# ruihuang1124/CAFE-MPC

Measured on AMD Instinct MI355X. Metric: DDP iterations/sec, Mini-Cheetah WB N=200, batch=4096; 1/2/4/8 GPU, higher is better.
Workload: dtype f64

## Files before the change

### cafe-mpc_amd/csrc/hkd_knot.hpp

```cpp
#pragma once
#include "hs_types.hpp"
#include "srb_knot.hpp"

namespace hs {

constexpr double HKD_MASS = 8.912;
constexpr double HKD_IXX = 0.02746078, HKD_IYY = 0.2425157968, HKD_IZZ = 0.2651935768;

template <class S>
HD void hkd_body_step(const S* xb, const S* pxy, const S* F, double dt, const int* contact, S* out) {
    S sy, cy, st, ct, sp, cp;
    sincos_(xb[0], sy, cy); sincos_(xb[1], st, ct); sincos_(xb[2], sp, cp);
    const V3<S> w{xb[6], xb[7], xb[8]};
    const S dyaw = (sp * w.y + cp * w.z) * srb_recip(ct);
    const S dth = cp * w.y - sp * w.z;
    const S dph = w.x + st * dyaw;
    V3<S> Fs{S(0.0), S(0.0), S(0.0)}, tw{S(0.0), S(0.0), S(0.0)};
    for (int l = 0; l < 4; l++) if (contact[l]) {
        const V3<S> f{F[3 * l], F[3 * l + 1], F[3 * l + 2]};
        const V3<S> r{pxy[2 * l] - xb[3], pxy[2 * l + 1] - xb[4], -xb[5]};
        Fs = Fs + f; tw = tw + cross(r, f);
    }
    const V3<S> tb = rotT<0, S>(cp, sp, rotT<1, S>(ct, st, rotT<2, S>(cy, sy, tw)));
    const V3<S> Iw{HKD_IXX * w.x, HKD_IYY * w.y, HKD_IZZ * w.z};
    const V3<S> rhs = tb - cross(w, Iw);
    out[0] = xb[0] + dt * dyaw; out[1] = xb[1] + dt * dth; out[2] = xb[2] + dt * dph;
    for (int i = 0; i < 3; i++) out[3 + i] = xb[3 + i] + dt * xb[9 + i];
    out[6] = xb[6] + dt * (rhs.x * (1.0 / HKD_IXX)); out[7] = xb[7] + dt * (rhs.y * (1.0 / HKD_IYY)); out[8] = xb[8] + dt * (rhs.z * (1.0 / HKD_IZZ));
    out[9] = xb[9] + dt * (Fs.x * (1.0 / HKD_MASS)); out[10] = xb[10] + dt * (Fs.y * (1.0 / HKD_MASS)); out[11] = xb[11] + dt * (Fs.z * (1.0 / HKD_MASS) - GRAV);
}

template <class S>
HD V3<S> hkd_foot(const S* pos, const S* eul, const S* ql, int leg, double cpsi, double spsi) {
    const double sx = leg < 2 ? 1.0 : -1.0, sgy = (leg % 2 == 0) ? -1.0 : 1.0;
    S s0, c0, s1, c1, s2, c2, sy, cy, st, ct, sp, cp;
    sincos_(ql[0], s0, c0); sincos_(ql[1], s1, c1); sincos_(ql[2], s2, c2);
    sincos_(eul[0], sy, cy); sincos_(eul[1], st, ct); sincos_(eul[2], sp, cp);
    V3<S> w{S(0.0), S(0.0), S(-0.195)};
    w = rot<1, S>(c2, s2, w); w.z = w.z - 0.209;
    w = rot<1, S>(c1, s1, w); w = rot<2, S>(cpsi, spsi, w); w.y = w.y + sgy * 0.062;
    w = rot<0, S>(c0, s0, w); w.x = w.x + sx * 0.19; w.y = w.y + sgy * 0.049;
    w = rot<2, S>(cy, sy, rot<1, S>(ct, st, rot<0, S>(cp, sp, w)));
    return {w.x + pos[0], w.y + pos[1], w.z + pos[2]};
}

struct HkdLds {
    double x[24], xb[24], u[24], xn[24], red[24], tmp[24];
    double K[576];
    double gval[20], bar[20], bd[20], bdd[20];
    double J[4 * 27];
    double pf[12], hx[4 * 24], coefg[4], coefh[4];
};

HD double hkd_grf_row(const double* u, int f, int r, double mu) {
    const double fx = u[3 * f], fy = u[3 * f + 1], fz = u[3 * f + 2];
    return r == 0 ? fz : r == 1 ? -fx + mu * fz : r == 2 ? fx + mu * fz : r == 3 ? -fy + mu * fz : fy + mu * fz;
}
HD double hkd_footreg(PhaseC& P, const double* x, int b, int k) {
    const double* fp = P.foot_pos + ref_row(P, b, k) * 12; const double* bp = P.body_pos + ref_row(P, b, k) * 3;
    double s = 0;
    for (int f = 0; f < 4; f++) for (int a = 0; a < 3; a++) { const double d = (x[12 + 3 * f + a] - x[3 + a]) - (fp[3 * f + a] - bp[a]); s += d * (P.contact[f] * P.w_foot_reg[a]) * d; }
    return s;
}

template <int NT>
HD void hkd_rollout_knot(HkdLds& L, PhaseC& P, int b, int k, double eps, int reb_active, const double* x0, SlotOut so, size_t slot, int* fail_flag, bool ss = false, bool wr = true) {
    const int h = P.h;
    const size_t kx = ((size_t)b * (h + 1) + k) * 24, ku = ((size_t)b * h + k) * 24, kk = (size_t)b * h + k;
    HS_PHASE(NT, if (tid < 24) { double xb = P.Xbar[kx + tid], x = ss ? P.Xsim[kx + tid] : xb + eps * P.dX[kx + tid]; L.xb[tid] = xb; L.x[tid] = x; if (wr) { P.X[kx + tid] = x; if (ss && k == 0) P.Defect[kx + tid] = 0.0; } }
             for (int i = tid; i < 576; i += NT) L.K[i] = P.K[kk * 576 + i];)
    HS_PHASE(NT, if (tid < 24) {
        double s = 0; for (int j = 0; j < 24; j++) s += L.K[tid + 24 * j] * (L.x[j] - L.xb[j]);
        const double u = P.Ubar[ku + tid] + eps * P.dU[ku + tid] + s;
        L.u[tid] = u; if (wr) P.U[ku + tid] = u;
    })
    HS_PHASE(NT, if (tid == 0) {
        double pxy[8]; for (int l = 0; l < 4; l++) { pxy[2 * l] = L.x[12 + 3 * l]; pxy[2 * l + 1] = L.x[13 + 3 * l]; }
        hkd_body_step<double>(L.x, pxy, L.u, P.dt, P.contact, L.xn);
    } else if (tid >= 32 && tid < 44) { const int j = tid - 32; L.xn[12 + j] = P.contact[j / 3] ? L.x[12 + j] : L.x[12 + j] + P.dt * L.u[12 + j]; })
    HS_PHASE(NT, if (tid < 24) {
        const double xs = L.xn[tid];
        if (wr) P.Xsim[kx + 24 + tid] = xs;
        const double d = ss ? 0.0 : xs - (P.Xbar[kx + 24 + tid] + eps * P.dX[kx + 24 + tid]);
        if (wr) P.Defect[kx + 24 + tid] = d;
        double dsq = d * d;
        if (x0 != nullptr && k == 0) { const double d0 = x0[(size_t)b * 24 + tid] - L.x[tid]; if (wr) { P.Xsim[kx + tid] = x0[(size_t)b * 24 + tid]; P.Defect[kx + tid] = d0; } dsq += d0 * d0; }
        L.red[tid] = dsq; L.tmp[tid] = xs * xs;
// ... 1 lines not shown
        const int c = tid - 32; const size_t gi = kk * P.ng + c;
        const double g = hkd_grf_row(L.u, P.feet[c / 5], c % 5, P.mu);
        L.gval[c] = g; if (wr) P.g[gi] = g; L.bar[c] = P.eps[gi] * reb_barrier(g, P.delta[gi]);
    })
    HS_PHASE(NT, if (tid == 0) {
        double lq = 0, lr = 0;
        const size_t rw = ref_row(P, b, k);
        for (int i = 0; i < 24; i++) { const double d = L.x[i] - P.xr[rw * 24 + i]; lq += d * P.q[i] * d; }
        for (int i = 0; i < 24; i++) { const double d = L.u[i] - P.ur[rw * 24 + i]; lr += d * P.r[i] * d; }
        double l = 0.5 * lq; l += 0.5 * lr; l *= P.dt;
        if (P.w_foot_reg[0] >= 0) { double t = .5 * hkd_footreg(P, L.x, b, k); t *= P.dt; l += t; }
        if (wr) P.lbase[kk] = l;
        double ming = 0;
        if (P.ng > 0) {
            double c = 0; for (int i = 0; i < P.ng; i++) { c += L.bar[i]; ming = fmin(ming, L.gval[i]); }
            if (reb_active) l += P.dt * c;
        }
        if (wr) P.l[kk] = l;
        double dsq = 0, nsq = 0; for (int i = 0; i < 24; i++) { dsq += L.red[i]; nsq += L.tmp[i]; }
        so.cost[slot] = l; so.dsq[slot] = dsq; so.ming[slot] = ming; so.maxh[slot] = 0.0;
        if (sqrt(nsq) > 1e6 || !(nsq == nsq)) fail_flag[b] = 1;
    })
}

template <int NT>
HD void hkd_rollout_terminal(HkdLds& L, PhaseC& P, PhaseC* Pn, const ModelDev& md, int b, double eps, int al_active, SlotOut so, size_t slot, bool ss = false, bool wr = true) {
    const int h = P.h;
    const size_t kx = ((size_t)b * (h + 1) + h) * 24;
    HS_PHASE(NT, if (tid < 24) { const double x = ss ? P.Xsim[kx + tid] : P.Xbar[kx + tid] + eps * P.dX[kx + tid]; L.x[tid] = x; if (wr) P.X[kx + tid] = x; })
    HS_PHASE(NT, if (tid < 4 && P.td[tid]) {
        const V3<double> f = hkd_foot<double>(L.x + 3, L.x, L.x + 12 + 3 * tid, tid, md.cpsi_kin, md.spsi_kin);
        L.pf[3 * tid] = f.x; L.pf[3 * tid + 1] = f.y; L.pf[3 * tid + 2] = f.z;
    })
    HS_PHASE(NT, if (tid == 0) {
        double s = 0; const size_t rw = ref_row(P, b, h); for (int i = 0; i < 24; i++) { const double d = L.x[i] - P.xr[rw * 24 + i]; s += d * P.qf[i] * d; }
        double pb = 0.5 * s;
        if (P.w_foot_reg[0] >= 0) pb += 10 * hkd_footreg(P, L.x, b, h);
        if (wr) P.Phibase[b] = pb;
        double maxh = 0, c = 0; int i = 0;
        for (int f = 0; f < 4; f++) if (P.td[f] && P.nt > 0) {
            const double hh = L.pf[3 * f + 2] - P.ground_height; if (wr) P.th[(size_t)b * P.nt + i] = hh; maxh = fmax(maxh, fabs(hh));
            const double sg = P.sigma[(size_t)b * P.nt + i], lm = P.lambda[(size_t)b * P.nt + i];
            c += 0.5 * sg * hh * hh; c += lm * hh; i++;
        }
        double Phi = pb; if (al_active && P.nt > 0) Phi += c;
        if (wr) P.Phi[b] = Phi;
        so.cost[slot] = Phi; so.ming[slot] = 0.0; so.maxh[slot] = maxh; so.dsq[slot] = 0.0;
    })
    if (Pn == nullptr) return;
    const size_t nx = ((size_t)b * (Pn->h + 1)) * 24;
    HS_PHASE(NT, if (tid < 24) {
        double xi = L.x[tid];
        if (tid >= 12) {
            const int l = (tid - 12) / 3, a = (tid - 12) % 3;
            if (P.contact[l] && !P.next_contact[l]) xi = (a == 0) ? 0.0 : (a == 1) ? -0.8 : 1.7;
            if (!P.contact[l] && P.next_contact[l]) xi = (a < 2) ? L.pf[3 * l + a] : 0.0;
        }
        if (wr) Pn->Xsim[nx + tid] = xi;
        const double d = (ss || !Pn->shooting) ? 0.0 : xi - (Pn->Xbar[nx + tid] + eps * Pn->dX[nx + tid]);
        if (wr) Pn->Defect[nx + tid] = d; L.red[tid] = d * d;
    })
    HS_PHASE(NT, if (tid == 0) { double s = 0; for (int i = 0; i < 24; i++) s += L.red[i]; so.dsq[slot] = s; })
}

template <int NT>
HD void hkd_lq_knot(HkdLds& L, PhaseC& P, int b, int k, int reb_active) {
    const int h = P.h; const double dt = P.dt;
    const size_t kx = ((size_t)b * (h + 1) + k) * 24, ku = ((size_t)b * h + k) * 24, kk = (size_t)b * h + k;
    double* AB = L.K;
    HS_PHASE(NT, if (tid < 24) { L.x[tid] = P.X[kx + tid]; L.u[tid] = P.U[ku + tid]; })
    HS_PHASE(NT, if (tid < 32) {
        Dual xb[12], pxy[8], F[12], out[12];
        for (int i = 0; i < 12; i++) { xb[i] = Dual(L.x[i], (tid == i) ? 1.0 : 0.0); F[i] = Dual(L.u[i], (tid == 20 + i) ? 1.0 : 0.0); }
        for (int i = 0; i < 8; i++) pxy[i] = Dual(L.x[12 + 3 * (i / 2) + (i % 2)], (tid == 12 + i) ? 1.0 : 0.0);
        hkd_body_step<Dual>(xb, pxy, F, dt, P.contact, out);
        for (int i = 0; i < 12; i++) AB[i * 32 + tid] = out[i].d;
    } else if (tid >= 32 && tid < 32 + P.ng) {
        const int c = tid - 32; const size_t gi = kk * P.ng + c;
        const double g = P.g[gi], delta = P.delta[gi], e = P.eps[gi]; double bd, bdd;
        if (g > delta) { bd = -1.0 / g; bdd = 1.0 / (g * g); } else { bd = (g - 2 * delta) / delta / delta; bdd = 1.0 / (delta * delta); }
        L.bd[c] = reb_active ? e * bd : 0.0; L.bdd[c] = reb_active ? e * bdd : 0.0;
    })
    const double fr = (P.w_foot_reg[0] >= 0) ? 1.0 : 0.0;
    HS_PHASE(NT, for (int e = tid; e < 576; e += NT) {
        const int r = e % 24, c = e / 24;
        double a, bb;
        if (r < 12) {
            if (c < 12) a = AB[r * 32 + c];
            else { const int l = (c - 12) / 3, ax = (c - 12) % 3; a = (ax < 2) ? AB[r * 32 + 12 + 2 * l + ax] : 0.0; }
            bb = (c < 12) ? AB[r * 32 + 20 + c] : 0.0;
        } else {
            a = (r == c) ? 1.0 : 0.0;
            bb = (r == c && !P.contact[(r - 12) / 3]) ? dt : 0.0;
        }
        rec_put(P, kk, P.oA + e, a); rec_put(P, kk, P.oB + e, bb);
        double q = (r == c) ? dt * P.q[r] : 0.0;
        if (fr != 0.0) {
            if (r == c && r >= 3 && r < 6) { for (int f = 0; f < 4; f++) q += dt * P.contact[f] * P.w_foot_reg[r - 3]; }
            else if (r == c && r >= 12) q += dt * P.contact[(r - 12) / 3] * P.w_foot_reg[(r - 12) % 3];
            else if (r >= 3 && r < 6 && c >= 12 && (c - 12) % 3 == r - 3) q -= dt * P.contact[(c - 12) / 3] * P.w_foot_reg[r - 3];
            else if (c >= 3 && c < 6 && r >= 12 && (r - 12) % 3 == c - 3) q -= dt * P.contact[(r - 12) / 3] * P.w_foot_reg[c - 3];
        }
        rec_put(P, kk, P.oLxx + e, q);
        double uu = (r == c) ? dt * P.r[r] : 0.0;
        if (P.go_grf >= 0 && r < 12 && c < 12 && r / 3 == c / 3) {
            const int f = r / 3; int a2 = -1; for (int t = 0; t < P.nc; t++) if (P.feet[t] == f) a2 = t;
            if (a2 >= 0) for (int cc = 0; cc < 5; cc++) {
                const double r0 = (cc == 1) ? -1.0 : (cc == 2) ? 1.0 : 0.0, r1 = (cc == 3) ? -1.0 : (cc == 4) ? 1.0 : 0.0, r2 = (cc == 0) ? 1.0 : P.mu;
                const double vr = (r % 3 == 0) ? r0 : (r % 3 == 1) ? r1 : r2, vc = (c % 3 == 0) ? r0 : (c % 3 == 1) ? r1 : r2;
                uu += dt * L.bdd[P.go_grf + 5 * a2 + cc] * vr * vc;
            }
        }
        rec_put(P, kk, P.oLuu + e, uu);
    } if (tid < 24) {
        const int i = tid;
        const size_t rw = ref_row(P, b, k);
        double lx = dt * P.q[i] * (L.x[i] - P.xr[rw * 24 + i]);
        if (fr != 0.0) {
            const double* fp = P.foot_pos + rw * 12; const double* bp = P.body_pos + rw * 3;
            if (i >= 3 && i < 6) { for (int f = 0; f < 4; f++) lx -= dt * P.contact[f] * P.w_foot_reg[i - 3] * ((L.x[12 + 3 * f + i - 3] - L.x[i]) - (fp[3 * f + i - 3] - bp[i - 3])); }
            else if (i >= 12) { const int f = (i - 12) / 3, a = (i - 12) % 3; lx += dt * P.contact[f] * P.w_foot_reg[a] * ((L.x[i] - L.x[3 + a]) - (fp[3 * f + a] - bp[a])); }
        }
        rec_put(P, kk, P.oLx + i, lx);
        double lu = dt * P.r[i] * (L.u[i] - P.ur[rw * 24 + i]);
        if (P.go_grf >= 0 && i < 12) {
            const int f = i / 3; int a2 = -1; for (int t = 0; t < P.nc; t++) if (P.feet[t] == f) a2 = t;
            if (a2 >= 0) for (int cc = 0; cc < 5; cc++) {
                const double r0 = (cc == 1) ? -1.0 : (cc == 2) ? 1.0 : 0.0, r1 = (cc == 3) ? -1.0 : (cc == 4) ? 1.0 : 0.0, r2 = (cc == 0) ? 1.0 : P.mu;
                lu += dt * L.bd[P.go_grf + 5 * a2 + cc] * ((i % 3 == 0) ? r0 : (i % 3 == 1) ? r1 : r2);
            }
        }
        rec_put(P, kk, P.oLu + i, lu);
    })
}

template <int NT>
HD void hkd_lq_terminal(HkdLds& L, PhaseC& P, PhaseC* Pn, const ModelDev& md, int b, int al_active) {
    const int h = P.h;
    const size_t kx = ((size_t)b * (h + 1) + h) * 24;
    HS_PHASE(NT, if (tid < 24) L.x[tid] = P.X[kx + tid]; for (int i = tid; i < 96; i += NT) L.hx[i] = 0.0; for (int i = tid; i < 108; i += NT) L.J[i] = 0.0;)
    HS_PHASE(NT, if (tid < 24 && P.td[tid / 6]) {
        const int l = tid / 6, d = tid % 6;
        Dual pos[3], eul[3], ql[3];
        for (int i = 0; i < 3; i++) { pos[i] = Dual(L.x[3 + i]); eul[i] = Dual(L.x[i], (d == i) ? 1.0 : 0.0); ql[i] = Dual(L.x[12 + 3 * l + i], (d == 3 + i) ? 1.0 : 0.0); }
        const V3<Dual> f = hkd_foot<Dual>(pos, eul, ql, l, md.cpsi_kin, md.spsi_kin);
        L.J[l * 27 + 0 * 9 + 3 + d] = f.x.d; L.J[l * 27 + 1 * 9 + 3 + d] = f.y.d; L.J[l * 27 + 2 * 9 + 3 + d] = f.z.d;
        if (d < 3) L.J[l * 27 + d * 9 + d] = 1.0;
    })
    HS_PHASE(NT, if (tid == 0) {
        int t = 0;
        for (int f = 0; f < 4; f++) if (P.td[f] && P.nt > 0) {
            const double sg = P.sigma[(size_t)b * P.nt + t], lm = P.lambda[(size_t)b * P.nt + t], hh = P.th[(size_t)b * P.nt + t];
            L.coefg[t] = al_active ? sg * hh + lm : 0.0; L.coefh[t] = al_active ? sg * (1 + hh) + lm : 0.0;
            for (int j = 0; j < 3; j++) { L.hx[t * 24 + j] = L.J[f * 27 + 2 * 9 + 3 + j]; L.hx[t * 24 + 3 + j] = L.J[f * 27 + 2 * 9 + j]; L.hx[t * 24 + 12 + 3 * f + j] = L.J[f * 27 + 2 * 9 + 6 + j]; }
            t++;
        }
    })
    const double fr = (P.w_foot_reg[0] >= 0) ? 20.0 : 0.0;
    HS_PHASE(NT, for (int e = tid; e < 576; e += NT) {
        const int r = e % 24, c = e / 24;
        double q = (r == c) ? P.qf[r] : 0.0;
        if (fr != 0.0) {
            if (r == c && r >= 3 && r < 6) { for (int f = 0; f < 4; f++) q += fr * P.contact[f] * P.w_foot_reg[r - 3]; }
            else if (r == c && r >= 12) q += fr * P.contact[(r - 12) / 3] * P.w_foot_reg[(r - 12) % 3];
            else if (r >= 3 && r < 6 && c >= 12 && (c - 12) % 3 == r - 3) q -= fr * P.contact[(c - 12) / 3] * P.w_foot_reg[r - 3];
            else if (c >= 3 && c < 6 && r >= 12 && (r - 12) % 3 == c - 3) q -= fr * P.contact[(r - 12) / 3] * P.w_foot_reg[c - 3];
        }
        for (int t = 0; t < P.nt; t++) q += L.coefh[t] * (L.hx[t * 24 + r] * L.hx[t * 24 + c]);
        P.Phixx[(size_t)b * 576 + e] = q;
        if (Pn != nullptr) {
            double v = (r == c) ? 1.0 : 0.0;
            if (r >= 12) {
                const int l = (r - 12) / 3, a = (r - 12) % 3;
                if (P.contact[l] && !P.next_contact[l]) v = 0.0;
                if (!P.contact[l] && P.next_contact[l]) {
                    if (a == 2) v = 0.0;
                    else if (c < 3) v = L.J[l * 27 + a * 9 + 3 + c];
                    else if (c < 6) v = L.J[l * 27 + a * 9 + (c - 3)];
                    else if (c >= 12 && (c - 12) / 3 == l) v = L.J[l * 27 + a * 9 + 6 + (c - 12) % 3];
                    else v = 0.0;
                }
            }
            P.Px[(size_t)b * 576 + e] = v;
        }
    } if (tid < 24) {
        const int i = tid;
        const size_t rw = ref_row(P, b, h);
        double px = P.qf[i] * (L.x[i] - P.xr[rw * 24 + i]);
        if (fr != 0.0) {
            const double* fp = P.foot_pos + rw * 12; const double* bp = P.body_pos + rw * 3;
            if (i >= 3 && i < 6) { for (int f = 0; f < 4; f++) px -= fr * P.contact[f] * P.w_foot_reg[i - 3] * ((L.x[12 + 3 * f + i - 3] - L.x[i]) - (fp[3 * f + i - 3] - bp[i - 3])); }
            else if (i >= 12) { const int f = (i - 12) / 3, a = (i - 12) % 3; px += fr * P.contact[f] * P.w_foot_reg[a] * ((L.x[i] - L.x[3 + a]) - (fp[3 * f + a] - bp[a])); }
        }
        for (int t = 0; t < P.nt; t++) px += L.coefg[t] * L.hx[t * 24 + i];
        P.Phix[(size_t)b * 24 + i] = px;
    })
// ... 4 lines not shown
```

### cafe-mpc_amd/csrc/hs_host.hpp

```cpp
#pragma once
#include <cstring>
#include <vector>
#include <algorithm>
#include "hsddp.h"
#include "hs_types.hpp"

#if !defined(__HIP_DEVICE_COMPILE__)
namespace hs {

inline bool phase_chain_ok(int model, int next_model) {
    if (model == HSDDP_MODEL_WB) return next_model == HSDDP_MODEL_WB || next_model == HSDDP_MODEL_SRB;
    return model == next_model;
}

template <class Mem>
int setup_phase(Mem& mem, const hsddp_phase_desc_t& d, const hsddp_phase_desc_t* next, bool is_last, size_t B, PhaseDev& P, int slot0, bool f32 = false) {
    std::memset(&P, 0, sizeof(P));
    P.model = d.model; P.h = d.horizon; P.dt = d.dt; P.bg_alpha = d.BG_alpha;
    if (d.model == HSDDP_MODEL_WB) { P.n = 36; P.m = 12; P.p = 12; } else if (d.model == HSDDP_MODEL_SRB) { P.n = 12; P.m = 12; P.p = 0; } else { P.n = 24; P.m = 24; P.p = 0; }
    const size_t n = P.n, m = P.m, py = P.p;
    for (int l = 0; l < 4; l++) {
        P.contact[l] = d.contact[l]; P.next_contact[l] = d.next_contact[l];
        if (d.contact[l] > 0) P.feet[P.nc++] = l;
        P.td[l] = (d.contact[l] == 0 && d.next_contact[l] == 1) ? 1 : 0; P.n_td += P.td[l];
    }
    P.has_impact = P.n_td > 0; P.next_model = d.next_model; P.shooting = d.shooting; P.is_last = is_last ? 1 : 0;
    P.next_n = next ? (next->model == HSDDP_MODEL_WB ? 36 : next->model == HSDDP_MODEL_SRB ? 12 : 24) : P.n;
    std::memcpy(P.q, d.q, sizeof(P.q)); std::memcpy(P.r, d.r, sizeof(P.r)); std::memcpy(P.qf, d.qf, sizeof(P.qf));
    std::memcpy(P.w_foot_reg, d.w_foot_reg, 24); std::memcpy(P.w_swing_pos, d.w_swing_pos, 24); std::memcpy(P.w_swing_vel, d.w_swing_vel, 24);
    P.w_td_vel = d.w_td_vel;
    P.c_torque = d.c_torque; P.c_joint = d.c_joint; P.c_minheight = d.c_minheight; P.c_grf = d.c_grf; P.c_touchdown = d.c_touchdown;
    P.torque_limit = d.torque_limit; std::memcpy(P.joint_lb, d.joint_lb, 24); std::memcpy(P.joint_ub, d.joint_ub, 24);
    P.h_min = d.h_min; P.mu = d.mu; P.ground_height = d.ground_height;
    P.c_jspeed = d.c_jointspeed; P.jspeed_lb = d.jointspeed_lb; P.jspeed_ub = d.jointspeed_ub;
    const hsddp_reb_t* rb[5] = {&d.reb_torque, &d.reb_joint, &d.reb_minheight, &d.reb_grf, &d.reb_jointspeed};
    for (int g = 0; g < 5; g++) { P.reb_init[g][0] = rb[g]->delta; P.reb_init[g][1] = rb[g]->delta_min; P.reb_init[g][2] = rb[g]->eps; }
    P.al_init[0] = d.al_td.sigma; P.al_init[1] = d.al_td.lambda; P.al_init[2] = d.al_td.sigma_max;
    int ng = 0; P.go_torque = P.go_joint = P.go_height = P.go_grf = P.go_jspeed = -1;
    const bool wb = d.model == HSDDP_MODEL_WB;
    if (wb && d.c_torque) { P.go_torque = ng; ng += 24; }
    if (wb && d.c_jointspeed) { P.go_jspeed = ng; ng += 24; }
    if (wb && d.c_joint) { P.go_joint = ng; ng += 24; }
    if (d.c_minheight) { P.go_height = ng; ng += 1; }
    const bool hkd = d.model == HSDDP_MODEL_HKD, srb = d.model == HSDDP_MODEL_SRB;
    if (hkd) { ng = 0; P.go_height = -1; }
    if ((wb || hkd) && d.c_grf && P.nc > 0) { P.go_grf = ng; ng += 5 * P.nc; }
    if (srb) { P.n_td = 0; P.has_impact = 0; for (int l = 0; l < 4; l++) P.td[l] = 0; }
    P.ng = ng; P.nt = (!srb && d.c_touchdown) ? P.n_td : 0; P.slot0 = slot0;
    { int offs[5], sz[5]; P.nobj = constraint_objects(P, offs, sz); P.obj_off = P.obj_sz = 0;
      for (int o = 0; o < P.nobj; o++) { P.obj_off |= (unsigned long long)offs[o] << (8 * o); P.obj_sz |= (unsigned long long)sz[o] << (8 * o); } }
    const size_t h1 = P.h + 1, hh = P.h;
    bool ok = true;
    auto up = [&](const double** dst, const double* src, size_t cnt) { void* p = mem.alloc(cnt * 8); if (!p) { ok = false; return; } if (src) mem.upload(p, src, cnt * 8); *dst = (const double*)p; };
    up(&P.xr, d.xr, h1 * n); up(&P.ur, d.ur, h1 * m); up(&P.yr, py ? d.yr : nullptr, h1 * std::max<size_t>(py, 1));
    up(&P.foot_pos, d.foot_pos, h1 * 12); up(&P.foot_vel, d.foot_vel, h1 * 12); up(&P.body_pos, d.body_pos, h1 * 3);
    { void* p = mem.alloc(h1 * 4 * sizeof(int)); if (!p) ok = false; else { if (d.ref_contact) mem.upload(p, d.ref_contact, h1 * 4 * sizeof(int)); P.ref_contact = (const int*)p; } }
    if (d.model == HSDDP_MODEL_WB) {
        std::vector<double> rr(h1 * 80, 0.0);
        for (size_t k = 0; k < h1; k++) {
            double* r = rr.data() + k * 80;
            if (d.xr) for (int i = 0; i < 36; i++) r[i] = d.xr[k * 36 + i];
            if (d.ur) for (int i = 0; i < 12; i++) r[36 + i] = d.ur[k * 12 + i];
            if (d.foot_vel) for (int i = 0; i < 12; i++) r[48 + i] = d.foot_vel[k * 12 + i];
            if (d.ref_contact) for (int i = 0; i < 4; i++) r[60 + i] = (double)d.ref_contact[k * 4 + i];
            for (int i = 0; i < 12; i++) r[64 + i] = (d.foot_pos ? d.foot_pos[k * 12 + i] : 0.0) - (d.body_pos ? d.body_pos[k * 3 + i % 3] : 0.0);
        }
        up(&P.rref, rr.data(), h1 * 80);
    }
    auto al = [&](double** dst, size_t cnt) { void* p = mem.alloc(std::max<size_t>(cnt, 1) * 8); if (!p) ok = false; *dst = (double*)p; };
    double** sx[] = {&P.X, &P.Xbar, &P.Xsim, &P.Defect, &P.Defect_bar, &P.dX, &P.G};
    for (auto p : sx) al(p, B * h1 * n);
    double** su[] = {&P.U, &P.Ubar, &P.dU, &P.Qu, &P.KdX};
    for (auto p : su) al(p, B * hh * m);
    al(&P.Y, B * hh * py);
    double** smn[] = {&P.K, &P.Qux};
    for (auto p : smn) al(p, B * hh * m * n);
    al(&P.Quu, B * hh * m * m);
    {
        auto rnd = [](size_t x) { return (x + 255) / 256 * 256; };
        const size_t ar = (size_t)rec_arows((int)n);
        const size_t oA = 0, oLxx = oA + rnd(ar * n), oB = oLxx + rnd(n * n), oC = oB + rnd(ar * m), oD = oC + rnd(py * n), oLuu = oD + rnd(py * m),
                     oLyy = oLuu + rnd(m * m), oLx = oLyy + rnd(py * py), oLu = oLx + n, oLy = oLu + m, size = oLx + rnd(n + m + py);
        P.rs = (int)size;
        P.oA = (int)oA; P.oLxx = (int)oLxx; P.oB = (int)oB; P.oC = (int)oC; P.oD = (int)oD; P.oLuu = (int)oLuu; P.oLyy = (int)oLyy; P.oLx = (int)oLx; P.oLu = (int)oLu; P.oLy = (int)oLy;
        if (f32) { void* p = mem.alloc(std::max<size_t>(B * hh * size, 1) * sizeof(float)); if (!p) ok = false; P.rec32 = (float*)p; }
        else al(&P.rec, B * hh * size);
        if (P.rec) { P.A = P.rec + oA; P.lxx = P.rec + oLxx; P.B = P.rec + oB; P.C = P.rec + oC; P.D = P.rec + oD; P.luu = P.rec + oLuu;
                     P.lyy = P.rec + oLyy; P.lx = P.rec + oLx; P.lu = P.rec + oLu; P.ly = P.rec + oLy; }
    }
    al(&P.l, B * hh); al(&P.lbase, B * hh);
    al(&P.Phi, B); al(&P.Phibase, B); al(&P.Phix, B * n); al(&P.Phixx, B * n * n); al(&P.H0, B * n * n); al(&P.Px, B * (size_t)P.next_n * n);
    al(&P.g, B * hh * ng); al(&P.delta, B * hh * ng); al(&P.eps, B * hh * ng);
    if (wb) al(&P.kc, B * hh * KC_SIZE);
    al(&P.th, B * P.nt); al(&P.sigma, B * P.nt); al(&P.lambda, B * P.nt);
    if (!ok) return HSDDP_ENOMEM;
    if (ng > 0) {
        std::vector<double> dl(hh * ng), ep(hh * ng);
        for (size_t k = 0; k < hh; k++) for (int c = 0; c < ng; c++) { int grp = constraint_group(P, c); dl[k * ng + c] = P.reb_init[grp][0]; ep[k * ng + c] = P.reb_init[grp][2]; }
        mem.upload(P.delta, dl.data(), dl.size() * 8); mem.replicate(P.delta, dl.size() * 8, B);
        mem.upload(P.eps, ep.data(), ep.size() * 8); mem.replicate(P.eps, ep.size() * 8, B);
    }
    if (P.nt > 0) { std::vector<double> sg(B * P.nt, P.al_init[0]), lm(B * P.nt, P.al_init[1]); mem.upload(P.sigma, sg.data(), sg.size() * 8); mem.upload(P.lambda, lm.data(), lm.size() * 8); }
    return HSDDP_OK;
}

inline const double* field_dev(const PhaseDev& P, int f, int& count, int& elems) {
    const int n = P.n, m = P.m, p = P.p, h = P.h;
    switch (f) {
        case HSDDP_F_X: count = h + 1; elems = n; return P.X;
        case HSDDP_F_XBAR: count = h + 1; elems = n; return P.Xbar;
        case HSDDP_F_XSIM: count = h + 1; elems = n; return P.Xsim;
        case HSDDP_F_DEFECT: count = h + 1; elems = n; return P.Defect;
        case HSDDP_F_DX: count = h + 1; elems = n; return P.dX;
        case HSDDP_F_G: count = h + 1; elems = n; return P.G;
        case HSDDP_F_U: count = h; elems = m; return P.U;
        case HSDDP_F_UBAR: count = h; elems = m; return P.Ubar;
        case HSDDP_F_DU: count = h; elems = m; return P.dU;
        case HSDDP_F_QU: count = h; elems = m; return P.Qu;
        case HSDDP_F_Y: count = h; elems = p; return P.Y;
        case HSDDP_F_K: count = h; elems = m * n; return P.K;
        case HSDDP_F_QUX: count = h; elems = m * n; return P.Qux;
        case HSDDP_F_QUU: count = h; elems = m * m; return P.Quu;
        case HSDDP_F_A: count = h; elems = n * n; return P.A;
        case HSDDP_F_B: count = h; elems = n * m; return P.B;
        case HSDDP_F_C: count = h; elems = p * n; return P.C;
        case HSDDP_F_D: count = h; elems = p * m; return P.D;
        case HSDDP_F_L: count = h; elems = 1; return P.l;
        case HSDDP_F_LX: count = h; elems = n; return P.lx;
        case HSDDP_F_LU: count = h; elems = m; return P.lu;
        case HSDDP_F_LY: count = h; elems = p; return P.ly;
        case HSDDP_F_LXX: count = h; elems = n * n; return P.lxx;
        case HSDDP_F_LUX: count = h; elems = m * n; return nullptr;
        case HSDDP_F_LUU: count = h; elems = m * m; return P.luu;
        case HSDDP_F_LYY: count = h; elems = p * p; return P.lyy;
        case HSDDP_F_PHI: count = 1; elems = 1; return P.Phi;
        case HSDDP_F_PHIX: count = 1; elems = n; return P.Phix;
        case HSDDP_F_PHIXX: count = 1; elems = n * n; return P.Phixx;
        case HSDDP_F_H0: count = 1; elems = n * n; return P.H0;
        case HSDDP_F_REB_EPS: count = h; elems = P.ng; return P.eps;
        case HSDDP_F_REB_DELTA: count = h; elems = P.ng; return P.delta;
        case HSDDP_F_AL_SIGMA: count = 1; elems = P.nt; return P.sigma;
        case HSDDP_F_AL_LAMBDA: count = 1; elems = P.nt; return P.lambda;
        default: count = 0; elems = 0; return nullptr;
    }
}

inline bool wb_structured(const PhaseDev& P, int f) { return P.model == HSDDP_MODEL_WB && (f == HSDDP_F_A || f == HSDDP_F_B); }
inline void wb_expand_ab(int f, double dt, const double* stored, double* full) {
    const int cols = f == HSDDP_F_A ? 36 : 12;
    for (int c = 0; c < cols; c++) for (int r = 0; r < 36; r++) {
        double v;
        if (r >= 18) v = stored[(r - 18) + 18 * c];
        else v = f == HSDDP_F_A ? ((c == r ? 1.0 : 0.0) + (c == 18 + r ? dt : 0.0)) : 0.0;
        full[r + 36 * c] = v;
    }
}

inline const double* field_dev(const PhaseDev& P, int f, int& count, int& elems, int& stride) {
    const double* base = field_dev(P, f, count, elems);
    const bool in_rec = (f == HSDDP_F_A || f == HSDDP_F_B || f == HSDDP_F_C || f == HSDDP_F_D || f == HSDDP_F_LX || f == HSDDP_F_LU || f == HSDDP_F_LY ||
                         f == HSDDP_F_LXX || f == HSDDP_F_LUU || f == HSDDP_F_LYY);
    stride = in_rec ? P.rs : elems;
    return base;
}

}
#endif
```

### cafe-mpc_amd/csrc/hs_types.hpp

```cpp
#pragma once
#include "hs_common.hpp"

namespace hs {

constexpr int MAXN = 36, MAXM = 24, MAXP = 12, MAXG = 96;
constexpr int rec_rnd(int x) { return (x + 255) / 256 * 256; }
constexpr int rec_arows(int N) { return N == 36 ? 18 : N; }
template <int N, int M, int PY> struct RecLayout {
    static constexpr int AR = rec_arows(N);
    static constexpr int oA = 0, oLxx = oA + rec_rnd(AR * N), oB = oLxx + rec_rnd(N * N), oC = oB + rec_rnd(AR * M), oD = oC + rec_rnd(PY * N),
                         oLuu = oD + rec_rnd(PY * M), oLyy = oLuu + rec_rnd(M * M), oLx = oLyy + rec_rnd(PY * PY), oLu = oLx + N, oLy = oLu + M,
                         size = oLx + rec_rnd(N + M + PY);
    static constexpr int rA = rec_rnd(AR * N) / 256, rQ = rec_rnd(N * N) / 256, rB = rec_rnd(AR * M) / 256, rC = rec_rnd(PY * N) / 256, rD = rec_rnd(PY * M) / 256,
                         rLuu = rec_rnd(M * M) / 256, rLyy = rec_rnd(PY * PY) / 256;
    static constexpr int rounds = rA + rQ + rB + rC + rD + rLuu + rLyy;
};

constexpr int KC_M = 0, KC_X = 324, KC_LG = 540, KC_RDM = 684, KC_RDG = 702, KC_QDD = 714, KC_GRF = 732, KC_LAM = 744, KC_J = 756, KC_FP = 972, KC_FV = 984, KC_SIZE = 1024;

struct PhaseDev {
    int model, n, m, p, h;
    double dt, bg_alpha;
    int contact[4], next_contact[4], td[4], feet[4];
    int nc, n_td, has_impact, next_model, next_n, shooting, is_last;
    double q[MAXN], r[MAXM], qf[MAXN], w_foot_reg[3], w_swing_pos[3], w_swing_vel[3], w_td_vel;
    int c_torque, c_joint, c_minheight, c_grf, c_touchdown, c_jspeed;
    double torque_limit, joint_lb[3], joint_ub[3], h_min, mu, ground_height, jspeed_lb, jspeed_ub;
    double reb_init[5][3];
    double al_init[3];
    int ng, go_torque, go_joint, go_height, go_grf, go_jspeed;
    int nt;
    int slot0;
    int nobj; unsigned long long obj_off, obj_sz;
    const HS_GLOBAL double *xr, *ur, *yr, *foot_pos, *foot_vel, *body_pos;
    const HS_GLOBAL int* ref_contact;
    const HS_GLOBAL double* rref;
    int ref_pb;
    HS_GLOBAL double *X, *Xbar, *Xsim, *Defect, *Defect_bar, *dX, *G;
    HS_GLOBAL double *U, *Ubar, *dU, *Qu;
    HS_GLOBAL double *KdX;
    HS_GLOBAL double *Y;
    HS_GLOBAL double *K, *Qux, *Quu;
    HS_GLOBAL double *A, *B, *C, *D;
    HS_GLOBAL double* rec; int rs;
    HS_GLOBAL float* rec32;
    int oA, oLxx, oB, oC, oD, oLuu, oLyy, oLx, oLu, oLy;
    HS_GLOBAL double *l, *lbase, *lx, *lu, *ly, *lxx, *luu, *lyy;
    HS_GLOBAL double *Phi, *Phibase, *Phix, *Phixx, *H0, *Px;
    HS_GLOBAL double *g, *delta, *eps;
    HS_GLOBAL double* kc;
    HS_GLOBAL double *th, *sigma, *lambda;
};

template <class PD> HD void rec_put(PD& P, size_t kk, int off, double v) {
    if (P.rec32 != nullptr) P.rec32[kk * P.rs + off] = (float)v; else P.rec[kk * P.rs + off] = v;
}

template <class PD> HD size_t ref_row(PD& P, int b, int k) { return (unsigned)(b * P.ref_pb + k); }

using PhaseC = const HS_CONST PhaseDev;

HDH int constraint_group(const PhaseDev& P, int c) {
    if (P.go_torque >= 0 && c >= P.go_torque && c < P.go_torque + 24) return 0;
    if (P.go_jspeed >= 0 && c >= P.go_jspeed && c < P.go_jspeed + 24) return 4;
    if (P.go_joint >= 0 && c >= P.go_joint && c < P.go_joint + 24) return 1;
    if (P.go_height >= 0 && c == P.go_height) return 2;
    return 3;
}
HDH int constraint_objects(const PhaseDev& P, int* offs, int* sz) {
    int n = 0;
    if (P.go_torque >= 0) { offs[n] = P.go_torque; sz[n++] = 24; }
    if (P.go_jspeed >= 0) { offs[n] = P.go_jspeed; sz[n++] = 24; }
    if (P.go_joint >= 0) { offs[n] = P.go_joint; sz[n++] = 24; }
    if (P.go_height >= 0) { offs[n] = P.go_height; sz[n++] = 1; }
    if (P.go_grf >= 0) { offs[n] = P.go_grf; sz[n++] = 5 * P.nc; }
    return n;
}

struct ProbState {
    double actual_cost, merit, feas, dV_1, dV_2, merit_rho;
    double cost_prev, merit_prev, feas_prev, reg;
    double max_tconstr, max_pconstr, max_tconstr_prev, max_pconstr_prev;
    double info_tconstr, info_pconstr;
    double ls_eps;
    int iter, ls_total, reg_total, status;
    int outer_active, inner_active, ls_active, ls_success, rollout_ok, bs_ok;
    int iter_in, iter_ou;
    int hist_n, push_pending;
    int need_commit, pad_;
};

struct OptDev {
    double alpha, gamma, update_penalty, update_relax, update_regularization, update_ReB;
    int max_DDP_iter, max_AL_iter;
    double cost_thresh, tconstr_thresh, pconstr_thresh, dynamics_feas_thresh, merit_scale, merit_offset;
    int AL_active, ReB_active, MS;
};

struct ModelDev { double cpsi_dyn, spsi_dyn, cpsi_kin, spsi_kin; };

}
```

### cafe-mpc_amd/csrc/hsddp_hip.hip

```cpp
#include <hip/hip_runtime.h>
#include <atomic>
#include <chrono>
#include <cstdio>
#include <cstring>
#include <string>
#include <thread>
#include <vector>
#include <cmath>
#include "hsddp.h"
#include "hsddp_ensemble.h"
#include "hsddp_hkd.h"
#include "hsddp_refs.h"
#include "hsddp_sim.h"
#include "hsddp_mc.h"
#include "hs_types.hpp"
#include "hs_host.hpp"
#include "wb_knot.hpp"
#include "wb_quad.hpp"
#include "srb_knot.hpp"
#include "hkd_knot.hpp"
#include "sweep.hpp"
#include "ensemble.hpp"
#include "hkd_pack.hpp"
#include "refs.hpp"
// ... 1001 lines not shown
    HIPCK(hipGetLastError());
    return HSDDP_OK;
}

int hsddp_hybrid_rollout(hsddp_handle_t* h, double eps, const hsddp_option_t* opt) {
    if (!h || !opt) return HSDDP_EINVAL;
    HIPCK(hipSetDevice(h->device)); OptDev o = to_dev(*opt);
    launch_rollout(h, eps, o, MASK_NONE); launch_eval(h, EV_REDUCE_ONLY, o, 0.0, false, 0);
    HIPCK(hipStreamSynchronize(h->stream)); drain_events(h); HIPCK(hipGetLastError()); return HSDDP_OK;
}
int hsddp_compute_cost(hsddp_handle_t* h, const hsddp_option_t* opt) {
    if (!h || !opt) return HSDDP_EINVAL; HIPCK(hipSetDevice(h->device)); OptDev o = to_dev(*opt);
    launch_cost(h, o, MASK_NONE); launch_eval(h, EV_REDUCE_ONLY, o, 0.0, false, 0);
    HIPCK(hipStreamSynchronize(h->stream)); drain_events(h); HIPCK(hipGetLastError()); return HSDDP_OK;
}
int hsddp_LQ_approximation(hsddp_handle_t* h, const hsddp_option_t* opt) {
    if (!h || !opt) return HSDDP_EINVAL; HIPCK(hipSetDevice(h->device)); OptDev o = to_dev(*opt);
    launch_lq(h, o, MASK_NONE); HIPCK(hipStreamSynchronize(h->stream)); drain_events(h); HIPCK(hipGetLastError()); return HSDDP_OK;
}
int hsddp_backward_sweep(hsddp_handle_t* h, double regularization, int* success) {
    if (!h) return HSDDP_EINVAL; HIPCK(hipSetDevice(h->device)); OptDev o{};
    launch_sweep(h, o, MASK_NONE, regularization, 0, 0, 0.0, h->d_success);
    if (!h->has_hkd && !h->f32) hipLaunchKernelGGL(k_refresh_kdx, dim3(64, h->batch), dim3(64), 0, h->stream, h->d_ph, h->nph);
    HIPCK(hipStreamSynchronize(h->stream)); drain_events(h); HIPCK(hipGetLastError());
    if (success) HIPCK(hipMemcpy(success, h->d_success, h->batch * sizeof(int), hipMemcpyDeviceToHost));
    return HSDDP_OK;
}
int hsddp_linear_rollout(hsddp_handle_t* h, double eps, const hsddp_option_t* opt) {
    (void)opt; if (!h) return HSDDP_EINVAL; HIPCK(hipSetDevice(h->device));
    { Timed t(h, "k_linear");
      if (h->f32) hipLaunchKernelGGL(k_linear32, dim3(h->batch), dim3(SW_NT), 0, h->stream, h->d_ph, h->nph, h->d_st, eps);
      else if (h->has_hkd) hipLaunchKernelGGL(k_linear_hkd, dim3(h->batch), dim3(SW_NT), 0, h->stream, h->d_ph, h->nph, h->d_st, eps);
      else hipLaunchKernelGGL(k_linear, dim3(h->batch), dim3(SW_NT), 0, h->stream, h->d_ph, h->nph, h->d_st, eps); }
    HIPCK(hipStreamSynchronize(h->stream)); drain_events(h); HIPCK(hipGetLastError()); return HSDDP_OK;
}
int hsddp_update_nominal_trajectory(hsddp_handle_t* h) {
    if (!h) return HSDDP_EINVAL; HIPCK(hipSetDevice(h->device));
    launch_update_nominal(h, MASK_NONE); HIPCK(hipStreamSynchronize(h->stream)); drain_events(h); return HSDDP_OK;
}
static int read_states(hsddp_handle* h, std::vector<ProbState>& st) {
    st.resize(h->batch); HIPCK(hipSetDevice(h->device));
    HIPCK(hipMemcpy(st.data(), h->d_st, sizeof(ProbState) * h->batch, hipMemcpyDeviceToHost)); return HSDDP_OK;
}
int hsddp_get_exp_cost_change(hsddp_handle_t* h, double* dV_1, double* dV_2) {
    if (!h || !dV_1 || !dV_2) return HSDDP_EINVAL;
    std::vector<ProbState> st; int rc = read_states(h, st); if (rc) return rc;
    for (int b = 0; b < h->batch; b++) { dV_1[b] = st[b].dV_1; dV_2[b] = st[b].dV_2; } return HSDDP_OK;
}
int hsddp_measure_dynamics_feasibility(hsddp_handle_t* h, double* feas) {
    if (!h || !feas) return HSDDP_EINVAL;
    std::vector<ProbState> st; int rc = read_states(h, st); if (rc) return rc;
    for (int b = 0; b < h->batch; b++) feas[b] = st[b].feas; return HSDDP_OK;
}
int hsddp_get_info(hsddp_handle_t* h, hsddp_info_t* info) {
    if (!h || !info) return HSDDP_EINVAL;
    std::vector<ProbState> st; int rc = read_states(h, st); if (rc) return rc;
    for (int b = 0; b < h->batch; b++) {
        info[b].actual_cost = st[b].actual_cost; info[b].dyn_feas = st[b].feas; info[b].max_tconstr = st[b].info_tconstr; info[b].max_pconstr = st[b].info_pconstr;
        info[b].n_iters = st[b].iter; info[b].n_ls_iters = st[b].ls_total; info[b].n_reg_iters = st[b].reg_total; info[b].status = st[b].status;
    }
    return HSDDP_OK;
}

int hsddp_get_history(hsddp_handle_t* h, int problem, int cap, float* cost, float* dyn_feas, float* eqn_feas, float* ineq_feas, int* n) {
    if (!h || problem < 0 || problem >= h->batch || cap < 0 || !n) return HSDDP_EINVAL;
    HIPCK(hipSetDevice(h->device));
    ProbState st; HIPCK(hipMemcpy(&st, h->d_st + problem, sizeof(ProbState), hipMemcpyDeviceToHost));
    const int have = std::min(st.hist_n, h->hist_cap); *n = have;
    const int m = std::min(have, cap);
    float* dst[4] = {cost, dyn_feas, eqn_feas, ineq_feas};
    for (int q = 0; q < 4 && m > 0; q++) if (dst[q]) HIPCK(hipMemcpy(dst[q], h->d_hist + ((size_t)problem * 4 + q) * h->hist_cap, m * sizeof(float), hipMemcpyDeviceToHost));
    return HSDDP_OK;
}

int hsddp_field_shape(hsddp_handle_t* h, int phase, int field, int* count, int* elems) {
    if (!h || phase < 0 || phase >= h->nph || field < 0 || field >= HSDDP_F_COUNT) return HSDDP_EINVAL;
    int stride; field_dev(h->ph[phase], field, *count, *elems, stride); return HSDDP_OK;
}
int hsddp_get_field(hsddp_handle_t* h, int phase, int field, int b0, int nb, double* dst) {
    if (!h || phase < 0 || phase >= h->nph || field < 0 || field >= HSDDP_F_COUNT || b0 < 0 || nb < 0 || b0 + nb > h->batch || !dst) return HSDDP_EINVAL;
    HIPCK(hipSetDevice(h->device));
    int count, elems, stride; const double* src = field_dev(h->ph[phase], field, count, elems, stride);
    const size_t sz = (size_t)count * elems;
    if (h->f32 && stride != elems && sz > 0 && nb > 0) {
        const PhaseDev& P = h->ph[phase];
        const int off = field == HSDDP_F_A ? P.oA : field == HSDDP_F_B ? P.oB : field == HSDDP_F_C ? P.oC : field == HSDDP_F_D ? P.oD : field == HSDDP_F_LX ? P.oLx : field == HSDDP_F_LU ? P.oLu :
                        field == HSDDP_F_LY ? P.oLy : field == HSDDP_F_LXX ? P.oLxx : field == HSDDP_F_LUU ? P.oLuu : P.oLyy;
        std::vector<float> tmp(sz * nb);
        HIPCK(hipMemcpy2D(tmp.data(), (size_t)elems * 4, P.rec32 + (size_t)b0 * count * stride + off, (size_t)stride * 4, (size_t)elems * 4, (size_t)nb * count, hipMemcpyDeviceToHost));
        for (size_t i = 0; i < tmp.size(); i++) dst[i] = tmp[i];
        return HSDDP_OK;
    }
    if (!src) { memset(dst, 0, sz * nb * 8); return HSDDP_OK; }
    if (sz == 0 || nb == 0) return HSDDP_OK;
    if (wb_structured(h->ph[phase], field)) {
        const int st = field == HSDDP_F_A ? 648 : 216;
        std::vector<double> tmp((size_t)st * nb * count);
        HIPCK(hipMemcpy2D(tmp.data(), (size_t)st * 8, src + (size_t)b0 * count * stride, (size_t)stride * 8, (size_t)st * 8, (size_t)nb * count, hipMemcpyDeviceToHost));
        for (size_t r = 0; r < (size_t)nb * count; r++) wb_expand_ab(field, h->ph[phase].dt, tmp.data() + r * st, dst + r * elems);
        return HSDDP_OK;
    }
    if (stride == elems) HIPCK(hipMemcpy(dst, src + (size_t)b0 * sz, sz * nb * 8, hipMemcpyDeviceToHost));
    else HIPCK(hipMemcpy2D(dst, (size_t)elems * 8, src + (size_t)b0 * count * stride, (size_t)stride * 8, (size_t)elems * 8, (size_t)nb * count, hipMemcpyDeviceToHost));
    return HSDDP_OK;
}
float hsddp_get_solve_time_ms(hsddp_handle_t* h) { return h ? h->solve_ms : 0.f; }

int hsddp_warm_start_phase(hsddp_handle_t* dst, int dphase, hsddp_handle_t* src, int sphase, int shift) {
    if (!dst || dphase < 0 || dphase >= dst->nph || shift < 0) return HSDDP_EINVAL;
    const PhaseDev& D = dst->ph[dphase];
    dst->cache_valid = false;
    const bool has = src != nullptr && sphase >= 0;
    if (has && (sphase >= src->nph || src->batch != dst->batch || src->device != dst->device || src->ph[sphase].model != D.model)) return HSDDP_EINVAL;
    HIPCK(hipSetDevice(dst->device));
    if (has) HIPCK(hipStreamSynchronize(src->stream));
    hipLaunchKernelGGL(k_warm_start, dim3(D.h + 1, dst->batch), dim3(256), 0, dst->stream, D, has ? src->ph[sphase] : D, has ? 1 : 0, shift);
    HIPCK(hipStreamSynchronize(dst->stream));
    return HSDDP_OK;
}

int hsddp_export_mpc_command(hsddp_handle_t* h, int problem, int n_steps, double mpc_time, double dt, const float* status_times, unsigned int* out) {
    if (!h || problem < 0 || problem >= h->batch || n_steps <= 0 || !out) return HSDDP_EINVAL;
    std::vector<int> sp, sk;
    for (int i = 0; i < h->nph && (int)sp.size() < n_steps; i++) {
        if (h->ph[i].model != HSDDP_MODEL_WB) break;
        for (int k = 0; k < h->ph[i].h && (int)sp.size() < n_steps; k++) { sp.push_back(i); sk.push_back(k); }
    }
    if ((int)sp.size() < n_steps) return HSDDP_EINVAL;
    HIPCK(hipSetDevice(h->device));
    const size_t words = 1 + (size_t)n_steps * HSDDP_CMD_WORDS_PER_STEP;
    if (words > h->cmd_words) { if (h->d_cmd) HIPCK(hipFree(h->d_cmd)); h->d_cmd = nullptr; h->cmd_words = 0; HIPCK(hipMalloc((void**)&h->d_cmd, words * 4)); h->cmd_words = words; }
    if (n_steps > h->cmd_steps) { if (h->d_cmd_map) HIPCK(hipFree(h->d_cmd_map)); h->d_cmd_map = nullptr; h->cmd_steps = 0; HIPCK(hipMalloc((void**)&h->d_cmd_map, 2 * (size_t)n_steps * sizeof(int))); h->cmd_steps = n_steps; }
    if (status_times && !h->d_cmd_status) HIPCK(hipMalloc((void**)&h->d_cmd_status, (size_t)h->nph * 4 * sizeof(float)));
    HIPCK(hipMemcpyAsync(h->d_cmd_map, sp.data(), n_steps * sizeof(int), hipMemcpyHostToDevice, h->stream));
    HIPCK(hipMemcpyAsync(h->d_cmd_map + n_steps, sk.data(), n_steps * sizeof(int), hipMemcpyHostToDevice, h->stream));
    if (status_times) HIPCK(hipMemcpyAsync(h->d_cmd_status, status_times, (size_t)h->nph * 4 * sizeof(float), hipMemcpyHostToDevice, h->stream));
    hipLaunchKernelGGL(k_pack_command, dim3(n_steps), dim3(256), 0, h->stream, h->d_ph, h->d_cmd_map, h->d_cmd_map + n_steps, n_steps, problem, mpc_time, dt,
                       status_times ? h->d_cmd_status : nullptr, h->d_cmd);
    HIPCK(hipMemcpyAsync(out, h->d_cmd, words * 4, hipMemcpyDeviceToHost, h->stream));
    HIPCK(hipStreamSynchronize(h->stream));
    return HSDDP_OK;
}

int hsddp_export_solver_info(hsddp_handle_t* h, int problem, unsigned int* out) {
    if (!h || problem < 0 || problem >= h->batch || !out) return HSDDP_EINVAL;
    HIPCK(hipSetDevice(h->device));
    ProbState st; HIPCK(hipMemcpy(&st, h->d_st + problem, sizeof(ProbState), hipMemcpyDeviceToHost));
    const int iv[3] = {st.iter, st.ls_total, st.reg_total};
    const float fv[5] = {h->solve_ms, (float)st.actual_cost, (float)st.feas, (float)st.info_pconstr, (float)st.info_tconstr};
    memcpy(out, iv, sizeof(iv)); memcpy(out + 3, fv, sizeof(fv));
    return HSDDP_OK;
}

int hsddp_get_kernel_units(hsddp_handle_t* h, const char* name, long long* units) {
    if (!h || !name || !units) return HSDDP_EINVAL;
    const int id = !strcmp(name, "k_rollout") ? UNIT_ROLLOUT : !strcmp(name, "k_lq") ? UNIT_LQ : !strcmp(name, "k_sweep") ? UNIT_SWEEP : !strcmp(name, "k_ls_probe") ? UNIT_PROBE : -1;
    if (id < 0) return HSDDP_EINVAL;
    HIPCK(hipSetDevice(h->device));
    unsigned long long v = 0; HIPCK(hipMemcpy(&v, h->d_units + id, sizeof(v), hipMemcpyDeviceToHost));
    *units = (long long)v; return HSDDP_OK;
}

int hsddp_get_kernel_times(hsddp_handle_t* h, int max_n, double* ms, long long* launches, char* names, int names_cap) {
    if (!h) return 0;
    int n = std::min<int>(max_n, (int)h->kname.size()); int pos = 0;
    for (int i = 0; i < n; i++) {
        ms[i] = h->kms[i]; launches[i] = h->kcnt[i];
        int len = (int)h->kname[i].size();
        if (pos + len + 1 < names_cap) { memcpy(names + pos, h->kname[i].c_str(), len + 1); pos += len + 1; }
    }
    if (pos < names_cap) names[pos] = 0;
    return n;
}
#if defined(LQ_PROF) || defined(ROLL_PROF)
int hsddp_debug_lq_prof(unsigned long long* out16, int reset) {
    hipMemcpyFromSymbol(out16, HIP_SYMBOL(g_lq_prof), 16 * sizeof(unsigned long long));
    if (reset) { unsigned long long z[16] = {0}; hipMemcpyToSymbol(HIP_SYMBOL(g_lq_prof), z, sizeof(z)); }
    return 0;
}
#endif
#ifdef QUAD_PROF
int hsddp_debug_quad_prof(unsigned long long* out24, int reset) {
    hipMemcpyFromSymbol(out24, HIP_SYMBOL(g_quad_prof), 24 * sizeof(unsigned long long));
    if (reset) { unsigned long long z[24] = {0}; hipMemcpyToSymbol(HIP_SYMBOL(g_quad_prof), z, sizeof(z)); }
// ... 530 lines not shown
```

### cafe-mpc_amd/csrc/srb_knot.hpp

```cpp
#pragma once
#include "hs_types.hpp"
#include "wb_knot.hpp"

namespace hs {

constexpr double SRB_MASS = 8.912;
constexpr double SRB_IXX = 0.061578036, SRB_IYY = 0.2207093, SRB_IZZ = 0.272612336, SRB_IXZ = 5.38e-5;

HD double srb_recip(double a) { return 1.0 / a; }
HD Dual srb_recip(Dual a) { const double r = 1.0 / a.v; return Dual(r, -a.d * r * r); }

template <class S>
HD void srb_xdot(const S* x, const S* u, const double* pf, const int* contact, S* xd) {
    S sy, cy, st, ct, sp, cp;
    sincos_(x[3], sy, cy); sincos_(x[4], st, ct); sincos_(x[5], sp, cp);
    const S dyaw = x[9], dth = x[10], dph = x[11];
    V3<S> F{S(0.0), S(0.0), S(0.0)}, tw{S(0.0), S(0.0), S(0.0)};
    for (int l = 0; l < 4; l++) if (contact[l]) {
        const V3<S> f{u[3 * l], u[3 * l + 1], u[3 * l + 2]};
        const V3<S> r{S(pf[3 * l]) - x[0], S(pf[3 * l + 1]) - x[1], S(pf[3 * l + 2]) - x[2]};
        F = F + f; tw = tw + cross(r, f);
    }
    for (int i = 0; i < 6; i++) xd[i] = x[6 + i];
    xd[6] = F.x * (1.0 / SRB_MASS); xd[7] = F.y * (1.0 / SRB_MASS); xd[8] = F.z * (1.0 / SRB_MASS) - GRAV;
    const V3<S> tb = rotT<0, S>(cp, sp, rotT<1, S>(ct, st, rotT<2, S>(cy, sy, tw)));
    const V3<S> w{dph - st * dyaw, sp * ct * dyaw + cp * dth, cp * ct * dyaw - sp * dth};
    const V3<S> Iw{SRB_IXX * w.x + SRB_IXZ * w.z, SRB_IYY * w.y, SRB_IXZ * w.x + SRB_IZZ * w.z};
    const V3<S> rhs = tb - cross(w, Iw);
    constexpr double det = SRB_IXX * SRB_IZZ - SRB_IXZ * SRB_IXZ;
    const V3<S> wd{(SRB_IZZ * rhs.x - SRB_IXZ * rhs.z) * (1.0 / det), rhs.y * (1.0 / SRB_IYY), (SRB_IXX * rhs.z - SRB_IXZ * rhs.x) * (1.0 / det)};
    const V3<S> c0d{-(ct * dth), cp * ct * dph - sp * st * dth, -(sp * ct * dph) - cp * st * dth};
    const V3<S> c1d{S(0.0), -(sp * dph), -(cp * dph)};
    const V3<S> bb = wd - (scale(dyaw, c0d) + scale(dth, c1d));
    const S ddyaw = (sp * bb.y + cp * bb.z) * srb_recip(ct);
    xd[9] = ddyaw; xd[10] = cp * bb.y - sp * bb.z; xd[11] = bb.x + st * ddyaw;
}

struct SrbLds {
    double x[12], xb[12], u[12], xd[12], red[12], tmp[12];
    double K[144], AB[288];
    double g, bar, bd, bdd;
};

template <int NT>
HD void srb_rollout_knot(SrbLds& L, PhaseC& P, int b, int k, double eps, int reb_active, const double* x0, SlotOut so, size_t slot, int* fail_flag, bool ss = false, bool wr = true) {
    const int h = P.h;
    const size_t kx = ((size_t)b * (h + 1) + k) * 12, ku = ((size_t)b * h + k) * 12, kk = (size_t)b * h + k;
    HS_PHASE(NT, if (tid < 12) { double xb = P.Xbar[kx + tid], x = ss ? P.Xsim[kx + tid] : xb + eps * P.dX[kx + tid]; L.xb[tid] = xb; L.x[tid] = x; if (wr) { P.X[kx + tid] = x; if (ss && k == 0) P.Defect[kx + tid] = 0.0; } }
             for (int i = tid; i < 144; i += NT) L.K[i] = P.K[kk * 144 + i];)
    HS_PHASE(NT, if (tid < 12) {
        double s = 0; for (int j = 0; j < 12; j++) s += L.K[tid + 12 * j] * (L.x[j] - L.xb[j]);
        const double u = P.Ubar[ku + tid] + eps * P.dU[ku + tid] + s;
        L.u[tid] = u; if (wr) P.U[ku + tid] = u;
    })
    HS_PHASE(NT, if (tid == 0) srb_xdot<double>(L.x, L.u, P.foot_pos + ref_row(P, b, k) * 12, P.ref_contact + ref_row(P, b, k) * 4, L.xd);)
    HS_PHASE(NT, if (tid < 12) {
        const double xs = L.x[tid] + L.xd[tid] * P.dt;
        if (wr) P.Xsim[kx + 12 + tid] = xs;
        const double d = ss ? 0.0 : xs - (P.Xbar[kx + 12 + tid] + eps * P.dX[kx + 12 + tid]);
        if (wr) P.Defect[kx + 12 + tid] = d;
        double dsq = d * d;
        if (x0 != nullptr && k == 0) { const double d0 = x0[(size_t)b * 12 + tid] - L.x[tid]; if (wr) { P.Xsim[kx + tid] = x0[(size_t)b * 12 + tid]; P.Defect[kx + tid] = d0; } dsq += d0 * d0; }
        L.red[tid] = dsq; L.tmp[tid] = xs * xs;
    })
    HS_PHASE(NT, if (tid == 0) {
        double lq = 0, lr = 0;
        const size_t rw = ref_row(P, b, k);
        for (int i = 0; i < 12; i++) { const double d = L.x[i] - P.xr[rw * 12 + i]; lq += d * P.q[i] * d; }
        for (int i = 0; i < 12; i++) { const double d = L.u[i] - P.ur[rw * 12 + i]; lr += d * P.r[i] * d; }
        double l = 0.5 * lq; l += 0.5 * lr; l *= P.dt;
        if (wr) P.lbase[kk] = l;
        double ming = 0;
        if (P.go_height >= 0) {
            const size_t gi = kk * P.ng + P.go_height; const double g = L.x[2] - P.h_min;
            if (wr) P.g[gi] = g; ming = fmin(ming, g);
            if (reb_active) l += P.dt * (P.eps[gi] * reb_barrier(g, P.delta[gi]));
        }
        if (wr) P.l[kk] = l;
        double dsq = 0, nsq = 0; for (int i = 0; i < 12; i++) { dsq += L.red[i]; nsq += L.tmp[i]; }
        so.cost[slot] = l; so.dsq[slot] = dsq; so.ming[slot] = ming; so.maxh[slot] = 0.0;
        if (sqrt(nsq) > 1e6 || !(nsq == nsq)) fail_flag[b] = 1;
    })
}

template <int NT>
HD void srb_rollout_terminal(SrbLds& L, PhaseC& P, PhaseC* Pn, int b, double eps, SlotOut so, size_t slot, bool ss = false, bool wr = true) {
    const int h = P.h;
    const size_t kx = ((size_t)b * (h + 1) + h) * 12;
    HS_PHASE(NT, if (tid < 12) { const double x = ss ? P.Xsim[kx + tid] : P.Xbar[kx + tid] + eps * P.dX[kx + tid]; L.x[tid] = x; if (wr) P.X[kx + tid] = x; })
    HS_PHASE(NT, if (tid == 0) {
        double s = 0; const size_t rw = ref_row(P, b, h); for (int i = 0; i < 12; i++) { const double d = L.x[i] - P.xr[rw * 12 + i]; s += d * P.qf[i] * d; }
        const double Phi = 0.5 * s;
        if (wr) { P.Phibase[b] = Phi; P.Phi[b] = Phi; }
        so.cost[slot] = Phi; so.ming[slot] = 0.0; so.maxh[slot] = 0.0; so.dsq[slot] = 0.0;
    })
    if (Pn == nullptr) return;
    const size_t nx = ((size_t)b * (Pn->h + 1)) * 12;
    HS_PHASE(NT, if (tid < 12) {
        const double xi = L.x[tid];
        if (wr) Pn->Xsim[nx + tid] = xi;
        const double d = (ss || !Pn->shooting) ? 0.0 : xi - (Pn->Xbar[nx + tid] + eps * Pn->dX[nx + tid]);
        if (wr) Pn->Defect[nx + tid] = d; L.red[tid] = d * d;
    })
    HS_PHASE(NT, if (tid == 0) { double s = 0; for (int i = 0; i < 12; i++) s += L.red[i]; so.dsq[slot] = s; })
}

template <int NT>
HD void srb_lq_knot(SrbLds& L, PhaseC& P, int b, int k, int reb_active) {
    const int h = P.h; const double dt = P.dt;
    const size_t kx = ((size_t)b * (h + 1) + k) * 12, ku = ((size_t)b * h + k) * 12, kk = (size_t)b * h + k;
    HS_PHASE(NT, if (tid < 12) { L.x[tid] = P.X[kx + tid]; L.u[tid] = P.U[ku + tid]; })
    HS_PHASE(NT, if (tid < 24) {
        Dual xs[12], us[12], out[12];
        for (int i = 0; i < 12; i++) { xs[i] = Dual(L.x[i], (tid == i) ? 1.0 : 0.0); us[i] = Dual(L.u[i], (tid == 12 + i) ? 1.0 : 0.0); }
        srb_xdot<Dual>(xs, us, P.foot_pos + ref_row(P, b, k) * 12, P.ref_contact + ref_row(P, b, k) * 4, out);
        for (int i = 0; i < 12; i++) L.AB[i + 12 * tid] = out[i].d * dt + ((tid == i) ? 1.0 : 0.0);
    } if (tid == 32) {
        double bd = 0, bdd = 0;
        if (P.go_height >= 0 && reb_active) {
            const size_t gi = kk * P.ng + P.go_height; const double g = P.g[gi], delta = P.delta[gi], e = P.eps[gi];
            if (g > delta) { bd = -1.0 / g; bdd = 1.0 / (g * g); } else { bd = (g - 2 * delta) / delta / delta; bdd = 1.0 / (delta * delta); }
            bd *= e; bdd *= e;
        }
        L.bd = bd; L.bdd = bdd;
    })
    HS_PHASE(NT, for (int e = tid; e < 144; e += NT) {
        const int r = e % 12, c = e / 12;
        rec_put(P, kk, P.oA + e, L.AB[e]); rec_put(P, kk, P.oB + e, L.AB[144 + e]);
        double qd = 0, rd = 0;
        if (r == c) { qd = dt * P.q[r]; rd = dt * P.r[r]; if (r == 2) qd += dt * L.bdd; }
        rec_put(P, kk, P.oLxx + e, qd); rec_put(P, kk, P.oLuu + e, rd);
    } if (tid < 12) {
        double lx = dt * P.q[tid] * (L.x[tid] - P.xr[ref_row(P, b, k) * 12 + tid]); if (tid == 2) lx += dt * L.bd;
        rec_put(P, kk, P.oLx + tid, lx);
        rec_put(P, kk, P.oLu + tid, dt * P.r[tid] * (L.u[tid] - P.ur[ref_row(P, b, k) * 12 + tid]));
    })
}

template <int NT>
HD void srb_lq_terminal(SrbLds& L, PhaseC& P, PhaseC* Pn, int b) {
    const int h = P.h;
    const size_t kx = ((size_t)b * (h + 1) + h) * 12;
    HS_PHASE(NT, if (tid < 12) P.Phix[(size_t)b * 12 + tid] = P.qf[tid] * (P.X[kx + tid] - P.xr[ref_row(P, b, h) * 12 + tid]);
             for (int e = tid; e < 144; e += NT) { P.Phixx[(size_t)b * 144 + e] = (e % 12 == e / 12) ? P.qf[e % 12] : 0.0; if (Pn != nullptr) P.Px[(size_t)b * 144 + e] = (e % 12 == e / 12) ? 1.0 : 0.0; })
    (void)L;
}

}
```

### cafe-mpc_amd/csrc/sweep.hpp

```cpp
#pragma once
#include <cstddef>
#include <limits>
#include <type_traits>
#include "hs_types.hpp"
#include "hs_mfma.hpp"

namespace hs {

constexpr int SW_NT = 256;
constexpr int SW_SET_WB = 0, SW_SET_HKD = 1;
constexpr int SW_N = 36;
constexpr int SW_PRE = 20;
#ifndef SW_UNROLL_N
#define SW_UNROLL_N 4
#endif
#define HS_STR_(x) #x
#define HS_UNROLL_N(n) _Pragma(HS_STR_(unroll n))
#ifndef SW_LDLT_NB
#define SW_LDLT_NB ((M <= 12 || sizeof(R) == 4) ? 2 : 1)
#endif
#ifndef SW_MINB
#define SW_MINB 2
#endif
#ifndef SW_LDLT_WDW
#define SW_LDLT_WDW 1
#endif
#ifndef SW_OVERLAP_LDLT
#define SW_OVERLAP_LDLT 1
#endif

template <int N, int M, int PY, class R = double> struct SweepLdsT {
    static constexpr int LDN = N + 1, LDM = (M > PY ? M : PY) + 1, PYd = PY > 0 ? PY : 1;
    static constexpr int AR = rec_arows(N), LDA = AR + 1, A0 = N - AR;
    R H[LDN * N], A[LDA * N], HA[LDN * N];
    R B[LDA * M], HB[LDN * M];
    R Qux[LDM * N];
    union { R K[LDM * N]; R lC[PY > 0 ? LDM * N : 1]; };
    R C[PY > 0 ? LDM * N : 1], D[PY > 0 ? LDM * M : 1];
    union { R LQ[LDM * M]; R lD[PY > 0 ? LDM * M : 1]; };
    R lyy[PY > 0 ? LDM * PY : 1], Quu[LDM * M];
    R G[N], Gn[N], Qx[N], Qu[M], dU[M], ly[PYd], def[N];
};
template <int N, int M, int PY, class R = double> struct LinLdsT {
    static constexpr int AR = rec_arows(N), A0 = N - AR;
    R A[2][AR * N], Q[2][N * N], B[2][AR * M], K[2][M * N], U[2][M * M], v[2][256];
    R dx[N], dxn[N], du[M];
};
struct SweepCtl { double dV1, dV2, xfer[SW_N]; unsigned long long t_last; int ok; };
constexpr size_t sw_max(size_t a, size_t b) { return a > b ? a : b; }
template <class R> constexpr size_t sweep_bytes_wb() { return sw_max(sw_max(sizeof(SweepLdsT<36, 12, 12, R>), sizeof(LinLdsT<36, 12, 12, R>)), sw_max(sizeof(SweepLdsT<12, 12, 0, R>), sizeof(LinLdsT<12, 12, 0, R>))); }
template <class R> constexpr size_t sweep_bytes_hkd() { return sw_max(sw_max(sizeof(SweepLdsT<24, 24, 0, R>), sizeof(LinLdsT<24, 24, 0, R>)), sw_max(sizeof(SweepLdsT<12, 12, 0, R>), sizeof(LinLdsT<12, 12, 0, R>))); }
template <class R, int SET> struct SweepLdsRaw { R raw[(SET == 0 ? sweep_bytes_wb<R>() : sweep_bytes_hkd<R>()) / sizeof(R)]; SweepCtl c; };
using SweepLds = SweepLdsRaw<double, 0>;
using SweepLdsHkd = SweepLdsRaw<double, 1>;
using SweepLds32 = SweepLdsRaw<float, 1>;

#define CM(M, i, j, ld) (M)[(i) + (ld) * (j)]

#if defined(SW_PROF) && !defined(HS_HOST_EMU)
__device__ unsigned long long g_sw_prof[48];
#define SW_STAMP(i) { if (blockIdx.x == 0 && threadIdx.x == 0) { unsigned long long t_ = clock64(); atomicAdd(&g_sw_prof[i], t_ - SWC.t_last); SWC.t_last = t_; } }
#define SW_STAMP0() { if (blockIdx.x == 0 && threadIdx.x == 0) SWC.t_last = clock64(); }
#define SW_WSTAMP(p) { if (blockIdx.x == 0 && (tid & 63) == 0) atomicAdd(&g_sw_prof[16 + 4 * (p) + (tid >> 6)], clock64() - SWC.t_last); }
#else
#define SW_WSTAMP(p)
#define SW_STAMP(i)
#define SW_STAMP0()
#endif

#ifdef HS_HOST_EMU
#define SW_PRE_DECL static R pre_all_[SW_NT][SW_PRE];
#define PRE(r) pre_all_[tid][r]
#else
#define SW_PRE_DECL R pre_[SW_PRE];
#define PRE(r) pre_[r]
#endif

#ifndef HS_HOST_EMU
template <int CTRL> HD double dpp_quad(double v) {
    const int lo = __builtin_amdgcn_mov_dpp(__double2loint(v), CTRL, 0xf, 0xf, true), hi = __builtin_amdgcn_mov_dpp(__double2hiint(v), CTRL, 0xf, 0xf, true);
    return __hiloint2double(hi, lo);
}
HD double quad_sum(double v) { v += dpp_quad<0xB1>(v); v += dpp_quad<0x4E>(v); return v; }
template <int CTRL> HD float dpp_quad(float v) { return __int_as_float(__builtin_amdgcn_mov_dpp(__float_as_int(v), CTRL, 0xf, 0xf, true)); }
HD float quad_sum(float v) { v += dpp_quad<0xB1>(v); v += dpp_quad<0x4E>(v); return v; }
#endif
#ifdef HS_HOST_EMU
#define SW_QS 1
#define SW_QUAD_ROWS(CNT, PARTIAL, FINISH) if (tid < (CNT)) { const int o = tid; R p_[4]; R p2_[4]; for (int part = 0; part < 4; part++) { R partial = 0; R partial2 = 0; PARTIAL p_[part] = partial; p2_[part] = partial2; } \
    const R total = (p_[0] + p_[1]) + (p_[2] + p_[3]); const R total2 = (p2_[0] + p2_[1]) + (p2_[2] + p2_[3]); (void)total2; FINISH }
#else
#define SW_QS 4
#define SW_QUAD_ROWS(CNT, PARTIAL, FINISH) if ((tid >> 2) < (CNT)) { const int o = tid >> 2; const int part = tid & 3; R partial = 0; R partial2 = 0; PARTIAL \
    const R total = quad_sum(partial); const R total2 = quad_sum(partial2); (void)total2; if (part == 0) FINISH }
#endif

template <int M, int LD, class R, int PART>
HD void ldlt_parts(int tid, const R* A, R diag_add, R* NI, R* Lw, int* iw, int* ok, R* W1 = nullptr, R* W2 = nullptr) {
    const R TOL = R(1.0) / std::numeric_limits<R>::max();
#ifdef HS_HOST_EMU
    if (PART == 2) return;
    if (tid == 0) {
        R m[M * M]; int tr[M]; int sign = 0; (void)Lw; (void)iw;
        for (int j = 0; j < M; j++) for (int i = 0; i < M; i++) m[i + M * j] = A[i + LD * j] + (i == j ? diag_add : 0.0);
        auto Mx = [&](int i, int j) -> R& { return m[i + M * j]; };
        R temp[M];
        for (int k = 0; k < M; k++) {
            int big = k; R best = std::fabs(Mx(k, k));
            for (int i = k + 1; i < M; i++) if (std::fabs(Mx(i, i)) > best) { best = std::fabs(Mx(i, i)); big = i; }
            tr[k] = big;
            if (k != big) {
                for (int j = 0; j < k; j++) { const R t = Mx(k, j); Mx(k, j) = Mx(big, j); Mx(big, j) = t; }
                for (int i = big + 1; i < M; i++) { const R t = Mx(i, k); Mx(i, k) = Mx(i, big); Mx(i, big) = t; }
                { const R t = Mx(k, k); Mx(k, k) = Mx(big, big); Mx(big, big) = t; }
                for (int i = k + 1; i < big; i++) { const R t = Mx(i, k); Mx(i, k) = Mx(big, i); Mx(big, i) = t; }
            }
            for (int j = 0; j < k; j++) temp[j] = Mx(j, j) * Mx(k, j);
            { R s = 0; for (int j = 0; j < k; j++) s += Mx(k, j) * temp[j]; Mx(k, k) -= s; }
            for (int i = k + 1; i < M; i++) { R t = 0; for (int j = 0; j < k; j++) t += Mx(i, j) * temp[j]; Mx(i, k) -= t; }
            const R akk = Mx(k, k); const bool valid = std::fabs(akk) > 0.0;
            if (valid) for (int i = k + 1; i < M; i++) Mx(i, k) /= akk;
            if (sign == 1) { if (akk < 0) sign = 2; } else if (sign == -1) { if (akk > 0) sign = 2; } else if (sign == 0) { if (akk > 0) sign = 1; else if (akk < 0) sign = -1; }
        }
        if (!(sign == 1 || sign == 0)) *ok = 0;
        for (int c = 0; c < M; c++) {
            R x[M]; for (int i = 0; i < M; i++) x[i] = (i == c) ? 1.0 : 0.0;
            for (int k = 0; k < M; k++) if (tr[k] != k) { const R t = x[k]; x[k] = x[tr[k]]; x[tr[k]] = t; }
            for (int i = 0; i < M; i++) { R s = x[i]; for (int j = 0; j < i; j++) s -= Mx(i, j) * x[j]; x[i] = s; }
// ... 43 lines not shown
        int pv[M]; int myrank = 0;
        _Pragma("unroll") for (int k = 0; k < M; k++) { pv[k] = iw[k]; myrank = (pv[k] == me) ? k : myrank; }
        if (PART != 2) {
        const int prow = iw[me];
        R arow[M];
        _Pragma("unroll") for (int j = 0; j < M; j++) { const int r = prow > pv[j] ? prow : pv[j], c = prow > pv[j] ? pv[j] : prow; arow[j] = A[r + LD * c] + ((j == me) ? diag_add : 0.0); }
        SW_LSTAMP(10)
        bool anyneg = false;
        _Pragma("unroll") for (int j = 0; j < M; j++) {
            const R d = hs_readlane(arow[j], j);
            R rd = hs_rcp(d); rd = rd * (R(2.0) - d * rd); rd = rd * (R(2.0) - d * rd);
            rd = (fabs(d) > TOL) ? rd : 0.0;
            anyneg = anyneg || (d < 0.0);
            const R lij = (fabs(d) > 0.0) ? arow[j] * rd : arow[j];
            if (M <= 12) { if (act && me >= j) Lw[me * M + j] = (me == j) ? rd : lij; }
            else if (act) { if (me > j) Lw[me * M + j] = lij; else if (me == j) Lw[j * M + j] = rd; }
            _Pragma("unroll") for (int k = j + 1; k < M; k++) arow[k] -= lij * hs_readlane(arow[j], k);
        }
        SW_LSTAMP(11)
        if (tid == 0 && anyneg) *ok = 0;
        }
        if (PART == 1) return;
        __builtin_amdgcn_fence(__ATOMIC_RELEASE, "wavefront"); __builtin_amdgcn_wave_barrier(); __builtin_amdgcn_fence(__ATOMIC_ACQUIRE, "wavefront");
        constexpr int NB = SW_LDLT_NB;
        R y[M], lr[NB][M];
        if (NB == 1) { lr[0][0] = 0.0; }
        _Pragma("unroll") for (int k = 0; k < M; k++) {
            if (NB == 2) { if (k + 1 < M) { _Pragma("unroll") for (int j = 0; j <= k; j++) lr[(k + 1) % NB][j] = Lw[(k + 1) * M + j]; } }
            else { _Pragma("unroll") for (int j = 0; j < k; j++) lr[0][j] = Lw[k * M + j]; }
            HS_CBAR();
            R sacc = (k == myrank) ? 1.0 : 0.0;
            _Pragma("unroll") for (int j = 0; j < k; j++) sacc -= lr[k % NB][j] * y[j];
            HS_PIN(sacc);
            y[k] = sacc;
        }
        SW_LSTAMP(12)
#if SW_LDLT_WDW
        if (PART == 2 && sizeof(R) == 8) {
            if (act) { _Pragma("unroll") for (int k = 0; k < M; k++) { W1[k + M * me] = y[k]; W2[k + M * me] = -(y[k] * Lw[k * M + k]); } }
            __builtin_amdgcn_fence(__ATOMIC_RELEASE, "wavefront"); __builtin_amdgcn_wave_barrier(); __builtin_amdgcn_fence(__ATOMIC_ACQUIRE, "wavefront");
            constexpr int TMq = (M + 15) / 16;
            MTileT<R> td[TMq * TMq];
            _Pragma("unroll") for (int t = 0; t < TMq * TMq; t++) td[t] = MTileT<R>{NI, LD, nullptr, 0, 16 * (t % TMq), 16 * (t / TMq), M, M, W1, M, W2, M, M, true, nullptr, 0, nullptr, 0, 0};
            mfma_tiles<TMq * TMq, (M + 3) / 4 * 4, 0, R>(tid, td);
            SW_LSTAMP(13)
            return;
        }
#endif
        _Pragma("unroll") for (int k = 0; k < M; k++) y[k] = y[k] * Lw[k * M + k];
        _Pragma("unroll") for (int k = M - 1; k >= 0; k--) {
            if (NB == 2) { if (k > 0) { _Pragma("unroll") for (int j = k; j < M; j++) lr[(k - 1) % NB][j] = Lw[j * M + (k - 1)]; } }
            else { _Pragma("unroll") for (int j = k + 1; j < M; j++) lr[0][j] = Lw[j * M + k]; }
            HS_CBAR();
            R sacc = y[k];
            _Pragma("unroll") for (int j = k + 1; j < M; j++) sacc -= lr[k % NB][j] * y[j];
            HS_PIN(sacc);
            y[k] = sacc;
        }
        if (act) { _Pragma("unroll") for (int k = 0; k < M; k++) NI[pv[k] + LD * me] = -y[k]; }
        SW_LSTAMP(13)
    }
#endif
}
template <int M, int LD, class R>
HD void ldlt_inverse_w(const R* A, R diag_add, R* NI, R* Lw, int* iw, int* ok) {
    HS_WPHASE(ldlt_parts<M, LD, R, 0>(tid, A, diag_add, NI, Lw, iw, ok);)
}
template <int NT, class TD, class TS> HD void ld_mat(int tid, TD* dst, int ldd, const TS* src, int rows, int cols) {
    const int i = tid % rows, j0 = tid / rows, js = NT / rows;
    if (j0 < js) for (int j = j0; j < cols; j += js) dst[i + ldd * j] = src[i + rows * j];
}
template <int NT, class TD, class TS> HD void st_mat(int tid, TD* dst, const TS* src, int lds_, int rows, int cols) {
    const int i = tid % rows, j0 = tid / rows, js = NT / rows;
    if (j0 < js) for (int j = j0; j < cols; j += js) dst[i + rows * j] = src[i + lds_ * j];
}

#define SW_RICCATI_FETCH(kk_, k_) { \
    const HS_GLOBAL R* rec_ = grec + (kk_) * (size_t)RL::size + tid; \
    _Pragma("unroll") for (int r = 0; r < RL::rounds; r++) if (r < RL::rA || r >= RL::rA + RL::rQ) PRE(r) = rec_[NT * r];      \
    PRE(RL::rounds) = (tid < N + M + PY) ? rec_[RL::oLx] : (tid < 2 * N + M + PY) ? (R)gDefect[((size_t)b * (h + 1) + (k_) + 1) * N + tid - N - M - PY] : R(0.0); }
#define SW_RICCATI_FETCH_LXX(kk_) { \
    const HS_GLOBAL R* rec_ = grec + (kk_) * (size_t)RL::size + tid; \
    _Pragma("unroll") for (int r = RL::rA; r < RL::rA + RL::rQ; r++) PRE(r) = rec_[NT * r]; }
#define SW_RICCATI_LXX() { \
    _Pragma("unroll") for (int r = 0; r < RL::rQ; r++) { const int e = tid + NT * r; if (e < N * N) S.H[(e % N) + LDN * (e / N)] += PRE(RL::rA + r); } }
#define SW_RICCATI_COMMIT() { \
    constexpr int PYd = PY > 0 ? PY : 1; \
    _Pragma("unroll") for (int r = 0; r < RL::rA; r++) { const int e = tid + NT * r; if (e < AR * N) S.A[(e % AR) + LDA * (e / AR)] = PRE(r); } \
    _Pragma("unroll") for (int r = 0; r < RL::rB; r++) { const int e = tid + NT * r; if (e < AR * M) S.B[(e % AR) + LDA * (e / AR)] = PRE(RL::rA + RL::rQ + r); } \
    _Pragma("unroll") for (int r = 0; r < RL::rC; r++) { const int e = tid + NT * r; if (e < PY * N) S.C[(e % PYd) + LDM * (e / PYd)] = PRE(RL::rA + RL::rQ + RL::rB + r); } \
    _Pragma("unroll") for (int r = 0; r < RL::rD; r++) { const int e = tid + NT * r; if (e < PY * M) S.D[(e % PYd) + LDM * (e / PYd)] = PRE(RL::rA + RL::rQ + RL::rB + RL::rC + r); } \
    _Pragma("unroll") for (int r = 0; r < RL::rLuu; r++) { const int e = tid + NT * r; if (e < M * M) S.Quu[(e % M) + LDM * (e / M)] = PRE(RL::rA + RL::rQ + RL::rB + RL::rC + RL::rD + r); } \
    _Pragma("unroll") for (int r = 0; r < RL::rLyy; r++) { const int e = tid + NT * r; if (e < PY * PY) S.lyy[(e % PYd) + LDM * (e / PYd)] = PRE(RL::rA + RL::rQ + RL::rB + RL::rC + RL::rD + RL::rLuu + r); } \
    if (tid < N) S.Qx[tid] = PRE(RL::rounds); else if (tid < N + M) S.Qu[tid - N] = PRE(RL::rounds); else if (tid < N + M + PY) S.ly[tid - N - M] = PRE(RL::rounds); \
    else if (tid < 2 * N + M + PY) S.def[tid - N - M - PY] = PRE(RL::rounds); }

template <class R> HD const HS_GLOBAL R* rec_of(const PhaseDev& P);
template <> HD const HS_GLOBAL double* rec_of<double>(const PhaseDev& P) { return P.rec; }
template <> HD const HS_GLOBAL float* rec_of<float>(const PhaseDev& P) { return P.rec32; }

template <class E> HD constexpr int deal_order(int n, int ix) {
    int c = 0;
    for (int e = 0; e < n; e++) if (!E::edge(e)) { if (c == ix) return e; c++; }
    for (int e = 0; e < n; e++) if (E::edge(e)) { if (c == ix) return e; c++; }
    return ix;
}
template <int W, int N, int M, int PY, class R, int DEAL = 0>
HD void sweep_tiles1(SweepLdsT<N, M, PY, R>& S, int lane, R dt) {
    constexpr int LDN = SweepLdsT<N, M, PY, R>::LDN, LDM = SweepLdsT<N, M, PY, R>::LDM, AR = SweepLdsT<N, M, PY, R>::AR, LDA = SweepLdsT<N, M, PY, R>::LDA, A0 = SweepLdsT<N, M, PY, R>::A0;
    constexpr int TN = (N + 15) / 16, TM = (M + 15) / 16, TP = (PY + 15) / 16, TPd = TP > 0 ? TP : 1;
    constexpr int t1 = TN * TN, t2 = t1 + TN * TM, t3 = t2 + TP * TN, t4 = t3 + TP * TM;
    constexpr bool WBT = (DEAL == 0 && t4 == 16 && t3 == 15);
    constexpr int nA = t1 + (t3 - t2), nB = (t2 - t1) + (t4 - t3);
    constexpr int NTL = DEAL == 1 ? (W == 0 ? nB : (nA - (W - 1) + 2) / 3) : WBT ? (W == 0 ? 5 : W == 3 ? 3 : 4) : (t4 - W + 3) / 4;
    if (NTL <= 0) return;
    MTileT<R> td[NTL > 0 ? NTL : 1];
    _Pragma("unroll") for (int q = 0; q < NTL; q++) {
        struct E1 { static constexpr bool edge(int e) { return e < t1 ? mfma_edge_tile<R>(N, N, 16 * (e % TN), 16 * (e / TN)) : mfma_edge_tile<R>(PY, N, 16 * ((e - t1) % TPd), 16 * ((e - t1) / TPd)); } };
        const int ix = DEAL == 1 && W > 0 ? deal_order<E1>(nA, (W - 1) + 3 * q) : (W - 1) + 3 * q;
        const int t = DEAL == 1 ? (W == 0 ? (q < t2 - t1 ? t1 + q : t3 + (q - (t2 - t1))) : (ix < t1 ? ix : t2 + (ix - t1))) : (WBT && W == 0 && q == 4) ? 15 : W + 4 * q;
        if (t < t1) { td[q] = MTileT<R>{S.HA, LDN, nullptr, 0, 16 * (t % TN), 16 * (t / TN), N, N, S.H + LDN * A0, LDN, S.A, LDA, AR, false, nullptr, 0, nullptr, 0, 0};
                      if (A0 > 0) { td[q].T = S.H; td[q].ldt = LDN; td[q].tmode = 1; td[q].tsplit = A0; td[q].tscale = dt; } }
        else if (t < t2) td[q] = MTileT<R>{S.HB, LDN, nullptr, 0, 16 * ((t - t1) % TN), 16 * ((t - t1) / TN), N, M, S.H + LDN * A0, LDN, S.B, LDA, AR, false, nullptr, 0, nullptr, 0, 0};
        else if (t < t3) td[q] = MTileT<R>{S.lC, LDM, nullptr, 0, 16 * ((t - t2) % TPd), 16 * ((t - t2) / TPd), PY, N, S.lyy, LDM, S.C, LDM, PY, false, nullptr, 0, nullptr, 0, 0};
        else td[q] = MTileT<R>{S.lD, LDM, nullptr, 0, 16 * ((t - t3) % TPd), 16 * ((t - t3) / TPd), PY, M, S.lyy, LDM, S.D, LDM, PY, false, nullptr, 0, nullptr, 0, 0};
    }
    mfma_tiles<(NTL > 0 ? NTL : 1), ((AR > PY ? AR : PY) + 3) / 4 * 4, 0, R>(lane, td);
}
template <int W, int N, int M, int PY, class R, int DEAL = 0>
HD void sweep_tiles2(SweepLdsT<N, M, PY, R>& S, int lane, R reg, R dt) {
    constexpr int LDN = SweepLdsT<N, M, PY, R>::LDN, LDM = SweepLdsT<N, M, PY, R>::LDM, AR = SweepLdsT<N, M, PY, R>::AR, LDA = SweepLdsT<N, M, PY, R>::LDA, A0 = SweepLdsT<N, M, PY, R>::A0;
    constexpr int TN = (N + 15) / 16, TM = (M + 15) / 16;
    constexpr int t1 = TN * (TN + 1) / 2, t2 = t1 + TM * TN, t3 = t2 + TM * TM;
    constexpr int NTL = DEAL == 0 ? (t3 - W + 3) / 4 : DEAL == 2 ? (t3 - t2 - W + 3) / 4 : (W == 0 ? t3 - t2 : (t2 - (W - 1) + 2) / 3);
    if (NTL <= 0) return;
    MTileT<R> td[NTL > 0 ? NTL : 1];
    _Pragma("unroll") for (int q = 0; q < NTL; q++) {
        struct E2 { static constexpr bool edge(int e) {
            if (e < t1) { int c = 0; for (int jj = 0; jj < TN; jj++) for (int ii = 0; ii <= jj; ii++) { if (c == e) return mfma_edge_tile<R>(N, N, 16 * ii, 16 * jj); c++; } return false; }
            return mfma_edge_tile<R>(M, N, 16 * ((e - t1) % TM), 16 * ((e - t1) / TM)); } };
        const int t = DEAL == 0 ? W + 4 * q : DEAL == 2 ? t2 + W + 4 * q : (W == 0 ? t2 + q : deal_order<E2>(t2, (W - 1) + 3 * q));
        int bi = 0, bj = 0;
        { int c = 0; for (int jj = 0; jj < TN; jj++) for (int ii = 0; ii <= jj; ii++) { if (c == t) { bi = ii; bj = jj; } c++; } }
        if (t < t1) { td[q] = MTileT<R>{S.H, LDN, nullptr, 0, 16 * bi, 16 * bj, N, N, S.A, LDA, S.HA + A0, LDN, AR, true, S.C, LDM, S.lC, LDM, PY}; if (bi == bj) td[q].dadd = reg; else td[q].mirror = true;
                      if (A0 > 0) { td[q].T = S.HA; td[q].ldt = LDN; td[q].tmode = 2; td[q].tsplit = A0; td[q].tscale = dt; } }
        else if (t < t2) td[q] = MTileT<R>{S.Qux, LDM, nullptr, 0, 16 * ((t - t1) % TM), 16 * ((t - t1) / TM), M, N, S.B, LDA, S.HA + A0, LDN, AR, true, S.D, LDM, S.lC, LDM, PY};
        else { td[q] = MTileT<R>{S.Quu, LDM, S.Quu, LDM, 16 * ((t - t2) % TM), 16 * ((t - t2) / TM), M, M, S.B, LDA, S.HB + A0, LDN, AR, true, S.D, LDM, S.lD, LDM, PY}; if ((t - t2) % TM == (t - t2) / TM) td[q].dadd = reg; }
    }
    mfma_tiles<(NTL > 0 ? NTL : 1), (AR + 3) / 4 * 4, (PY + 3) / 4 * 4, R>(lane, td);
}

template <int W, int N, int M, int PY, class R>
HD void sweep_tiles3(SweepLdsT<N, M, PY, R>& S, int lane) {
    constexpr int LDN = SweepLdsT<N, M, PY, R>::LDN, LDM = SweepLdsT<N, M, PY, R>::LDM;
    constexpr int TN = (N + 15) / 16;
    constexpr int NTL = (TN * TN - W + 3) / 4;
    if (NTL <= 0) return;
    MTileT<R> td[NTL > 0 ? NTL : 1];
    _Pragma("unroll") for (int q = 0; q < NTL; q++) {
        struct E3 { static constexpr bool edge(int e) { return mfma_edge_tile<R>(N, N, 16 * (e % TN), 16 * (e / TN)); } };
        const int t = deal_order<E3>(TN * TN, W + 4 * q);
        td[q] = MTileT<R>{S.H, LDN, S.H, LDN, 16 * (t % TN), 16 * (t / TN), N, N, S.Qux, LDM, S.K, LDM, M, true, nullptr, 0, nullptr, 0, 0};
    }
    mfma_tiles<(NTL > 0 ? NTL : 1), (M + 3) / 4 * 4, 0, R>(lane, td);
}

template <int W, int N, int M, int PY, class R>
HD void sweep_tilesK(SweepLdsT<N, M, PY, R>& S, int lane) {
    constexpr int LDM = SweepLdsT<N, M, PY, R>::LDM;
    constexpr int TN = (N + 15) / 16, TM = (M + 15) / 16;
    constexpr int NTL = (TM * TN - W + 3) / 4;
    if (NTL <= 0) return;
    MTileT<R> td[NTL > 0 ? NTL : 1];
    _Pragma("unroll") for (int q = 0; q < NTL; q++) {
        const int t = W + 4 * q;
        td[q] = MTileT<R>{S.K, LDM, nullptr, 0, 16 * (t % TM), 16 * (t / TM), M, N, S.LQ, LDM, S.Qux, LDM, M, false, nullptr, 0, nullptr, 0, 0};
    }
    mfma_tiles<(NTL > 0 ? NTL : 1), (M + 3) / 4 * 4, 0, R>(lane, td);
}

template <int NT, int N, int M, int PY, class R, class LDS>
HD bool riccati_phase(LDS& SS, const PhaseDev& P, int b, R reg) {
    using RL = RecLayout<N, M, PY>; using ST = SweepLdsT<N, M, PY, R>;
    static_assert(NT == 256 && RL::rounds + 1 <= SW_PRE && N <= SW_N && 2 * N + M + PY <= NT && 64 + M <= NT - N - 1 - M && N <= 64 && M <= 64, "sweep limits");
    constexpr bool WBS = (N == 36 && M == 12 && PY == 12);
    constexpr bool OVL = SW_OVERLAP_LDLT != 0;
    constexpr int GN0 = WBS ? 64 : 0, G0 = WBS ? 64 : NT - N, DV0 = WBS ? 64 + N : NT - N - 1, DU0 = WBS ? 64 + N + 1 : NT - N - 1 - M;
    constexpr int LDN = ST::LDN, LDM = ST::LDM, AR = ST::AR, LDA = ST::LDA, A0 = ST::A0;
    static_assert(sizeof(ST) <= sizeof(SS.raw), "the view fits the raw LDS block of its model set");
    ST& S = *reinterpret_cast<ST*>(SS.raw); SweepCtl& SWC = SS.c;
    constexpr int TN = (N + 15) / 16, TM = (M + 15) / 16, TP = (PY + 15) / 16;
    const int h = P.h; const R dtR = (R)P.dt;
    const auto grec = rec_of<R>(P); const auto gDefect = P.Defect; const auto gQu = P.Qu; const auto gQuu = P.Quu; const auto gQux = P.Qux;
    const auto gK = P.K; const auto gdU = P.dU; const auto gG = P.G;
    SW_PRE_DECL
    HS_PHASE(NT, { const int i = tid % N, j0 = tid / N; if (j0 < NT / N) for (int j = j0; j < N; j += NT / N) CM(S.H, i, j, LDN) += P.Phixx[(size_t)b * N * N + i + N * j]; }
             if (tid < N) { const R g = SWC.xfer[tid] + P.Phix[(size_t)b * N + tid]; S.G[tid] = g; gG[((size_t)b * (h + 1) + h) * N + tid] = g; }
             if (tid == 0) { SWC.ok = 1; }
             SW_RICCATI_FETCH((size_t)b * h + (h - 1), h - 1) SW_RICCATI_FETCH_LXX((size_t)b * h + (h - 1)))
    for (int k = h - 1; k >= 0; k--) {
        const size_t kk = (size_t)b * h + k;
        SW_STAMP0()
        HS_PHASE_L(NT, SW_RICCATI_COMMIT() if (k > 0) SW_RICCATI_FETCH(kk - 1, k - 1))
        SW_STAMP(0)
        HS_PHASE_L(NT, {
            const int w = tid >> 6, lane = tid & 63;
            if constexpr (OVL && M > 12) {
            switch (w) { case 0: sweep_tiles1<0, N, M, PY, R>(S, lane, dtR); break; case 1: sweep_tiles1<1, N, M, PY, R>(S, lane, dtR); break;
                         case 2: sweep_tiles1<2, N, M, PY, R>(S, lane, dtR); break; default: sweep_tiles1<3, N, M, PY, R>(S, lane, dtR); }
            } else if constexpr (OVL) {
            switch (w) { case 0: sweep_tiles1<0, N, M, PY, R, 1>(S, lane, dtR);
#ifndef HS_HOST_EMU
                                 __builtin_amdgcn_fence(__ATOMIC_RELEASE, "wavefront"); __builtin_amdgcn_wave_barrier(); __builtin_amdgcn_fence(__ATOMIC_ACQUIRE, "wavefront");
#endif
                                 sweep_tiles2<0, N, M, PY, R, 1>(S, lane, reg, dtR); break;
                         case 1: sweep_tiles1<1, N, M, PY, R, 1>(S, lane, dtR); break;
                         case 2: sweep_tiles1<2, N, M, PY, R, 1>(S, lane, dtR); break; default: sweep_tiles1<3, N, M, PY, R, 1>(S, lane, dtR); }
            } else {
            switch (w) { case 0: sweep_tiles1<0, N, M, PY, R>(S, lane, dtR); break; case 1: sweep_tiles1<1, N, M, PY, R>(S, lane, dtR); break;
                         case 2: sweep_tiles1<2, N, M, PY, R>(S, lane, dtR); break; default: sweep_tiles1<3, N, M, PY, R>(S, lane, dtR); }
            }
            if (tid >= GN0 && tid < GN0 + N) { const int i = tid - GN0; R s = S.G[i]; _Pragma("unroll 6") for (int j = 0; j < N; j++) s += CM(S.H, i, j, LDN) * S.def[j]; S.Gn[i] = s; }
            SW_WSTAMP(0)
        })
        if constexpr (OVL && M > 12) {
            HS_PHASE_L(NT, { const int w = tid >> 6, lane = tid & 63;
                switch (w) { case 0: sweep_tiles2<0, N, M, PY, R, 2>(S, lane, reg, dtR); break; case 1: sweep_tiles2<1, N, M, PY, R, 2>(S, lane, reg, dtR); break;
                             case 2: sweep_tiles2<2, N, M, PY, R, 2>(S, lane, reg, dtR); break; default: sweep_tiles2<3, N, M, PY, R, 2>(S, lane, reg, dtR); } })
        }
        SW_STAMP(1)
        if constexpr (OVL) {
        HS_PHASE_L(NT, {
            const int w = tid >> 6, lane = tid & 63;
            switch (w) { case 0: break; case 1: sweep_tiles2<1, N, M, PY, R, 1>(S, lane, reg, dtR); break;
                         case 2: sweep_tiles2<2, N, M, PY, R, 1>(S, lane, reg, dtR); break; default: sweep_tiles2<3, N, M, PY, R, 1>(S, lane, reg, dtR); }
            if (tid >= 128 && tid < 128 + N) {
                const int i = tid - 128; R s = 0;
                if (A0 > 0) s = (i < A0) ? S.Gn[i] : dtR * S.Gn[i - A0];
                _Pragma("unroll 6") for (int t = 0; t < AR; t++) s += CM(S.A, t, i, LDA) * S.Gn[A0 + t];
                if (PY > 0) { _Pragma("unroll 6") for (int t = 0; t < PY; t++) s += CM(S.C, t, i, LDM) * S.ly[t]; }
                S.Qx[i] += s;
            } else if (tid >= 192 && tid < 192 + M) {
                const int a = tid - 192; R s = 0;
                _Pragma("unroll 6") for (int t = 0; t < AR; t++) s += CM(S.B, t, a, LDA) * S.Gn[A0 + t];
                if (PY > 0) { _Pragma("unroll 6") for (int t = 0; t < PY; t++) s += CM(S.D, t, a, LDM) * S.ly[t]; }
                S.Qu[a] += s;
            }
            if (w == 0) ldlt_parts<M, LDM, R, 1>(lane, S.Quu, R(-1e-9), S.LQ, S.HB, reinterpret_cast<int*>(S.HB + M * M), &SWC.ok);
            SW_WSTAMP(1)
        })
        SW_STAMP(2)
        HS_PHASE_L(NT,
            if (tid < 64) ldlt_parts<M, LDM, R, 2>(tid, S.Quu, R(-1e-9), S.LQ, S.HB, reinterpret_cast<int*>(S.HB + M * M), &SWC.ok, S.HA, S.A);
            else for (int e = tid - 64; e < TN * 256; e += NT - 64) {
                const int i = 16 * (e >> 8) + (e & 15), j = 16 * (e >> 8) + ((e >> 4) & 15);
                if (i < j && j < N) { const R s = (CM(S.H, i, j, LDN) + CM(S.H, j, i, LDN)) / 2; CM(S.H, i, j, LDN) = s; CM(S.H, j, i, LDN) = s; }
            })
        SW_STAMP(5)
        } else {
        HS_PHASE_L(NT, {
            const int w = tid >> 6, lane = tid & 63;
            switch (w) { case 0: sweep_tiles2<0, N, M, PY, R>(S, lane, reg, dtR); break; case 1: sweep_tiles2<1, N, M, PY, R>(S, lane, reg, dtR); break;
                         case 2: sweep_tiles2<2, N, M, PY, R>(S, lane, reg, dtR); break; default: sweep_tiles2<3, N, M, PY, R>(S, lane, reg, dtR); }
            if (tid >= 128 && tid < 128 + N) {
                const int i = tid - 128; R s = 0;
                if (A0 > 0) s = (i < A0) ? S.Gn[i] : dtR * S.Gn[i - A0];
                _Pragma("unroll 6") for (int t = 0; t < AR; t++) s += CM(S.A, t, i, LDA) * S.Gn[A0 + t];
                if (PY > 0) { _Pragma("unroll 6") for (int t = 0; t < PY; t++) s += CM(S.C, t, i, LDM) * S.ly[t]; }
                S.Qx[i] += s;
            } else if (tid >= 192 && tid < 192 + M) {
                const int a = tid - 192; R s = 0;
                _Pragma("unroll 6") for (int t = 0; t < AR; t++) s += CM(S.B, t, a, LDA) * S.Gn[A0 + t];
// ... 20 lines not shown
        }
        if (!SWC.ok) return false;
        SW_STAMP(6)
        HS_PHASE_L(NT,
            { const int w = tid >> 6, lane = tid & 63;
              switch (w) { case 0: sweep_tilesK<0, N, M, PY, R>(S, lane); break; case 1: sweep_tilesK<1, N, M, PY, R>(S, lane); break;
                           case 2: sweep_tilesK<2, N, M, PY, R>(S, lane); break; default: sweep_tilesK<3, N, M, PY, R>(S, lane); } }
            if (tid >= NT - M) { const int i = tid - (NT - M); R s = 0; _Pragma("unroll") for (int t = 0; t < M; t++) s += CM(S.LQ, i, t, LDM) * S.Qu[t]; S.dU[i] = s; }
            SW_RICCATI_LXX() if (k > 0) SW_RICCATI_FETCH_LXX(kk - 1) SW_WSTAMP(2))
        HS_PHASE_L(NT,
            { const int w = tid >> 6, lane = tid & 63;
              switch (w) { case 0: sweep_tiles3<0, N, M, PY, R>(S, lane); break; case 1: sweep_tiles3<1, N, M, PY, R>(S, lane); break;
                           case 2: sweep_tiles3<2, N, M, PY, R>(S, lane); break; default: sweep_tiles3<3, N, M, PY, R>(S, lane); } }
            if constexpr (!WBS && M > 12) {
                constexpr int CH = (M + 3) / 4;
                SW_QUAD_ROWS(N, { _Pragma("unroll") for (int jj = 0; jj < CH; jj++) { const int t = part * CH + jj; if (t < M) partial += CM(S.Qux, t, o, LDM) * S.dU[t]; } },
                             { const R s = S.Qx[o] + total; S.G[o] = s; gG[((size_t)b * (h + 1) + k) * N + o] = s; })
            }
            if ((WBS || M <= 12) && tid >= G0 && tid < G0 + N) { const int i = tid - G0; R s = S.Qx[i]; _Pragma("unroll") for (int t = 0; t < M; t++) s += CM(S.Qux, t, i, LDM) * S.dU[t]; S.G[i] = s; gG[((size_t)b * (h + 1) + k) * N + i] = s; }
            else if (tid == DV0) { R dVk = 0; _Pragma("unroll") for (int t = 0; t < M; t++) dVk -= S.Qu[t] * S.dU[t]; SWC.dV1 -= dVk; SWC.dV2 += dVk; }
            else if (tid >= DU0 && tid < DU0 + M) { const int a = tid - DU0; gdU[kk * M + a] = S.dU[a]; } SW_WSTAMP(3))
        SW_STAMP(7)
        if constexpr (OVL) {
        HS_PHASE_L(NT, st_mat<NT>(tid, gK + kk * M * N, S.K, LDM, M, N); if (tid < M) gQu[kk * M + tid] = S.Qu[tid];
                   st_mat<NT>(tid, gQuu + kk * M * M, S.Quu, LDM, M, M); st_mat<NT>(tid, gQux + kk * M * N, S.Qux, LDM, M, N);)
        } else {
        HS_PHASE_L(NT, st_mat<NT>(tid, gK + kk * M * N, S.K, LDM, M, N);)
        }
        SW_STAMP(8)
    }
    HS_PHASE(NT, if (tid < N) S.def[tid] = gDefect[((size_t)b * (h + 1)) * N + tid];)
    HS_PHASE(NT, if (tid < N) { R s = S.G[tid]; for (int j = 0; j < N; j++) s += CM(S.H, tid, j, LDN) * S.def[j]; S.Gn[tid] = s; })
    HS_PHASE(NT, if (tid < N) { SWC.xfer[tid] = S.Gn[tid]; gG[((size_t)b * (h + 1)) * N + tid] = S.Gn[tid]; }
             st_mat<NT>(tid, P.H0 + (size_t)b * N * N, S.H, LDN, N, N);)
    return true;
}

template <int NT, class R, int SET, class LDS>
HD bool riccati_sweep(LDS& S, const PhaseDev* ph, int nph, int b, R reg) {
    HS_PHASE(NT, if (tid == 0) { S.c.dV1 = 0.0; S.c.dV2 = 0.0; })
    for (int i = nph - 1; i >= 0; i--) {
        const PhaseDev& P = ph[i];
        const int n = P.n;
        if (i == nph - 1) {
            HS_PHASE(NT, for (int e = tid; e < (n + 1) * n; e += NT) S.raw[e] = 0.0; if (tid < n) S.c.xfer[tid] = 0.0;)
        } else {
            const int nn = P.next_n, ldh = nn + 1;
            R* Hn = S.raw;
            R* Px = S.raw + (n + 1) * n;
            R* HP = S.raw + 2 * (n + 1) * n;
            const auto* Pxg = P.Px + (size_t)b * nn * n;
            R gnew = 0.0;
            HS_PHASE(NT, for (int e = tid; e < nn * n; e += NT) Px[e] = Pxg[e];)
            HS_PHASE(NT,
                for (int e = tid; e < nn * n; e += NT) { const int r = e % nn, c = e / nn; R s = 0; for (int t = 0; t < nn; t++) s += Hn[r + ldh * t] * Px[t + nn * c]; HP[e] = s; }
                if (tid >= NT - n) { const int i2 = tid - (NT - n); R s = 0; for (int t = 0; t < nn; t++) s += Px[t + nn * i2] * S.c.xfer[t]; S.raw[3 * (n + 1) * n + i2] = s; })
            (void)gnew;
            HS_PHASE(NT,
                for (int e = tid; e < n * n; e += NT) { const int r = e % n, c = e / n; R s = 0; for (int t = 0; t < nn; t++) s += Px[t + nn * r] * HP[t + nn * c]; S.raw[r + (n + 1) * c] = s; }
                if (tid >= NT - n) S.c.xfer[tid - (NT - n)] = S.raw[3 * (n + 1) * n + tid - (NT - n)];)
        }
        bool ok;
        if constexpr (SET == SW_SET_WB) {
            if (P.model == HSDDP_MODEL_WB) ok = riccati_phase<NT, 36, 12, 12, R>(S, P, b, reg); else ok = riccati_phase<NT, 12, 12, 0, R>(S, P, b, reg);
        } else {
            if (P.model == HSDDP_MODEL_SRB) ok = riccati_phase<NT, 12, 12, 0, R>(S, P, b, reg); else ok = riccati_phase<NT, 24, 24, 0, R>(S, P, b, reg);
        }
        if (!ok) return false;
    }
    return true;
}

#define SW_LIN_FETCH(kk_, k_) { \
    const HS_GLOBAL R* rec_ = grec + (kk_) * (size_t)RL::size + tid; \
    _Pragma("unroll") for (int r = 0; r < RL::rA; r++) PRE(r) = rec_[RL::oA + NT * r]; \
    _Pragma("unroll") for (int r = 0; r < RL::rQ; r++) PRE(RL::rA + r) = rec_[RL::oLxx + NT * r]; \
    _Pragma("unroll") for (int r = 0; r < RL::rB; r++) PRE(RL::rA + RL::rQ + r) = rec_[RL::oB + NT * r]; \
    _Pragma("unroll") for (int r = 0; r < rK; r++) { const int e = tid + NT * r; PRE(RL::rA + RL::rQ + RL::rB + r) = (e < M * N) ? (R)gK[(kk_) * M * N + e] : R(0.0); } \
    _Pragma("unroll") for (int r = 0; r < RL::rLuu; r++) PRE(RL::rA + RL::rQ + RL::rB + rK + r) = rec_[RL::oLuu + NT * r]; \
    PRE(RL::rA + RL::rQ + RL::rB + rK + RL::rLuu) = (tid < N + M) ? rec_[RL::oLx] : (tid < N + 2 * M) ? (R)gdU[(kk_) * M + tid - N - M] \
            : (tid < 2 * N + 2 * M) ? (R)gDefect[((size_t)b * (h + 1) + (k_) + 1) * N + tid - N - 2 * M] : R(0.0); }
#define SW_LIN_COMMIT(p_) { \
    R* A_ = S.A[p_]; R* Q_ = S.Q[p_]; R* B_ = S.B[p_]; R* K_ = S.K[p_]; R* U_ = S.U[p_]; R* v_ = S.v[p_]; \
    _Pragma("unroll") for (int r = 0; r < RL::rA; r++) { const int e = tid + NT * r; if (e < AR * N) A_[e] = PRE(r); } \
    _Pragma("unroll") for (int r = 0; r < RL::rQ; r++) { const int e = tid + NT * r; if (e < N * N) Q_[e] = PRE(RL::rA + r); } \
    _Pragma("unroll") for (int r = 0; r < RL::rB; r++) { const int e = tid + NT * r; if (e < AR * M) B_[e] = PRE(RL::rA + RL::rQ + r); } \
    _Pragma("unroll") for (int r = 0; r < rK; r++) { const int e = tid + NT * r; if (e < N * M) K_[e] = PRE(RL::rA + RL::rQ + RL::rB + r); } \
    _Pragma("unroll") for (int r = 0; r < RL::rLuu; r++) { const int e = tid + NT * r; if (e < M * M) U_[e] = PRE(RL::rA + RL::rQ + RL::rB + rK + r); } \
    { const R w_ = PRE(RL::rA + RL::rQ + RL::rB + rK + RL::rLuu); \
      if (tid < N) v_[tid] = w_; else if (tid < N + M) v_[64 + tid - N] = w_; \
      else if (tid < N + 2 * M) v_[128 + tid - N - M] = w_; else if (tid < 2 * N + 2 * M) v_[192 + tid - N - 2 * M] = w_; } }

template <int NT, int N, int M, int PY, class R, class LDS>
HD void linear_phase(LDS& SS, const PhaseDev& P, int b, R eps) {
    using RL = RecLayout<N, M, PY>; using ST = LinLdsT<N, M, PY, R>;
    constexpr int rK = rec_rnd(M * N) / 256, AR = ST::AR, A0 = ST::A0;
    static_assert(RL::rA + RL::rQ + RL::rB + rK + RL::rLuu + 1 <= SW_PRE && 2 * N + 2 * M <= NT && 4 * N <= 192 && 4 * M <= NT && 192 + M <= NT && N <= 64 && M <= 64, "prefetch registers / lane maps");
    const R dtR = (R)P.dt;
    static_assert(offsetof(ST, dx) >= 2 * NT * sizeof(R), "the partial-sum scratch must not reach dx");
    static_assert(sizeof(ST) <= sizeof(SS.raw), "the view fits the raw LDS block of its model set");
    ST& S = *reinterpret_cast<ST*>(SS.raw); SweepCtl& SWC = SS.c;
    const int h = P.h;
    const auto grec = rec_of<R>(P); const auto gDefect = P.Defect; const auto gK = P.K; const auto gdU = P.dU; const auto gdX = P.dX; const auto gKdX = P.KdX;
    SW_PRE_DECL
#ifdef HS_HOST_EMU
    static R acc1_all_[NT], acc2_all_[NT];
    for (int t = 0; t < NT; t++) { acc1_all_[t] = 0.0; acc2_all_[t] = 0.0; }
#define ACC1 acc1_all_[tid]
#define ACC2 acc2_all_[tid]
#else
    R acc1_ = 0.0, acc2_ = 0.0;
#define ACC1 acc1_
#define ACC2 acc2_
#endif
    HS_PHASE(NT, if (tid < N) { R v = SWC.xfer[tid] + eps * gDefect[((size_t)b * (h + 1)) * N + tid]; S.dx[tid] = v; gdX[((size_t)b * (h + 1)) * N + tid] = v; }
             SW_LIN_FETCH((size_t)b * h, 0))
    HS_PHASE_L(NT, SW_LIN_COMMIT(0) if (1 < h) SW_LIN_FETCH((size_t)b * h + 1, 1))
    for (int k = 0; k < h; k++) {
        const size_t kk = (size_t)b * h + k;
        const int p = k & 1;
        const R* A_ = S.A[p]; const R* Q_ = S.Q[p]; const R* B_ = S.B[p]; const R* K_ = S.K[p]; const R* U_ = S.U[p];
        const R* Qx_ = S.v[p]; const R* Qu_ = S.v[p] + 64; const R* dU_ = S.v[p] + 128; const R* def_ = S.v[p] + 192;
        const R* dxc = p ? S.dxn : S.dx; R* dxw = p ? S.dx : S.dxn;
        HS_PHASE_L(NT, SW_QUAD_ROWS(M, {
            constexpr int CH = (N + 3) / 4; R s = 0;
            _Pragma("unroll") for (int jj = 0; jj < CH; jj++) { const int j = part * CH + jj; if (j < N) s += CM(K_, o, j, M) * dxc[j]; }
            partial = s; }, { S.du[o] = eps * dU_[o] + total; gKdX[kk * M + o] = total; }))
        HS_PHASE_L(NT,
            SW_QUAD_ROWS(N, {
                constexpr int T = N + M; constexpr int CH = (T + 3) / 4; constexpr int CQ = (N + 3) / 4; R s = 0; R q = 0;
                if (o >= A0) {
                    _Pragma("unroll") for (int jj = 0; jj < CH; jj++) { const int t = part * CH + jj; if (t < N) s += CM(A_, o - A0, t, AR) * dxc[t]; else if (t < T) s += CM(B_, o - A0, t - N, AR) * S.du[t - N]; }
                } else if (part == 0) s = dxc[o] + dtR * dxc[A0 + o];
                _Pragma("unroll") for (int jj = 0; jj < CQ; jj++) { const int j = part * CQ + jj; if (j < N) q += CM(Q_, o, j, N) * dxc[j]; }
                partial = s; partial2 = q; }, {
                const R v = total + eps * def_[o];
                dxw[o] = v; gdX[((size_t)b * (h + 1) + k + 1) * N + o] = v;
                ACC2 += dxc[o] * total2;
                ACC1 += Qx_[o] * dxc[o]; })
            if (tid >= 192 && tid < 192 + M) {
                const int a = tid - 192; R q = 0;
                _Pragma("unroll") for (int j = 0; j < M; j++) q += CM(U_, a, j, M) * S.du[j];
                ACC2 += S.du[a] * q; ACC1 += Qu_[a] * S.du[a];
            }
            if (k + 1 < h) { SW_LIN_COMMIT(1 - p) if (k + 2 < h) SW_LIN_FETCH(kk + 2, k + 2) })
    }
    const R* dxe = (h & 1) ? S.dxn : S.dx;
    HS_PHASE(NT, for (int e = tid; e < N * N; e += NT) S.Q[0][e] = P.Phixx[(size_t)b * N * N + e];)
    HS_PHASE(NT, if (tid % SW_QS == 0 && tid / SW_QS < N) { const int o = tid / SW_QS;
                     R q = 0; for (int j = 0; j < N; j++) q += CM(S.Q[0], o, j, N) * dxe[j]; ACC2 += dxe[o] * q; ACC1 += P.Phix[(size_t)b * N + o] * dxe[o]; })
    R* scr = SS.raw;
    HS_PHASE(NT, scr[tid] = ACC1; scr[NT + tid] = ACC2;)
    HS_PHASE(NT, if (tid == 0) { R a1 = 0, a2 = 0; for (int j = 0; j < N; j++) { a1 += scr[SW_QS * j]; a2 += scr[NT + SW_QS * j]; }
                                 R b1 = 0, b2 = 0; for (int j = 0; j < M; j++) { b1 += scr[192 + j]; b2 += scr[NT + 192 + j]; }
                                 SWC.dV1 += a1 + b1; SWC.dV2 += a2; SWC.dV2 += b2; }
             if (tid >= 64 && tid < 64 + N) SWC.xfer[tid - 64] = dxe[tid - 64];)
#undef ACC1
#undef ACC2
}

template <int NT, class R, int SET, class LDS>
HD void linear_rollout(LDS& S, const PhaseDev* ph, int nph, int b, R eps) {
    HS_PHASE(NT, if (tid == 0) { S.c.dV1 = 0.0; S.c.dV2 = 0.0; } if (tid < SW_N) S.c.xfer[tid] = 0.0;)
    for (int i = 0; i < nph; i++) {
        const PhaseDev& P = ph[i];
        if (i > 0) {
            const PhaseDev& Pp = ph[i - 1]; const int np = Pp.n, n = P.n;
            const auto* Pxg = Pp.Px + (size_t)b * n * np;
            HS_PHASE(NT, if (tid < n) { R s = 0; for (int t = 0; t < np; t++) s += Pxg[tid + n * t] * S.c.xfer[t]; S.raw[tid] = s; })
            HS_PHASE(NT, if (tid < n) S.c.xfer[tid] = S.raw[tid];)
        }
        if constexpr (SET == SW_SET_WB) {
            if (P.model == HSDDP_MODEL_WB) linear_phase<NT, 36, 12, 12, R>(S, P, b, eps); else linear_phase<NT, 12, 12, 0, R>(S, P, b, eps);
        } else {
            if (P.model == HSDDP_MODEL_SRB) linear_phase<NT, 12, 12, 0, R>(S, P, b, eps); else linear_phase<NT, 24, 24, 0, R>(S, P, b, eps);
        }
    }
}

}
```

### cafe-mpc_amd/csrc/wb_knot.hpp

```cpp
#pragma once
#include "hs_types.hpp"
#include "wb_model.hpp"
#include "hs_mfma.hpp"

namespace hs {

struct WbCore {
    double x[36], xb[36], u[12], acc[18], tau[18], fext[12], cs[18], sn[18];
    double M[18 * 18];
    double h[18], Jall[12 * 18], Jdv[12], fpos[12], fvel[12];
    double JX[432];
    double gam[12];
    double GG[288 + 2 * MAXG];
    HD double* Jc() { return JX; }
    HD double* Xm() { return JX + 216; }
    HD double* G() { return GG; }
    HD double* LG() { return GG + 144; }
    HD double* gval() { return GG + 288; }
    HD double* bar() { return GG + 288 + MAXG; }
    HD double* dacc() { return GG; }
    HD double* dvel() { return GG + 216; }
    double a0[18], rhs[12], lam[12], qdd[18], grf[12], tmp[64], red[64], rdM[18], rdG[12];
    double wq[48];
    double xnext[36];
// ... 342 lines not shown
            if (part) { const int bs = 3 + (t >> 2); seed = base_seed(bs); leg = t & 3; slot = 4 * bs + leg; }
            else { const int jl = t - 12; seed = 42 + jl; leg = jl / 3; }
            LaneCfg c = lane_cfg(md, true, 0.0, 0.0, 1.0, vscale_kin, ascale_kin, -1, seed - 36, -1);
            c.l0 = leg; c.l1 = leg + 1; c.body = false; c.partial = part;
            DSink sk{&D, &L, seed, slot};
            wb_pass<Dual, DSink, 2>(c, L.x, L.x + 18, L.acc, L.cs, L.sn, L.fext, sk);
            if (!part) zero_rest(seed, leg);
        }
        for (int e = tid; e < 108; e += NT) { const int sd = e / 18, i = e % 18; D.W[i * WT + (sd < 3 ? sd : 33 + sd)] = 0.0; }
        for (int e = tid; e < 36; e += NT) { const int j = e / 12, r = e % 12; L.dacc()[r * 18 + j] = 0.0; L.dvel()[r * 18 + j] = 0.0; }
        if (NT >= 128 && chol_g && tid >= 64) WB_CHOL_G(D.LGs, D.rdGs, tid - 64);
        WB_W1_STAMP_END(6))
    HS_PHASE(NT, if (tid < (q_only ? 6 : 12)) {
        const int seed = base_seed(tid), tq = seed < 18 ? seed : seed >= 36 ? seed - 36 : -1;
        V3<Dual> fb = {Dual(0.0), Dual(0.0), Dual(0.0)}, nb = fb;
        for (int l = 0; l < 4; l++) {
            const double* p = D.JPW + 12 * (4 * tid + l);
            fb = fb + V3<Dual>{Dual(p[0], p[1]), Dual(p[2], p[3]), Dual(p[4], p[5])}; nb = nb + V3<Dual>{Dual(p[6], p[7]), Dual(p[8], p[9]), Dual(p[10], p[11])};
        }
        auto SC = [&](int i, Dual& s_, Dual& c_) { const double c0 = L.cs[i], s0 = L.sn[i]; const bool sd = (tq == i); s_ = Dual(s0, sd ? c0 : 0.0); c_ = Dual(c0, sd ? -s0 : 0.0); };
        Dual c3, s3, c4, s4, c5, s5;
        SC(3, s3, c3); SC(4, s4, c4); SC(5, s5, c5);
        DSink sk{&D, &L, seed, 0};
        sk.tau(5, nb.x);
        V3<Dual> f = rot<0>(c5, s5, fb), n = rot<0>(c5, s5, nb);
        sk.tau(4, n.y);
        f = rot<1>(c4, s4, f); n = rot<1>(c4, s4, n);
        sk.tau(3, n.z);
        f = rot<2>(c3, s3, f);
        sk.tau(0, f.x); sk.tau(1, f.y); sk.tau(2, f.z);
    })
}

HD double reb_barrier(double g, double delta) {
    if (g > delta) return -log(g);
    double t = (g - 2 * delta) / delta;
    return .5 * (t * t - 1) - log(delta);
}

HD double wb_constraint(PhaseC& P, const WbCore& L, int c) {
    if (P.go_torque >= 0 && c >= P.go_torque && c < P.go_torque + 24) { int i = c - P.go_torque; return i < 12 ? -L.u[i] + P.torque_limit : L.u[i - 12] + P.torque_limit; }
    if (P.go_jspeed >= 0 && c >= P.go_jspeed && c < P.go_jspeed + 24) { int i = c - P.go_jspeed; return i < 12 ? L.x[24 + i] - P.jspeed_lb : -L.x[24 + i - 12] + P.jspeed_ub; }
    if (P.go_joint >= 0 && c >= P.go_joint && c < P.go_joint + 24) { int i = c - P.go_joint; return i < 12 ? L.x[6 + i] - pick3(P.joint_lb, i % 3) : -L.x[6 + i - 12] + pick3(P.joint_ub, i % 3); }
    if (P.go_height >= 0 && c == P.go_height) return L.x[2] - P.h_min;
    int i = c - P.go_grf, a = i / 5, r = i % 5, f = feet_of(P)[a];
    double fx = L.grf[3 * f], fy = L.grf[3 * f + 1], fz = L.grf[3 * f + 2];
    if (r == 0) return fz;
    if (r == 1) return -fx + P.mu * fz;
    if (r == 2) return fx + P.mu * fz;
    if (r == 3) return -fy + P.mu * fz;
    return fy + P.mu * fz;
}

HD double wb_constraint_sel(PhaseC& P, const WbCore& L, int c) {
    const double* w = reinterpret_cast<const double*>(&L);
    constexpr int OX = offsetof(WbCore, x) / 8, OU = offsetof(WbCore, u) / 8, OG = offsetof(WbCore, grf) / 8;
    const int it = c - P.go_torque, is = c - P.go_jspeed, ij = c - P.go_joint;
    const bool bt = P.go_torque >= 0 && it >= 0 && it < 24, bs = P.go_jspeed >= 0 && is >= 0 && is < 24, bj = P.go_joint >= 0 && ij >= 0 && ij < 24;
    const bool bh = P.go_height >= 0 && c == P.go_height, lin = bt || bs || bj || bh;
    const int i = bt ? it : bs ? is : ij, lo = i < 12 ? i : i - 12;
    const bool up = i >= 12;
    const int a3 = lo % 3;
    const double cj = up ? pick3(P.joint_ub, a3) : -pick3(P.joint_lb, a3);
    const double c0 = bt ? P.torque_limit : bs ? (up ? P.jspeed_ub : -P.jspeed_lb) : bj ? cj : -P.h_min;
    const double sg = bt ? (up ? 1.0 : -1.0) : (bh || !up) ? 1.0 : -1.0;
    const int i1l = bt ? OU + lo : bs ? OX + 24 + lo : bj ? OX + 6 + lo : OX + 2;
    const int ig = lin ? 0 : c - P.go_grf, ga = ig / 5, gr = ig - 5 * ga, f = feet_of(P).pick(ga & 3);
    const int i1 = lin ? i1l : OG + 3 * f + 2, i2 = lin ? i1l : OG + 3 * f + (gr >= 3 ? 1 : 0);
    const double v1 = w[i1], v2 = w[i2];
    const double a = lin ? sg : (gr == 0 ? 1.0 : P.mu);
    const double t2 = lin ? c0 : (gr == 0 ? 0.0 : ((gr == 1 || gr == 3) ? -v2 : v2));
    return hs_fma(a, v1, t2);
}
HD double reb_barrier1(double g, double delta) {
    const bool above = g > delta;
    const double lg = log(above ? g : delta);
    double q = 0.0;
    if (!above) { const double t = (g - 2 * delta) / delta; q = .5 * (t * t - 1); }
    return above ? -lg : q - lg;
}

struct SlotOut { double* cost; double* dsq; double* ming; double* maxh; };

template <int NT, int CNT, int ROWS, class DST, class F>
HD void store_image(DST dst, int tid, F f) {
    constexpr int R = (CNT + NT - 1) / NT;
    const int c0 = tid / ROWS, r0 = tid - ROWS * c0;
    double v[R];
    _Pragma("unroll")
    for (int q = 0; q < R; q++) {
        const int e = tid + NT * q; int r = r0 + (NT * q) % ROWS, c = c0 + (NT * q) / ROWS;
        if (r >= ROWS) { r -= ROWS; c++; }
        v[q] = 0.0;
        if (R * NT == CNT || e < CNT) v[q] = f(e, r, c);
    }
    _Pragma("unroll")
    for (int q = 0; q < R; q++) { const int e = tid + NT * q; if (R * NT == CNT || e < CNT) dst[e] = v[q]; }
}

template <int NT>
HD void wb_rollout_knot(WbCore& L, PhaseC& P, const ModelDev& md, int b, int k, double eps, int reb_active,
                        const double* x0, SlotOut so, size_t slot, int* fail_flag, bool ss = false, bool wr = true) {
    const int h = P.h;
    const size_t kx = ((size_t)b * (h + 1) + k) * 36, ku = ((size_t)b * h + k) * 12;
    double* Kst = L.Jc();
    RL_STAMP0()
    const size_t kk = (size_t)b * h + k;
    struct Late { double kr[7]; } late[HS_NLANES(NT)];
    HS_PHASE(NT,
        const int g = tid < 36 ? 0 : tid < 48 ? 1 : tid < 60 ? 2 : 3, i = tid < 36 ? tid : tid < 48 ? tid - 36 : tid < 60 ? tid - 48 : 0;
        const double* pa = g == 0 ? P.Xbar + kx + i : (g == 1 && !ss) ? P.KdX + ku + i : P.Xbar + kx; const double* pb = P.dX + kx + (g == 0 ? i : 0);
        const double* rr = P.rref + ref_row(P, b, k) * 80;
        const double* pc = rr + tid;
        const double* pd = g == 0 ? P.Xbar + kx + (ss ? 0 : 36) + i : g == 1 ? P.Ubar + ku + i : rr + 64 + i;
        const double* pe = g == 0 ? P.dX + kx + (ss ? 0 : 36) + i : g == 1 ? P.dU + ku + i : rr;
        double va = *pa, vb = *pb, vc = *pc, vd = *pd, ve = *pe;
        const double* pw = tid < 36 ? &P.q[tid] : &P.r[tid < 48 ? tid - 36 : 0];
        const double vw = *pw;
        double er[2], dr[2];
        _Pragma("unroll") for (int q = 0; q < 2; q++) { const int c = q * NT + tid; er[q] = (c < P.ng) ? P.eps[kk * P.ng + c] : 0.0; dr[q] = (c < P.ng) ? P.delta[kk * P.ng + c] : 0.0; }
        if (ss) { Late& lt = late[HS_LANE(tid)]; _Pragma("unroll") for (int q = 0; q < 7; q++) { const int e = q * NT + tid; lt.kr[q] = (e < 432) ? P.K[kk * 432 + e] : 0.0; } }
        HS_CBAR();
        if (tid < 36) {
            const double xb = va, x = ss ? L.xnext[tid] : xb + eps * vb;
            L.xb[tid] = xb; L.x[tid] = x; if (wr) P.X[kx + tid] = x;
            L.tmp[tid] = vc; L.red[tid] = ss ? 0.0 : vd + eps * ve;
        } else if (tid < 48) {
            L.tmp[tid] = vc;
            if (ss) L.red[tid] = vd + eps * ve;
            else { const double u = vd + eps * (ve + va); L.u[i] = u; if (wr) P.U[ku + i] = u; L.tau[6 + i] = u; }
        }
        else if (tid < 60) { L.tmp[tid] = vc; L.red[tid] = vd; }
        else if (tid < 64) L.red[tid] = vc;
        if (tid < 18) { L.acc[tid] = 0.0; if (ss || tid < 6) L.tau[tid] = 0.0; } if (tid < 12) L.fext[tid] = 0.0; if (tid < 48) L.wq[tid] = vw;
        _Pragma("unroll") for (int q = 0; q < 2; q++) { const int c = q * NT + tid; if (c < P.ng) { L.gval()[c] = er[q]; L.bar()[c] = dr[q]; } })
    RL_STAMP(0)
    wb_terms<NT>(L, md, true);
    RL_STAMP(1)
    if (ss) {
        HS_PHASE(NT,
            const Late& lt = late[HS_LANE(tid)];
            _Pragma("unroll") for (int q = 0; q < 7; q++) { const int e = q * NT + tid; if (e < 432) Kst[e] = lt.kr[q]; })
        HS_PHASE(NT, if (tid < 12) {
            double s = 0; for (int j = 0; j < 36; j++) s += Kst[tid + 12 * j] * (L.x[j] - L.xb[j]);
            double u = L.red[36 + tid] + s;
            L.u[tid] = u; if (wr) P.U[ku + tid] = u; L.tau[6 + tid] = u;
        })
    }
    wb_kkt_direct<NT>(L, P.nc, feet_of(P), 0, P.bg_alpha);
    RL_STAMP(2)
    if (wr) {
        double* kc = P.kc + kk * KC_SIZE;
        HS_PHASE_L(NT,
            store_image<NT, 324, 324>(kc + KC_M, tid, [&](int e, int, int) { return L.M[e]; });
            store_image<NT, 216, 216>(kc + KC_X, tid, [&](int e, int, int) { return L.Xm()[e]; });
            store_image<NT, 216, 216>(kc + KC_J, tid, [&](int e, int, int) { return L.Jall[e]; });
            store_image<NT, 144, 144>(kc + KC_LG, tid, [&](int e, int, int) { return L.G()[e]; });
            if (tid < 18) { kc[KC_RDM + tid] = L.rdM[tid]; kc[KC_QDD + tid] = L.qdd[tid]; }
            if (tid < 12) { kc[KC_GRF + tid] = L.grf[tid]; kc[KC_LAM + tid] = L.lam[tid]; kc[KC_FP + tid] = L.fpos[tid]; kc[KC_FV + tid] = L.fvel[tid]; })
    }
    RL_STAMP(3)
    double* S = L.JX;
    HS_PHASE(NT, if (tid < 36) {
        const double xs = (tid < 18) ? L.x[tid] + L.x[18 + tid] * P.dt : L.x[tid] + L.qdd[tid - 18] * P.dt;
        if (wr) P.Xsim[kx + 36 + tid] = xs;
        const double xn = ss ? xs : L.red[tid];
        const double d = xs - xn; if (wr) P.Defect[kx + 36 + tid] = d;
        if (ss) { L.xnext[tid] = xs; if (k == 0 && wr) { P.Xsim[kx + tid] = L.x[tid]; P.Defect[kx + tid] = 0.0; } }
        double dsq = d * d;
        if (x0 != nullptr && k == 0) { const double d0 = x0[(size_t)b * 36 + tid] - L.x[tid]; if (wr) { P.Xsim[kx + tid] = x0[(size_t)b * 36 + tid]; P.Defect[kx + tid] = d0; } dsq += d0 * d0; }
        S[64 + tid] = dsq; S[100 + tid] = xs * xs;
        const double dx = L.x[tid] - L.tmp[tid]; S[tid] = dx * L.wq[tid] * dx;
    } else if (tid < 48) {
        const int i = tid - 36; if (wr) P.Y[kk * 12 + i] = L.grf[i];
        const double du = L.u[i] - L.tmp[tid]; S[tid] = du * L.wq[36 + i] * du;
    } else if (tid < 52) {
        const int f = tid - 48; const int rc = (int)L.red[60 + f];
        const double d0 = (L.fpos[3 * f] - L.x[0]) - L.red[48 + 3 * f], d1 = (L.fpos[3 * f + 1] - L.x[1]) - L.red[48 + 3 * f + 1], d2 = (L.fpos[3 * f + 2] - L.x[2]) - L.red[48 + 3 * f + 2];
        double l2 = 0, l3 = 0, l4 = 0;
        if (rc > 0 && P.w_foot_reg[0] >= 0) l2 = 0.5 * (d0 * P.w_foot_reg[0] * d0 + d1 * P.w_foot_reg[1] * d1 + d2 * P.w_foot_reg[2] * d2) * P.dt;
// ... 264 lines not shown
    LQ_STAMP(11)
    if (cached) {
        if (NT < 128) chol_f<NT, 12, 12>(D.LGs, D.LGs, D.rdGs, 0.0);
        LQ_STAMP(0)
    } else {
        HS_PHASE(NT, if (tid < 12) L.tau[6 + tid] = L.u[tid];)
        wb_terms<NT>(L, md, true);
        LQ_STAMP(0)
        wb_kkt_direct<NT>(L, P.nc, feet_of(P), 0, P.bg_alpha);
        wb_keep_schur<NT>(L, D);
    }
    LQ_STAMP(1)
    const int m = 3 * P.nc;
    HS_PHASE(NT, if (tid < 18) L.acc[tid] = L.qdd[tid]; if (tid < 12) L.fext[tid] = L.grf[tid];)
    wb_dpass<NT>(L, D, md, GRAV, 1.0, 1.0, 1.0, false, cached);
    LQ_STAMP(2)
    if (NT >= 128) {
        HS_WPHASE_W(0, if (tid < 48) {
        const int d = tid;
        double top[18], bot[12];
        {
            const int dc = d < 36 ? d : 35, c = dc < 18 ? dc : dc - 18, d2 = d < 18 ? d : 0;
            double w1[18], w2[18], vg[12], vd[12], vj[12];
            _Pragma("unroll") for (int i = 0; i < 18; i++) { w1[i] = D.W[wb_pi(i) * WT + dc]; w2[i] = D.W[wb_pi(i) * WT + 36 + d2]; }
            const Feet4 ft = feet_of(P);
            _Pragma("unroll") for (int a = 0; a < 12; a++) {
                const int r = 3 * ft[a / 3] + a % 3;
                vg[a] = L.G()[r * 18 + c]; vd[a] = L.dvel()[r * 18 + c]; vj[a] = L.Jall[r * 18 + c];
            }
            HS_CBAR();
            _Pragma("unroll") for (int i = 0; i < 18; i++) top[i] = (d < 36) ? (w1[i] + ((d < 18) ? w2[i] : 0.0)) : ((wb_pi(i) == 6 + d - 36) ? 1.0 : 0.0);
            _Pragma("unroll") for (int a = 0; a < 12; a++) {
                const double t1 = dc < 18 ? vg[a] : 2.0 * vd[a], t2 = dc < 18 ? vd[a] : vj[a];
                bot[a] = (a < m && d < 36) ? t1 + 2.0 * P.bg_alpha * t2 : 0.0;
            }
        }
        wb_kkt_column(L, D, top, bot, false, m);
        if (d < 36) {
            _Pragma("unroll")
            for (int i = 0; i < 18; i++) D.W[WR0 + wb_pi(i) * 36 + d] = -top[i] * dt + ((d == 18 + wb_pi(i)) ? 1.0 : 0.0);
            _Pragma("unroll")
            for (int a = 0; a < 12; a++) D.stC()[a + 12 * d] = 0.0;
            for (int a = 0; a < m; a++) D.stC()[(3 * P.feet[a / 3] + a % 3) + 12 * d] = bot[a];
        } else {
            const int j = d - 36;
            _Pragma("unroll")
            for (int i = 0; i < 18; i++) D.stB()[wb_pi(i) + 18 * j] = top[i] * dt;
            _Pragma("unroll")
            for (int a = 0; a < 12; a++) D.stD()[a + 12 * j] = 0.0;
            for (int a = 0; a < m; a++) D.stD()[(3 * P.feet[a / 3] + a % 3) + 12 * j] = -bot[a];
        }
        })
        LQ_STAMP(3)
        double* const T1 = L.Jc();
        WB_W1_STAMP_BEGIN()
        HS_WPHASE_W(1, wb_cost_blocks_lane(S, P, false, tid);
            if (tid < 36) {
                const int d = tid;
                double lxd = dt * L.wq[d] * (L.x[d] - L.tmp[d]);
                double diag = dt * L.wq[d];
                if (P.go_joint >= 0 && d >= 6 && d < 18) {
                    const int i = d - 6;
                    lxd += dt * (D.bd()[P.go_joint + i] - D.bd()[P.go_joint + 12 + i]); diag += dt * (D.bdd()[P.go_joint + i] + D.bdd()[P.go_joint + 12 + i]);
                }
                if (P.go_height >= 0 && d == 2) { lxd += dt * D.bd()[P.go_height]; diag += dt * D.bdd()[P.go_height]; }
                if (P.go_jspeed >= 0 && d >= 24) {
                    const int i = d - 24;
                    lxd += dt * (D.bd()[P.go_jspeed + i] - D.bd()[P.go_jspeed + 12 + i]); diag += dt * (D.bdd()[P.go_jspeed + i] + D.bdd()[P.go_jspeed + 12 + i]);
                }
                T1[d] = lxd; T1[36 + d] = diag;
            })
#ifdef HS_HOST_EMU
        static double emu_tile[1296];
        HS_WPHASE_W(1, if (tid < 37) {
            const int j = tid;
            auto E = [&](int k2, int c) { if (k2 < 12) return (c >= 3 && c < 18) ? L.Jall[k2 * 18 + c] : 0.0; const int r = k2 - 12; return c < 18 ? L.dvel()[r * 18 + c] : L.Jall[r * 18 + c - 18]; };
            for (int i = 0; i < 36; i++) {
                double sm = 0;
                for (int k2 = 0; k2 < 24; k2++) { const double w = k2 < 12 ? D.wp[k2] : D.wv[k2 - 12]; sm += w * E(k2, i) * (j < 36 ? E(k2, j) : (k2 < 12 ? D.ep[k2] : D.ev[k2 - 12])); }
                if (j < 36) emu_tile[i * 36 + j] = sm; else T1[120 + i] = sm;
            }
        })
        HS_WPHASE_W(1, if (tid < 36) { emu_tile[tid * 36 + tid] += T1[36 + tid]; P.lx[kk * P.rs + tid] = T1[tid] + T1[120 + tid]; })
        HS_WPHASE_W(1, store_image<64, 1296, 36>(P.lxx + kk * P.rs, tid, [&](int, int r, int c) { return emu_tile[c * 36 + r]; });)
#else
        HS_WPHASE_W(1, {
            const int li = tid & 15, lk = tid >> 4;
            d4_t c[3][3];
            wb_cost_gram_acc(L, D, tid, c);
            _Pragma("unroll") for (int ti = 0; ti < 3; ti++) _Pragma("unroll") for (int tj = 0; tj < 3; tj++) _Pragma("unroll") for (int q = 0; q < 4; q++) {
                const int row = 16 * ti + lk + 4 * q, col = 16 * tj + li;
                if (row < 36) {
                    if (col < 36) { double v = c[ti][tj][q]; if (row == col) v += T1[36 + row]; P.lxx[kk * P.rs + col + 36 * row] = v; }
                    else if (col == 36) P.lx[kk * P.rs + row] = T1[row] + c[ti][tj][q];
                }
            }
        })
#endif
        HS_WPHASE_W(1, if (tid < 12) {
            const int i = tid;
            double lu = dt * L.wq[36 + i] * (L.u[i] - L.tmp[36 + i]), luu = dt * L.wq[36 + i];
            if (P.go_torque >= 0) { lu += dt * (-D.bd()[P.go_torque + i] + D.bd()[P.go_torque + 12 + i]); luu += dt * (D.bdd()[P.go_torque + i] + D.bdd()[P.go_torque + 12 + i]); }
            P.lu[kk * P.rs + i] = lu; T1[72 + i] = luu;
            double ly = 0.0, b0 = 0.0, b1 = 0.0, b2 = 0.0; const int f = i / 3, r = i % 3; int a = -1; for (int t = 0; t < P.nc; t++) if (P.feet[t] == f) a = t;
            if (P.go_grf >= 0 && a >= 0) {
                const double mu = P.mu;
                for (int c = 0; c < 5; c++) {
                    const double r0 = (c == 1) ? -1.0 : (c == 2) ? 1.0 : 0.0, r1 = (c == 3) ? -1.0 : (c == 4) ? 1.0 : 0.0, r2 = (c == 0) ? 1.0 : mu;
                    const double rr = (r == 0) ? r0 : (r == 1) ? r1 : r2;
                    const double hb = dt * D.bdd()[P.go_grf + 5 * a + c] * rr;
                    ly += D.bd()[P.go_grf + 5 * a + c] * rr;
                    b0 += hb * r0; b1 += hb * r1; b2 += hb * r2;
                }
            }
            T1[84 + 3 * i] = b0; T1[85 + 3 * i] = b1; T1[86 + 3 * i] = b2;
            P.ly[kk * P.rs + i] = dt * ly;
        })
        HS_WPHASE_W(1, store_image<64, 144, 12>(P.luu + kk * P.rs, tid, [&](int, int r, int c) { return r == c ? T1[72 + r] : 0.0; });
                       store_image<64, 144, 12>(P.lyy + kk * P.rs, tid, [&](int, int r, int c) { return (r / 3 == c / 3) ? T1[84 + (r % 3) + 3 * c] : 0.0; });)
        WB_W1_STAMP_END(5)
        hs_phase_sync_all<NT>();
        HS_PHASE_L(NT,
            store_image<NT, 648, 18>(P.A + kk * P.rs, tid, [&](int, int r, int c) { return D.W[WR0 + r * 36 + c]; });
            store_image<NT, 432, 36>(P.C + kk * P.rs, tid, [&](int e, int, int) { return D.stC()[e]; });
            store_image<NT, 216, 18>(P.B + kk * P.rs, tid, [&](int e, int, int) { return D.stB()[e]; });
            store_image<NT, 144, 12>(P.D + kk * P.rs, tid, [&](int e, int, int) { return D.stD()[e]; });)
        LQ_STAMP(4)
        return;
    }
    HS_PHASE(NT, if (tid < 48) {
        const int d = tid;
        double top[18], bot[12];
        {
            const int dc = d < 36 ? d : 35, c = dc < 18 ? dc : dc - 18, d2 = d < 18 ? d : 0;
            double w1[18], w2[18], vg[12], vd[12], vj[12];
            _Pragma("unroll") for (int i = 0; i < 18; i++) { w1[i] = D.W[wb_pi(i) * WT + dc]; w2[i] = D.W[wb_pi(i) * WT + 36 + d2]; }
            const Feet4 ft = feet_of(P);
            _Pragma("unroll") for (int a = 0; a < 12; a++) {
                const int r = 3 * ft[a / 3] + a % 3;
                vg[a] = L.G()[r * 18 + c]; vd[a] = L.dvel()[r * 18 + c]; vj[a] = L.Jall[r * 18 + c];
            }
            HS_CBAR();
            _Pragma("unroll") for (int i = 0; i < 18; i++) top[i] = (d < 36) ? (w1[i] + ((d < 18) ? w2[i] : 0.0)) : ((wb_pi(i) == 6 + d - 36) ? 1.0 : 0.0);
            _Pragma("unroll") for (int a = 0; a < 12; a++) {
                const double t1 = dc < 18 ? vg[a] : 2.0 * vd[a], t2 = dc < 18 ? vd[a] : vj[a];
                bot[a] = (a < m && d < 36) ? t1 + 2.0 * P.bg_alpha * t2 : 0.0;
            }
        }
        wb_kkt_column(L, D, top, bot, false, m);
        if (d < 36) {
            _Pragma("unroll")
            for (int i = 0; i < 18; i++) D.W[WR0 + wb_pi(i) * 36 + d] = -top[i] * dt + ((d == 18 + wb_pi(i)) ? 1.0 : 0.0);
            _Pragma("unroll")
            for (int a = 0; a < 12; a++) D.stC()[a + 12 * d] = 0.0;
            for (int a = 0; a < m; a++) D.stC()[(3 * P.feet[a / 3] + a % 3) + 12 * d] = bot[a];
        } else {
            const int j = d - 36;
            _Pragma("unroll")
            for (int i = 0; i < 18; i++) D.stB()[wb_pi(i) + 18 * j] = top[i] * dt;
            _Pragma("unroll")
            for (int a = 0; a < 12; a++) D.stD()[a + 12 * j] = 0.0;
            for (int a = 0; a < m; a++) D.stD()[(3 * P.feet[a / 3] + a % 3) + 12 * j] = -bot[a];
        }
    })
    LQ_STAMP(3)
    HS_PHASE_L(NT,
        store_image<NT, 648, 18>(P.A + kk * P.rs, tid, [&](int, int r, int c) { return D.W[WR0 + r * 36 + c]; });
        store_image<NT, 432, 36>(P.C + kk * P.rs, tid, [&](int e, int, int) { return D.stC()[e]; });
        store_image<NT, 216, 18>(P.B + kk * P.rs, tid, [&](int e, int, int) { return D.stB()[e]; });
        store_image<NT, 144, 12>(P.D + kk * P.rs, tid, [&](int e, int, int) { return D.stD()[e]; });)
    LQ_STAMP(4)
    wb_cost_blocks<NT>(S, P, k, false);
    wb_cost_gram<NT>(S, D.JPW);
    HS_PHASE_L(NT, if (tid < 36) {
        const int d = tid;
        double lxd = dt * L.wq[d] * (L.x[d] - L.tmp[d]);
        double diag = dt * L.wq[d];
        lxd += D.JPW[d];
        if (P.go_joint >= 0 && d >= 6 && d < 18) {
            const int i = d - 6;
            lxd += dt * (D.bd()[P.go_joint + i] - D.bd()[P.go_joint + 12 + i]); diag += dt * (D.bdd()[P.go_joint + i] + D.bdd()[P.go_joint + 12 + i]);
        }
        if (P.go_height >= 0 && d == 2) { lxd += dt * D.bd()[P.go_height]; diag += dt * D.bdd()[P.go_height]; }
        if (P.go_jspeed >= 0 && d >= 24) {
            const int i = d - 24;
            lxd += dt * (D.bd()[P.go_jspeed + i] - D.bd()[P.go_jspeed + 12 + i]); diag += dt * (D.bdd()[P.go_jspeed + i] + D.bdd()[P.go_jspeed + 12 + i]);
        }
        D.W[d * 36 + d] += diag;
        P.lx[kk * P.rs + d] = lxd;
    })
    HS_PHASE_L(NT, store_image<NT, 1296, 36>(P.lxx + kk * P.rs, tid, [&](int, int r, int c) { return D.W[r * 36 + c]; });)
    LQ_STAMP(5)
    HS_PHASE_L(NT, for (int i = tid; i < 288; i += NT) L.Jc()[i] = 0.0;)
    HS_PHASE_L(NT, if (tid < 12) {
        const int i = tid;
        double lu = dt * L.wq[36 + i] * (L.u[i] - L.tmp[36 + i]), luu = dt * L.wq[36 + i];
        if (P.go_torque >= 0) { lu += dt * (-D.bd()[P.go_torque + i] + D.bd()[P.go_torque + 12 + i]); luu += dt * (D.bdd()[P.go_torque + i] + D.bdd()[P.go_torque + 12 + i]); }
        P.lu[kk * P.rs + i] = lu; L.Jc()[i + 12 * i] = luu;
        double ly = 0.0; const int f = i / 3, r = i % 3; int a = -1; for (int t = 0; t < P.nc; t++) if (P.feet[t] == f) a = t;
        if (P.go_grf >= 0 && a >= 0) {
            const double mu = P.mu;
            for (int c = 0; c < 5; c++) {
                const double r0 = (c == 1) ? -1.0 : (c == 2) ? 1.0 : 0.0, r1 = (c == 3) ? -1.0 : (c == 4) ? 1.0 : 0.0, r2 = (c == 0) ? 1.0 : mu;
                const double rr = (r == 0) ? r0 : (r == 1) ? r1 : r2;
                const double hb = dt * D.bdd()[P.go_grf + 5 * a + c] * rr;
                ly += D.bd()[P.go_grf + 5 * a + c] * rr;
                L.Jc()[144 + (3 * f) + 12 * i] += hb * r0; L.Jc()[144 + (3 * f + 1) + 12 * i] += hb * r1; L.Jc()[144 + (3 * f + 2) + 12 * i] += hb * r2;
            }
        }
        P.ly[kk * P.rs + i] = dt * ly;
    })
    HS_PHASE_L(NT, store_image<NT, 144, 12>(P.luu + kk * P.rs, tid, [&](int e, int, int) { return L.Jc()[e]; });
                   store_image<NT, 144, 12>(P.lyy + kk * P.rs, tid, [&](int e, int, int) { return L.Jc()[144 + e]; });)
    LQ_STAMP(6)
}

template <int NT>
HD void wb_lq_terminal(WbLqLds& S, PhaseC& P, PhaseC* Pn, const ModelDev& md, int b, int al_active) {
    WbCore& L = S.c; WbDeriv& D = S.d;
    const int h = P.h;
    const size_t kx = ((size_t)b * (h + 1) + h) * 36;
    HS_PHASE(NT, if (tid < 36) L.x[tid] = P.X[kx + tid]; if (tid < 18) { L.acc[tid] = 0.0; L.tau[tid] = 0.0; } if (tid < 12) L.fext[tid] = 0.0;
             wb_cost_prefetch(L, P, b, h, tid);)
    wb_terms<NT>(L, md, true);
    wb_dpass<NT>(L, D, md, 0.0, 1.0, 1.0, 0.0, true);
    wb_cost_blocks<NT>(S, P, h, true);
    HS_PHASE(NT, if (tid < 36) {
        const int d = tid;
        double px = P.qf[d] * (L.x[d] - L.tmp[d]);
        px += wb_cost_column(D, L.Jall, L.dvel(), d, D.W + d);
        double diag = P.qf[d];
        if (al_active && P.nt > 0) {
            int t = 0;
            for (int f = 0; f < 4; f++) if (P.td[f]) {
                const double sg = P.sigma[(size_t)b * P.nt + t], lm = P.lambda[(size_t)b * P.nt + t], hh = P.th[(size_t)b * P.nt + t];
                const double hd = d < 18 ? L.Jall[(3 * f + 2) * 18 + d] : 0.0;
                px += (sg * hh + lm) * hd;
                for (int i = 0; i < 18; i++) D.W[i * 36 + d] += (sg * (1 + hh) + lm) * (L.Jall[(3 * f + 2) * 18 + i] * hd);
                t++;
            }
        }
        D.W[d * 36 + d] += diag;
        P.Phix[(size_t)b * 36 + d] = px;
    })
    HS_PHASE(NT, for (int e = tid; e < 1296; e += NT) { const int r = e % 36, c = e / 36; P.Phixx[(size_t)b * 1296 + e] = D.W[r * 36 + c]; })
    if (Pn == nullptr) return;
    const int nn = Pn->n;
    if (!P.has_impact) {
        HS_PHASE(NT, for (int i = tid; i < nn * 36; i += NT) { int r = i % nn, c = i / nn; int src = (nn == 36) ? r : (r < 6 ? r : r + 12); P.Px[(size_t)b * nn * 36 + i] = (src == c) ? 1.0 : 0.0; })
        return;
    }
    int tdfeet[4] = {0, 0, 0, 0}; int ntd = 0; for (int f = 0; f < 4; f++) if (P.td[f]) tdfeet[ntd++] = f;
    const int m = 3 * ntd;
    wb_kkt_direct<NT>(L, ntd, Feet4{tdfeet[0], tdfeet[1], tdfeet[2], tdfeet[3]}, 1, 0.0);
    wb_keep_schur<NT>(L, D);
    HS_PHASE(NT, if (tid < 18) L.acc[tid] = L.qdd[tid] - L.x[18 + tid]; if (tid < 12) L.fext[tid] = 0.0;)
    HS_PHASE(NT, if (tid == 0) { double pad[16]; for (int i = 0; i < 16; i++) pad[i] = i < m ? L.lam[i] : 0.0;
                 for (int i = 0; i < ntd; i++) for (int d = 0; d < 3; d++) L.fext[3 * tdfeet[i] + d] = pad[i + d]; })
    wb_dpass<NT>(L, D, md, 0.0, 0.0, 0.0, 0.0, true);
    HS_PHASE(NT, if (tid < 18) for (int i = 0; i < 18; i++) D.W[i * WT + tid] += D.W[i * WT + 36 + tid];)
    HS_PHASE(NT, if (tid < 18) { L.xb[tid] = L.x[18 + tid]; })
    HS_PHASE(NT, if (tid < 18) { L.x[18 + tid] = L.qdd[tid]; })
    HS_PHASE(NT, if (tid >= 36 && tid < 54) {
        LaneCfg c = lane_cfg(md, true, 0.0, 0.0, 0.0, 1.0, 0.0, -1, tid - 36, -1);
        struct VSink { WbCore* C; int j; HD void tau(int, const Dual&) const {} HD void base(const V3<Dual>&, const V3<Dual>&) const {} HD void foot(int f, const V3<Dual>&, const V3<Dual>& v, const V3<Dual>&) const {
            C->dvel()[(3 * f) * 18 + j] = v.x.d; C->dvel()[(3 * f + 1) * 18 + j] = v.y.d; C->dvel()[(3 * f + 2) * 18 + j] = v.z.d; } } sk{&L, tid - 36};
        wb_pass<Dual>(c, L.x, L.x + 18, L.acc, L.cs, L.sn, L.fext, sk);
    })
    HS_PHASE(NT, if (tid < 36) {
        const int d = tid;
        double top[18], bot[12];
        _Pragma("unroll")
        for (int i = 0; i < 18; i++) {
            if (d < 18) top[i] = D.W[wb_pi(i) * WT + d];
            else { const int j = wb_pj(d - 18); top[i] = (i < j) ? L.M[j * 18 + i] : (i == j) ? 1.0 / L.rdM[j] : 0.0; }
        }
        _Pragma("unroll")
        for (int a = 0; a < 12; a++) bot[a] = (d < 18 && a < m) ? L.dvel()[(3 * tdfeet[a / 3] + a % 3) * 18 + d] : 0.0;
        wb_kkt_column(L, D, top, bot, d >= 18, m);
        _Pragma("unroll")
        for (int i = 0; i < 18; i++) D.W[WR0 + wb_pi(i) * 36 + d] = (d < 18) ? -top[i] : top[i];
    })
    HS_PHASE(NT, for (int e = tid; e < nn * 36; e += NT) {
        const int r = e % nn, c = e / nn;
        double v;
        if (nn == 36) v = (r < 18) ? ((r == c) ? 1.0 : 0.0) : D.W[WR0 + (r - 18) * 36 + c];
        else v = (r < 6) ? ((r == c) ? 1.0 : 0.0) : D.W[WR0 + (r - 6) * 36 + c];
        P.Px[(size_t)b * nn * 36 + e] = v;
    })
}

}
```

Measured before the change: 96110.

## Store per-knot LQ record matrices with padded leading dimensions matching LDS layout

The per-knot record images (A, B, C, D, Lxx, Luu, Lyy) are now written with a leading dimension of rows+1, the same padded stride the sweep's LDS tiles use. The sweep can then copy prefetched registers straight into LDS without the modulo/divide scatter per element. The knot writers, the host layout, and the readback path are all updated to the padded layout. The records grow slightly and every writer has to zero the pad entries, but the static_assert shows the rounded record sizes are unchanged.

```diff
diff --git a/cafe-mpc_amd/csrc/hkd_knot.hpp b/cafe-mpc_amd/csrc/hkd_knot.hpp
--- a/cafe-mpc_amd/csrc/hkd_knot.hpp
+++ b/cafe-mpc_amd/csrc/hkd_knot.hpp
@@ -3,6 +3,7 @@
 #include "srb_knot.hpp"
 
 namespace hs {
+using HRL = RecLayout<24, 24, 0>;
 
 constexpr double HKD_MASS = 8.912;
 constexpr double HKD_IXX = 0.02746078, HKD_IYY = 0.2425157968, HKD_IZZ = 0.2651935768;
@@ -170,8 +171,8 @@
         L.bd[c] = reb_active ? e * bd : 0.0; L.bdd[c] = reb_active ? e * bdd : 0.0;
     })
     const double fr = (P.w_foot_reg[0] >= 0) ? 1.0 : 0.0;
-    HS_PHASE(NT, for (int e = tid; e < 576; e += NT) {
-        const int r = e % 24, c = e / 24;
+    HS_PHASE(NT, for (int ep = tid; ep < HRL::sQ; ep += NT) {
+        const int c = ep / HRL::ldN; const bool pad = ep - HRL::ldN * c == 24; const int r = pad ? 0 : ep - HRL::ldN * c;
         double a, bb;
         if (r < 12) {
             if (c < 12) a = AB[r * 32 + c];
@@ -181,7 +182,8 @@
             a = (r == c) ? 1.0 : 0.0;
             bb = (r == c && !P.contact[(r - 12) / 3]) ? dt : 0.0;
         }
-        rec_put(P, kk, P.oA + e, a); rec_put(P, kk, P.oB + e, bb);
+        if (HS_REC_PAD_ABCD) { rec_put(P, kk, P.oA + ep, pad ? 0.0 : a); rec_put(P, kk, P.oB + ep, pad ? 0.0 : bb); }
+        else if (!pad) { rec_put(P, kk, P.oA + r + 24 * c, a); rec_put(P, kk, P.oB + r + 24 * c, bb); }
         double q = (r == c) ? dt * P.q[r] : 0.0;
         if (fr != 0.0) {
             if (r == c && r >= 3 && r < 6) { for (int f = 0; f < 4; f++) q += dt * P.contact[f] * P.w_foot_reg[r - 3]; }
@@ -189,7 +191,7 @@
             else if (r >= 3 && r < 6 && c >= 12 && (c - 12) % 3 == r - 3) q -= dt * P.contact[(c - 12) / 3] * P.w_foot_reg[r - 3];
             else if (c >= 3 && c < 6 && r >= 12 && (r - 12) % 3 == c - 3) q -= dt * P.contact[(r - 12) / 3] * P.w_foot_reg[c - 3];
         }
-        rec_put(P, kk, P.oLxx + e, q);
+        rec_put(P, kk, P.oLxx + ep, pad ? 0.0 : q);
         double uu = (r == c) ? dt * P.r[r] : 0.0;
         if (P.go_grf >= 0 && r < 12 && c < 12 && r / 3 == c / 3) {
             const int f = r / 3; int a2 = -1; for (int t = 0; t < P.nc; t++) if (P.feet[t] == f) a2 = t;
@@ -199,7 +201,7 @@
                 uu += dt * L.bdd[P.go_grf + 5 * a2 + cc] * vr * vc;
             }
         }
-        rec_put(P, kk, P.oLuu + e, uu);
+        rec_put(P, kk, P.oLuu + ep, pad ? 0.0 : uu);
     } if (tid < 24) {
         const int i = tid;
         const size_t rw = ref_row(P, b, k);
diff --git a/cafe-mpc_amd/csrc/hs_host.hpp b/cafe-mpc_amd/csrc/hs_host.hpp
--- a/cafe-mpc_amd/csrc/hs_host.hpp
+++ b/cafe-mpc_amd/csrc/hs_host.hpp
@@ -78,10 +78,11 @@
     al(&P.Quu, B * hh * m * m);
     {
         auto rnd = [](size_t x) { return (x + 255) / 256 * 256; };
-        const size_t ar = (size_t)rec_arows((int)n);
-        const size_t oA = 0, oLxx = oA + rnd(ar * n), oB = oLxx + rnd(n * n), oC = oB + rnd(ar * m), oD = oC + rnd(py * n), oLuu = oD + rnd(py * m),
-                     oLyy = oLuu + rnd(m * m), oLx = oLyy + rnd(py * py), oLu = oLx + n, oLy = oLu + m, size = oLx + rnd(n + m + py);
-        P.rs = (int)size;
+        const size_t lda = (size_t)rec_lda((int)n), ldn = (size_t)rec_ldn((int)n), ldm = (size_t)rec_ldm((int)m, (int)py), ldc = (size_t)rec_ldc((int)m, (int)py);
+        const size_t sC = py ? ldc * n : 0, sD = py ? ldc * m : 0, sLyy = py ? ldm * py : 0;
+        const size_t oA = 0, oLxx = oA + rnd(lda * n), oB = oLxx + rnd(ldn * n), oC = oB + rnd(lda * m), oD = oC + rnd(sC), oLuu = oD + rnd(sD),
+                     oLyy = oLuu + rnd(ldm * m), oLx = oLyy + rnd(sLyy), oLu = oLx + n, oLy = oLu + m, size = oLx + rnd(n + m + py);
+        P.rs = (int)size; P.batch = (int)B;
         P.oA = (int)oA; P.oLxx = (int)oLxx; P.oB = (int)oB; P.oC = (int)oC; P.oD = (int)oD; P.oLuu = (int)oLuu; P.oLyy = (int)oLyy; P.oLx = (int)oLx; P.oLu = (int)oLu; P.oLy = (int)oLy;
         if (f32) { void* p = mem.alloc(std::max<size_t>(B * hh * size, 1) * sizeof(float)); if (!p) ok = false; P.rec32 = (float*)p; }
         else al(&P.rec, B * hh * size);
@@ -155,12 +156,46 @@
         full[r + 36 * c] = v;
     }
 }
+inline bool rec_field_geom(const PhaseDev& P, int f, int& off, int& rows, int& ld, int& cols) {
+    const int n = P.n, m = P.m, p = P.p, ar = rec_arows(n), lda = rec_lda(n), ldn = rec_ldn(n), ldm = rec_ldm(m, p), ldc = rec_ldc(m, p);
+    switch (f) {
+        case HSDDP_F_A: off = P.oA; rows = ar; ld = lda; cols = n; return true;
+        case HSDDP_F_B: off = P.oB; rows = ar; ld = lda; cols = m; return true;
+        case HSDDP_F_C: off = P.oC; rows = p; ld = ldc; cols = n; return true;
+        case HSDDP_F_D: off = P.oD; rows = p; ld = ldc; cols = m; return true;
+        case HSDDP_F_LXX: off = P.oLxx; rows = n; ld = ldn; cols = n; return true;
+        case HSDDP_F_LUU: off = P.oLuu; rows = m; ld = ldm; cols = m; return true;
+        case HSDDP_F_LYY: off = P.oLyy; rows = p; ld = ldm; cols = p; return true;
+        case HSDDP_F_LX: off = P.oLx; rows = n; ld = n; cols = 1; return true;
+        case HSDDP_F_LU: off = P.oLu; rows = m; ld = m; cols = 1; return true;
+        case HSDDP_F_LY: off = P.oLy; rows = p; ld = p; cols = 1; return true;
+        default: return false;
+    }
+}
+template <class T> inline void rec_unpad(const T* img, int rows, int ld, int cols, double* dense) {
+    for (int c = 0; c < cols; c++) for (int r = 0; r < rows; r++) dense[r + rows * c] = (double)img[r + ld * c];
+}
+
+#ifdef HS_HOST_EMU
+inline const double* rec_dense_view(const PhaseDev& P, int f, const double* base, int count, int elems) {
+    static std::vector<double> view;
+    int off, rows, ld, cols;
+    if (!base || !rec_field_geom(P, f, off, rows, ld, cols)) return base;
+    const size_t recs = (size_t)P.batch * count;
+    view.assign(recs * (size_t)elems + 1, 0.0);
+    for (size_t r = 0; r < recs; r++) rec_unpad(base + r * P.rs, rows, ld, cols, view.data() + r * elems);
+    return view.data();
+}
+#endif
 
 inline const double* field_dev(const PhaseDev& P, int f, int& count, int& elems, int& stride) {
     const double* base = field_dev(P, f, count, elems);
-    const bool in_rec = (f == HSDDP_F_A || f == HSDDP_F_B || f == HSDDP_F_C || f == HSDDP_F_D || f == HSDDP_F_LX || f == HSDDP_F_LU || f == HSDDP_F_LY ||
-                         f == HSDDP_F_LXX || f == HSDDP_F_LUU || f == HSDDP_F_LYY);
+    int off, rows, ld, cols;
+    const bool in_rec = rec_field_geom(P, f, off, rows, ld, cols);
     stride = in_rec ? P.rs : elems;
+#ifdef HS_HOST_EMU
+    if (in_rec && base) { base = rec_dense_view(P, f, base, count, elems); stride = elems; }
+#endif
     return base;
 }
 
diff --git a/cafe-mpc_amd/csrc/hs_types.hpp b/cafe-mpc_amd/csrc/hs_types.hpp
--- a/cafe-mpc_amd/csrc/hs_types.hpp
+++ b/cafe-mpc_amd/csrc/hs_types.hpp
@@ -6,15 +6,24 @@
 constexpr int MAXN = 36, MAXM = 24, MAXP = 12, MAXG = 96;
 constexpr int rec_rnd(int x) { return (x + 255) / 256 * 256; }
 constexpr int rec_arows(int N) { return N == 36 ? 18 : N; }
+#ifndef HS_REC_PAD_ABCD
+#define HS_REC_PAD_ABCD 1
+#endif
+constexpr int rec_lda(int N) { return rec_arows(N) + (HS_REC_PAD_ABCD ? 1 : 0); }
+constexpr int rec_ldc(int M, int PY) { return HS_REC_PAD_ABCD ? (M > PY ? M : PY) + 1 : PY; }
+constexpr int rec_ldn(int N) { return N + 1; }
+constexpr int rec_ldm(int M, int PY) { return (M > PY ? M : PY) + 1; }
 template <int N, int M, int PY> struct RecLayout {
-    static constexpr int AR = rec_arows(N);
-    static constexpr int oA = 0, oLxx = oA + rec_rnd(AR * N), oB = oLxx + rec_rnd(N * N), oC = oB + rec_rnd(AR * M), oD = oC + rec_rnd(PY * N),
-                         oLuu = oD + rec_rnd(PY * M), oLyy = oLuu + rec_rnd(M * M), oLx = oLyy + rec_rnd(PY * PY), oLu = oLx + N, oLy = oLu + M,
+    static constexpr int AR = rec_arows(N), ldA = rec_lda(N), ldN = rec_ldn(N), ldM = rec_ldm(M, PY), ldC = rec_ldc(M, PY);
+    static constexpr int sA = ldA * N, sQ = ldN * N, sB = ldA * M, sC = PY > 0 ? ldC * N : 0, sD = PY > 0 ? ldC * M : 0, sLuu = ldM * M, sLyy = PY > 0 ? ldM * PY : 0;
+    static constexpr int oA = 0, oLxx = oA + rec_rnd(sA), oB = oLxx + rec_rnd(sQ), oC = oB + rec_rnd(sB), oD = oC + rec_rnd(sC),
+                         oLuu = oD + rec_rnd(sD), oLyy = oLuu + rec_rnd(sLuu), oLx = oLyy + rec_rnd(sLyy), oLu = oLx + N, oLy = oLu + M,
                          size = oLx + rec_rnd(N + M + PY);
-    static constexpr int rA = rec_rnd(AR * N) / 256, rQ = rec_rnd(N * N) / 256, rB = rec_rnd(AR * M) / 256, rC = rec_rnd(PY * N) / 256, rD = rec_rnd(PY * M) / 256,
-                         rLuu = rec_rnd(M * M) / 256, rLyy = rec_rnd(PY * PY) / 256;
+    static constexpr int rA = rec_rnd(sA) / 256, rQ = rec_rnd(sQ) / 256, rB = rec_rnd(sB) / 256, rC = rec_rnd(sC) / 256, rD = rec_rnd(sD) / 256,
+                         rLuu = rec_rnd(sLuu) / 256, rLyy = rec_rnd(sLyy) / 256;
     static constexpr int rounds = rA + rQ + rB + rC + rD + rLuu + rLyy;
 };
+static_assert(RecLayout<36, 12, 12>::size == 4096 && RecLayout<24, 24, 0>::size == 3328 && RecLayout<12, 12, 0>::size == 1280, "the padded images fit the rounds of the dense ones");
 
 constexpr int KC_M = 0, KC_X = 324, KC_LG = 540, KC_RDM = 684, KC_RDG = 702, KC_QDD = 714, KC_GRF = 732, KC_LAM = 744, KC_J = 756, KC_FP = 972, KC_FV = 984, KC_SIZE = 1024;
 
@@ -43,6 +52,7 @@
     HS_GLOBAL double *K, *Qux, *Quu;
     HS_GLOBAL double *A, *B, *C, *D;
     HS_GLOBAL double* rec; int rs;
+    int batch;
     HS_GLOBAL float* rec32;
     int oA, oLxx, oB, oC, oD, oLuu, oLyy, oLx, oLu, oLy;
     HS_GLOBAL double *l, *lbase, *lx, *lu, *ly, *lxx, *luu, *lyy;
diff --git a/cafe-mpc_amd/csrc/hsddp_hip.hip b/cafe-mpc_amd/csrc/hsddp_hip.hip
--- a/cafe-mpc_amd/csrc/hsddp_hip.hip
+++ b/cafe-mpc_amd/csrc/hsddp_hip.hip
@@ -1107,24 +1107,27 @@
     HIPCK(hipSetDevice(h->device));
     int count, elems, stride; const double* src = field_dev(h->ph[phase], field, count, elems, stride);
     const size_t sz = (size_t)count * elems;
-    if (h->f32 && stride != elems && sz > 0 && nb > 0) {
-        const PhaseDev& P = h->ph[phase];
-        const int off = field == HSDDP_F_A ? P.oA : field == HSDDP_F_B ? P.oB : field == HSDDP_F_C ? P.oC : field == HSDDP_F_D ? P.oD : field == HSDDP_F_LX ? P.oLx : field == HSDDP_F_LU ? P.oLu :
-                        field == HSDDP_F_LY ? P.oLy : field == HSDDP_F_LXX ? P.oLxx : field == HSDDP_F_LUU ? P.oLuu : P.oLyy;
-        std::vector<float> tmp(sz * nb);
-        HIPCK(hipMemcpy2D(tmp.data(), (size_t)elems * 4, P.rec32 + (size_t)b0 * count * stride + off, (size_t)stride * 4, (size_t)elems * 4, (size_t)nb * count, hipMemcpyDeviceToHost));
-        for (size_t i = 0; i < tmp.size(); i++) dst[i] = tmp[i];
+    const PhaseDev& P = h->ph[phase];
+    int off, rows, ld, cols;
+    const bool in_rec = rec_field_geom(P, field, off, rows, ld, cols);
+    if (in_rec && !h->f32 && !src) { memset(dst, 0, sz * nb * 8); return HSDDP_OK; }
+    if (in_rec) {
+        if (sz == 0 || nb == 0) return HSDDP_OK;
+        const size_t img = (size_t)ld * cols, recs = (size_t)nb * count, esz = h->f32 ? 4 : 8;
+        std::vector<unsigned char> tmp(img * recs * esz);
+        const void* from = h->f32 ? (const void*)(P.rec32 + (size_t)b0 * count * stride + off) : (const void*)(src + (size_t)b0 * count * stride);
+        HIPCK(hipMemcpy2D(tmp.data(), img * esz, from, (size_t)stride * esz, img * esz, recs, hipMemcpyDeviceToHost));
+        const bool wbs = wb_structured(P, field);
+        std::vector<double> low(wbs ? (size_t)rows * cols : 0);
+        for (size_t r = 0; r < recs; r++) {
+            double* out = wbs ? low.data() : dst + r * elems;
+            if (h->f32) rec_unpad((const float*)tmp.data() + r * img, rows, ld, cols, out); else rec_unpad((const double*)tmp.data() + r * img, rows, ld, cols, out);
+            if (wbs) wb_expand_ab(field, P.dt, low.data(), dst + r * elems);
+        }
         return HSDDP_OK;
     }
     if (!src) { memset(dst, 0, sz * nb * 8); return HSDDP_OK; }
     if (sz == 0 || nb == 0) return HSDDP_OK;
-    if (wb_structured(h->ph[phase], field)) {
-        const int st = field == HSDDP_F_A ? 648 : 216;
-        std::vector<double> tmp((size_t)st * nb * count);
-        HIPCK(hipMemcpy2D(tmp.data(), (size_t)st * 8, src + (size_t)b0 * count * stride, (size_t)stride * 8, (size_t)st * 8, (size_t)nb * count, hipMemcpyDeviceToHost));
-        for (size_t r = 0; r < (size_t)nb * count; r++) wb_expand_ab(field, h->ph[phase].dt, tmp.data() + r * st, dst + r * elems);
-        return HSDDP_OK;
-    }
     if (stride == elems) HIPCK(hipMemcpy(dst, src + (size_t)b0 * sz, sz * nb * 8, hipMemcpyDeviceToHost));
     else HIPCK(hipMemcpy2D(dst, (size_t)elems * 8, src + (size_t)b0 * count * stride, (size_t)stride * 8, (size_t)elems * 8, (size_t)nb * count, hipMemcpyDeviceToHost));
     return HSDDP_OK;
diff --git a/cafe-mpc_amd/csrc/srb_knot.hpp b/cafe-mpc_amd/csrc/srb_knot.hpp
--- a/cafe-mpc_amd/csrc/srb_knot.hpp
+++ b/cafe-mpc_amd/csrc/srb_knot.hpp
@@ -3,6 +3,7 @@
 #include "wb_knot.hpp"
 
 namespace hs {
+using SRL = RecLayout<12, 12, 0>;
 
 constexpr double SRB_MASS = 8.912;
 constexpr double SRB_IXX = 0.061578036, SRB_IYY = 0.2207093, SRB_IZZ = 0.272612336, SRB_IXZ = 5.38e-5;
@@ -124,12 +125,13 @@
         }
         L.bd = bd; L.bdd = bdd;
     })
-    HS_PHASE(NT, for (int e = tid; e < 144; e += NT) {
-        const int r = e % 12, c = e / 12;
-        rec_put(P, kk, P.oA + e, L.AB[e]); rec_put(P, kk, P.oB + e, L.AB[144 + e]);
+    HS_PHASE(NT, for (int ep = tid; ep < SRL::sQ; ep += NT) {
+        const int c = ep / SRL::ldN; const bool pad = ep - SRL::ldN * c == 12; const int r = pad ? 0 : ep - SRL::ldN * c; const int e = r + 12 * c;
+        if (HS_REC_PAD_ABCD) { rec_put(P, kk, P.oA + ep, pad ? 0.0 : L.AB[e]); rec_put(P, kk, P.oB + ep, pad ? 0.0 : L.AB[144 + e]); }
+        else if (!pad) { rec_put(P, kk, P.oA + e, L.AB[e]); rec_put(P, kk, P.oB + e, L.AB[144 + e]); }
         double qd = 0, rd = 0;
-        if (r == c) { qd = dt * P.q[r]; rd = dt * P.r[r]; if (r == 2) qd += dt * L.bdd; }
-        rec_put(P, kk, P.oLxx + e, qd); rec_put(P, kk, P.oLuu + e, rd);
+        if (r == c && !pad) { qd = dt * P.q[r]; rd = dt * P.r[r]; if (r == 2) qd += dt * L.bdd; }
+        rec_put(P, kk, P.oLxx + ep, qd); rec_put(P, kk, P.oLuu + ep, rd);
     } if (tid < 12) {
         double lx = dt * P.q[tid] * (L.x[tid] - P.xr[ref_row(P, b, k) * 12 + tid]); if (tid == 2) lx += dt * L.bd;
         rec_put(P, kk, P.oLx + tid, lx);
diff --git a/cafe-mpc_amd/csrc/sweep.hpp b/cafe-mpc_amd/csrc/sweep.hpp
--- a/cafe-mpc_amd/csrc/sweep.hpp
+++ b/cafe-mpc_amd/csrc/sweep.hpp
@@ -42,8 +42,9 @@
     R G[N], Gn[N], Qx[N], Qu[M], dU[M], ly[PYd], def[N];
 };
 template <int N, int M, int PY, class R = double> struct LinLdsT {
-    static constexpr int AR = rec_arows(N), A0 = N - AR;
-    R A[2][AR * N], Q[2][N * N], B[2][AR * M], K[2][M * N], U[2][M * M], v[2][256];
+    static constexpr int AR = rec_arows(N), A0 = N - AR, LDA = rec_lda(N), LDN = rec_ldn(N), LDM = rec_ldm(M, PY);
+    static constexpr int VS = 192 + N;
+    R A[2][LDA * N], Q[2][LDN * N], B[2][LDA * M], K[2][M * N], U[2][LDM * M], v[2][VS];
     R dx[N], dxn[N], du[M];
 };
 struct SweepCtl { double dV1, dV2, xfer[SW_N]; unsigned long long t_last; int ok; };
@@ -253,16 +254,22 @@
 #define SW_RICCATI_FETCH_LXX(kk_) { \
     const HS_GLOBAL R* rec_ = grec + (kk_) * (size_t)RL::size + tid; \
     _Pragma("unroll") for (int r = RL::rA; r < RL::rA + RL::rQ; r++) PRE(r) = rec_[NT * r]; }
-#define SW_RICCATI_LXX() { \
-    _Pragma("unroll") for (int r = 0; r < RL::rQ; r++) { const int e = tid + NT * r; if (e < N * N) S.H[(e % N) + LDN * (e / N)] += PRE(RL::rA + r); } }
+#ifndef SW_COPY_BOUND_ALL
+#define SW_COPY_BOUND_ALL (sizeof(R) == 4)
+#endif
+#define SW_COPY_ROUNDS(dst_, cnt_, rounds_, first_, pad_, OP) \
+    _Pragma("unroll") for (int r = 0; r < (rounds_); r++) { if ((!SW_COPY_BOUND_ALL && NT * (r + 1) <= (cnt_)) || tid + NT * r < (cnt_)) (dst_)[tid + NT * r] OP PRE((first_) + r); }
+#define SW_COPY_IMAGE(dst_, rows_, ldr_, ldt_, cols_, rounds_, first_) \
+    if constexpr ((ldr_) == (ldt_)) { SW_COPY_ROUNDS(dst_, (ldr_) * (cols_), rounds_, first_, 0, =) } \
+    else { _Pragma("unroll") for (int r = 0; r < (rounds_); r++) { const int e = tid + NT * r; if (e < (ldr_) * (cols_)) (dst_)[(e % ((ldr_) > 0 ? (ldr_) : 1)) + (ldt_) * (e / ((ldr_) > 0 ? (ldr_) : 1))] = PRE((first_) + r); } }
+#define SW_RICCATI_LXX() { SW_COPY_ROUNDS(S.H, RL::sQ, RL::rQ, RL::rA, N, +=) }
 #define SW_RICCATI_COMMIT() { \
-    constexpr int PYd = PY > 0 ? PY : 1; \
-    _Pragma("unroll") for (int r = 0; r < RL::rA; r++) { const int e = tid + NT * r; if (e < AR * N) S.A[(e % AR) + LDA * (e / AR)] = PRE(r); } \
-    _Pragma("unroll") for (int r = 0; r < RL::rB; r++) { const int e = tid + NT * r; if (e < AR * M) S.B[(e % AR) + LDA * (e / AR)] = PRE(RL::rA + RL::rQ + r); } \
-    _Pragma("unroll") for (int r = 0; r < RL::rC; r++) { const int e = tid + NT * r; if (e < PY * N) S.C[(e % PYd) + LDM * (e / PYd)] = PRE(RL::rA + RL::rQ + RL::rB + r); } \
-    _Pragma("unroll") for (int r = 0; r < RL::rD; r++) { const int e = tid + NT * r; if (e < PY * M) S.D[(e % PYd) + LDM * (e / PYd)] = PRE(RL::rA + RL::rQ + RL::rB + RL::rC + r); } \
-    _Pragma("unroll") for (int r = 0; r < RL::rLuu; r++) { const int e = tid + NT * r; if (e < M * M) S.Quu[(e % M) + LDM * (e / M)] = PRE(RL::rA + RL::rQ + RL::rB + RL::rC + RL::rD + r); } \
-    _Pragma("unroll") for (int r = 0; r < RL::rLyy; r++) { const int e = tid + NT * r; if (e < PY * PY) S.lyy[(e % PYd) + LDM * (e / PYd)] = PRE(RL::rA + RL::rQ + RL::rB + RL::rC + RL::rD + RL::rLuu + r); } \
+    SW_COPY_IMAGE(S.A, AR, RL::ldA, LDA, N, RL::rA, 0) \
+    SW_COPY_IMAGE(S.B, AR, RL::ldA, LDA, M, RL::rB, RL::rA + RL::rQ) \
+    SW_COPY_IMAGE(S.C, PY, RL::ldC, LDM, N, RL::rC, RL::rA + RL::rQ + RL::rB) \
+    SW_COPY_IMAGE(S.D, PY, RL::ldC, LDM, M, RL::rD, RL::rA + RL::rQ + RL::rB + RL::rC) \
+    SW_COPY_ROUNDS(S.Quu, RL::sLuu, RL::rLuu, RL::rA + RL::rQ + RL::rB + RL::rC + RL::rD, M, =) \
+    SW_COPY_ROUNDS(S.lyy, RL::sLyy, RL::rLyy, RL::rA + RL::rQ + RL::rB + RL::rC + RL::rD + RL::rLuu, PY, =) \
     if (tid < N) S.Qx[tid] = PRE(RL::rounds); else if (tid < N + M) S.Qu[tid - N] = PRE(RL::rounds); else if (tid < N + M + PY) S.ly[tid - N - M] = PRE(RL::rounds); \
     else if (tid < 2 * N + M + PY) S.def[tid - N - M - PY] = PRE(RL::rounds); }
 
@@ -359,6 +366,7 @@
     constexpr int GN0 = WBS ? 64 : 0, G0 = WBS ? 64 : NT - N, DV0 = WBS ? 64 + N : NT - N - 1, DU0 = WBS ? 64 + N + 1 : NT - N - 1 - M;
     constexpr int LDN = ST::LDN, LDM = ST::LDM, AR = ST::AR, LDA = ST::LDA, A0 = ST::A0;
     static_assert(sizeof(ST) <= sizeof(SS.raw), "the view fits the raw LDS block of its model set");
+    static_assert(RL::ldN == LDN && RL::ldM == LDM && RL::sQ == LDN * N && RL::sLuu == LDM * M && (!HS_REC_PAD_ABCD || (RL::ldA == LDA && RL::ldC == LDM)), "record images and LDS tiles share their leading dimensions");
     ST& S = *reinterpret_cast<ST*>(SS.raw); SweepCtl& SWC = SS.c;
     constexpr int TN = (N + 15) / 16, TM = (M + 15) / 16, TP = (PY + 15) / 16;
     const int h = P.h; const R dtR = (R)P.dt;
@@ -545,11 +553,9 @@
             : (tid < 2 * N + 2 * M) ? (R)gDefect[((size_t)b * (h + 1) + (k_) + 1) * N + tid - N - 2 * M] : R(0.0); }
 #define SW_LIN_COMMIT(p_) { \
     R* A_ = S.A[p_]; R* Q_ = S.Q[p_]; R* B_ = S.B[p_]; R* K_ = S.K[p_]; R* U_ = S.U[p_]; R* v_ = S.v[p_]; \
-    _Pragma("unroll") for (int r = 0; r < RL::rA; r++) { const int e = tid + NT * r; if (e < AR * N) A_[e] = PRE(r); } \
-    _Pragma("unroll") for (int r = 0; r < RL::rQ; r++) { const int e = tid + NT * r; if (e < N * N) Q_[e] = PRE(RL::rA + r); } \
-    _Pragma("unroll") for (int r = 0; r < RL::rB; r++) { const int e = tid + NT * r; if (e < AR * M) B_[e] = PRE(RL::rA + RL::rQ + r); } \
+    SW_COPY_ROUNDS(A_, RL::sA, RL::rA, 0, AR, =) SW_COPY_ROUNDS(Q_, RL::sQ, RL::rQ, RL::rA, N, =) SW_COPY_ROUNDS(B_, RL::sB, RL::rB, RL::rA + RL::rQ, AR, =) \
     _Pragma("unroll") for (int r = 0; r < rK; r++) { const int e = tid + NT * r; if (e < N * M) K_[e] = PRE(RL::rA + RL::rQ + RL::rB + r); } \
-    _Pragma("unroll") for (int r = 0; r < RL::rLuu; r++) { const int e = tid + NT * r; if (e < M * M) U_[e] = PRE(RL::rA + RL::rQ + RL::rB + rK + r); } \
+    SW_COPY_ROUNDS(U_, RL::sLuu, RL::rLuu, RL::rA + RL::rQ + RL::rB + rK, M, =) \
     { const R w_ = PRE(RL::rA + RL::rQ + RL::rB + rK + RL::rLuu); \
       if (tid < N) v_[tid] = w_; else if (tid < N + M) v_[64 + tid - N] = w_; \
       else if (tid < N + 2 * M) v_[128 + tid - N - M] = w_; else if (tid < 2 * N + 2 * M) v_[192 + tid - N - 2 * M] = w_; } }
@@ -557,7 +563,7 @@
 template <int NT, int N, int M, int PY, class R, class LDS>
 HD void linear_phase(LDS& SS, const PhaseDev& P, int b, R eps) {
     using RL = RecLayout<N, M, PY>; using ST = LinLdsT<N, M, PY, R>;
-    constexpr int rK = rec_rnd(M * N) / 256, AR = ST::AR, A0 = ST::A0;
+    constexpr int rK = rec_rnd(M * N) / 256, AR = ST::AR, A0 = ST::A0, LDA = ST::LDA, LDN = ST::LDN, LDM = ST::LDM;
     static_assert(RL::rA + RL::rQ + RL::rB + rK + RL::rLuu + 1 <= SW_PRE && 2 * N + 2 * M <= NT && 4 * N <= 192 && 4 * M <= NT && 192 + M <= NT && N <= 64 && M <= 64, "prefetch registers / lane maps");
     const R dtR = (R)P.dt;
     static_assert(offsetof(ST, dx) >= 2 * NT * sizeof(R), "the partial-sum scratch must not reach dx");
@@ -593,9 +599,9 @@
             SW_QUAD_ROWS(N, {
                 constexpr int T = N + M; constexpr int CH = (T + 3) / 4; constexpr int CQ = (N + 3) / 4; R s = 0; R q = 0;
                 if (o >= A0) {
-                    _Pragma("unroll") for (int jj = 0; jj < CH; jj++) { const int t = part * CH + jj; if (t < N) s += CM(A_, o - A0, t, AR) * dxc[t]; else if (t < T) s += CM(B_, o - A0, t - N, AR) * S.du[t - N]; }
+                    _Pragma("unroll") for (int jj = 0; jj < CH; jj++) { const int t = part * CH + jj; if (t < N) s += CM(A_, o - A0, t, LDA) * dxc[t]; else if (t < T) s += CM(B_, o - A0, t - N, LDA) * S.du[t - N]; }
                 } else if (part == 0) s = dxc[o] + dtR * dxc[A0 + o];
-                _Pragma("unroll") for (int jj = 0; jj < CQ; jj++) { const int j = part * CQ + jj; if (j < N) q += CM(Q_, o, j, N) * dxc[j]; }
+                _Pragma("unroll") for (int jj = 0; jj < CQ; jj++) { const int j = part * CQ + jj; if (j < N) q += CM(Q_, o, j, LDN) * dxc[j]; }
                 partial = s; partial2 = q; }, {
                 const R v = total + eps * def_[o];
                 dxw[o] = v; gdX[((size_t)b * (h + 1) + k + 1) * N + o] = v;
@@ -603,7 +609,7 @@
                 ACC1 += Qx_[o] * dxc[o]; })
             if (tid >= 192 && tid < 192 + M) {
                 const int a = tid - 192; R q = 0;
-                _Pragma("unroll") for (int j = 0; j < M; j++) q += CM(U_, a, j, M) * S.du[j];
+                _Pragma("unroll") for (int j = 0; j < M; j++) q += CM(U_, a, j, LDM) * S.du[j];
                 ACC2 += S.du[a] * q; ACC1 += Qu_[a] * S.du[a];
             }
             if (k + 1 < h) { SW_LIN_COMMIT(1 - p) if (k + 2 < h) SW_LIN_FETCH(kk + 2, k + 2) })
diff --git a/cafe-mpc_amd/csrc/wb_knot.hpp b/cafe-mpc_amd/csrc/wb_knot.hpp
--- a/cafe-mpc_amd/csrc/wb_knot.hpp
+++ b/cafe-mpc_amd/csrc/wb_knot.hpp
@@ -448,6 +448,8 @@
 
 struct SlotOut { double* cost; double* dsq; double* ming; double* maxh; };
 
+using WRL = RecLayout<36, 12, 12>;
+static_assert(WRL::ldN == 37 && WRL::ldM == 13 && WRL::ldA == 18 + HS_REC_PAD_ABCD && WRL::ldC == 12 + HS_REC_PAD_ABCD, "store_image_padded writes leading dimension rows + 1");
 template <int NT, int CNT, int ROWS, class DST, class F>
 HD void store_image(DST dst, int tid, F f) {
     constexpr int R = (CNT + NT - 1) / NT;
@@ -462,6 +464,27 @@
     }
     _Pragma("unroll")
     for (int q = 0; q < R; q++) { const int e = tid + NT * q; if (R * NT == CNT || e < CNT) dst[e] = v[q]; }
+}
+template <int NT, int ROWS, int COLS, class DST, class F>
+HD void store_image_padded(DST dst, int tid, F f) {
+    constexpr int CNT = ROWS * COLS, R = (CNT + NT - 1) / NT;
+    const int c0 = tid / ROWS, r0 = tid - ROWS * c0;
+    double v[R]; int cc[R];
+    _Pragma("unroll")
+    for (int q = 0; q < R; q++) {
+        const int e = tid + NT * q; int r = r0 + (NT * q) % ROWS, c = c0 + (NT * q) / ROWS;
+        if (r >= ROWS) { r -= ROWS; c++; }
+        v[q] = 0.0; cc[q] = c;
+        if (R * NT == CNT || e < CNT) v[q] = f(e, r, c);
+    }
+    _Pragma("unroll")
+    for (int q = 0; q < R; q++) { const int e = tid + NT * q; if (R * NT == CNT || e < CNT) dst[e + cc[q]] = v[q]; }
+    _Pragma("unroll")
+    for (int c = tid; c < COLS; c += NT) dst[ROWS + (ROWS + 1) * c] = 0.0;
+}
+template <int NT, int ROWS, int COLS, class DST, class F>
+HD void store_image_abcd(DST dst, int tid, F f) {
+    if constexpr (HS_REC_PAD_ABCD != 0) store_image_padded<NT, ROWS, COLS>(dst, tid, f); else store_image<NT, ROWS * COLS, ROWS>(dst, tid, f);
 }
 
 template <int NT>
@@ -892,7 +915,7 @@
             }
         })
         HS_WPHASE_W(1, if (tid < 36) { emu_tile[tid * 36 + tid] += T1[36 + tid]; P.lx[kk * P.rs + tid] = T1[tid] + T1[120 + tid]; })
-        HS_WPHASE_W(1, store_image<64, 1296, 36>(P.lxx + kk * P.rs, tid, [&](int, int r, int c) { return emu_tile[c * 36 + r]; });)
+        HS_WPHASE_W(1, store_image_padded<64, 36, 36>(P.lxx + kk * P.rs, tid, [&](int, int r, int c) { return emu_tile[c * 36 + r]; });)
 #else
         HS_WPHASE_W(1, {
             const int li = tid & 15, lk = tid >> 4;
@@ -901,8 +924,8 @@
             _Pragma("unroll") for (int ti = 0; ti < 3; ti++) _Pragma("unroll") for (int tj = 0; tj < 3; tj++) _Pragma("unroll") for (int q = 0; q < 4; q++) {
                 const int row = 16 * ti + lk + 4 * q, col = 16 * tj + li;
                 if (row < 36) {
-                    if (col < 36) { double v = c[ti][tj][q]; if (row == col) v += T1[36 + row]; P.lxx[kk * P.rs + col + 36 * row] = v; }
-                    else if (col == 36) P.lx[kk * P.rs + row] = T1[row] + c[ti][tj][q];
+                    if (col < 36) { double v = c[ti][tj][q]; if (row == col) v += T1[36 + row]; P.lxx[kk * P.rs + col + WRL::ldN * row] = v; }
+                    else if (col == 36) { P.lx[kk * P.rs + row] = T1[row] + c[ti][tj][q]; P.lxx[kk * P.rs + 36 + WRL::ldN * row] = 0.0; }
                 }
             }
         })
@@ -926,15 +949,15 @@
             T1[84 + 3 * i] = b0; T1[85 + 3 * i] = b1; T1[86 + 3 * i] = b2;
             P.ly[kk * P.rs + i] = dt * ly;
         })
-        HS_WPHASE_W(1, store_image<64, 144, 12>(P.luu + kk * P.rs, tid, [&](int, int r, int c) { return r == c ? T1[72 + r] : 0.0; });
-                       store_image<64, 144, 12>(P.lyy + kk * P.rs, tid, [&](int, int r, int c) { return (r / 3 == c / 3) ? T1[84 + (r % 3) + 3 * c] : 0.0; });)
+        HS_WPHASE_W(1, store_image_padded<64, 12, 12>(P.luu + kk * P.rs, tid, [&](int, int r, int c) { return r == c ? T1[72 + r] : 0.0; });
+                       store_image_padded<64, 12, 12>(P.lyy + kk * P.rs, tid, [&](int, int r, int c) { return (r / 3 == c / 3) ? T1[84 + (r % 3) + 3 * c] : 0.0; });)
         WB_W1_STAMP_END(5)
         hs_phase_sync_all<NT>();
         HS_PHASE_L(NT,
-            store_image<NT, 648, 18>(P.A + kk * P.rs, tid, [&](int, int r, int c) { return D.W[WR0 + r * 36 + c]; });
-            store_image<NT, 432, 36>(P.C + kk * P.rs, tid, [&](int e, int, int) { return D.stC()[e]; });
-            store_image<NT, 216, 18>(P.B + kk * P.rs, tid, [&](int e, int, int) { return D.stB()[e]; });
-            store_image<NT, 144, 12>(P.D + kk * P.rs, tid, [&](int e, int, int) { return D.stD()[e]; });)
+            store_image_abcd<NT, 18, 36>(P.A + kk * P.rs, tid, [&](int, int r, int c) { return D.W[WR0 + r * 36 + c]; });
+            store_image_abcd<NT, 12, 36>(P.C + kk * P.rs, tid, [&](int e, int, int) { return D.stC()[e]; });
+            store_image_abcd<NT, 18, 12>(P.B + kk * P.rs, tid, [&](int e, int, int) { return D.stB()[e]; });
+            store_image_abcd<NT, 12, 12>(P.D + kk * P.rs, tid, [&](int e, int, int) { return D.stD()[e]; });)
         LQ_STAMP(4)
         return;
     }
@@ -975,10 +998,10 @@
     })
     LQ_STAMP(3)
     HS_PHASE_L(NT,
-        store_image<NT, 648, 18>(P.A + kk * P.rs, tid, [&](int, int r, int c) { return D.W[WR0 + r * 36 + c]; });
-        store_image<NT, 432, 36>(P.C + kk * P.rs, tid, [&](int e, int, int) { return D.stC()[e]; });
-        store_image<NT, 216, 18>(P.B + kk * P.rs, tid, [&](int e, int, int) { return D.stB()[e]; });
-        store_image<NT, 144, 12>(P.D + kk * P.rs, tid, [&](int e, int, int) { return D.stD()[e]; });)
+        store_image_abcd<NT, 18, 36>(P.A + kk * P.rs, tid, [&](int, int r, int c) { return D.W[WR0 + r * 36 + c]; });
+        store_image_abcd<NT, 12, 36>(P.C + kk * P.rs, tid, [&](int e, int, int) { return D.stC()[e]; });
+        store_image_abcd<NT, 18, 12>(P.B + kk * P.rs, tid, [&](int e, int, int) { return D.stB()[e]; });
+        store_image_abcd<NT, 12, 12>(P.D + kk * P.rs, tid, [&](int e, int, int) { return D.stD()[e]; });)
     LQ_STAMP(4)
     wb_cost_blocks<NT>(S, P, k, false);
     wb_cost_gram<NT>(S, D.JPW);
@@ -999,7 +1022,7 @@
         D.W[d * 36 + d] += diag;
         P.lx[kk * P.rs + d] = lxd;
     })
-    HS_PHASE_L(NT, store_image<NT, 1296, 36>(P.lxx + kk * P.rs, tid, [&](int, int r, int c) { return D.W[r * 36 + c]; });)
+    HS_PHASE_L(NT, store_image_padded<NT, 36, 36>(P.lxx + kk * P.rs, tid, [&](int, int r, int c) { return D.W[r * 36 + c]; });)
     LQ_STAMP(5)
     HS_PHASE_L(NT, for (int i = tid; i < 288; i += NT) L.Jc()[i] = 0.0;)
     HS_PHASE_L(NT, if (tid < 12) {
@@ -1020,8 +1043,8 @@
         }
         P.ly[kk * P.rs + i] = dt * ly;
     })
-    HS_PHASE_L(NT, store_image<NT, 144, 12>(P.luu + kk * P.rs, tid, [&](int e, int, int) { return L.Jc()[e]; });
-                   store_image<NT, 144, 12>(P.lyy + kk * P.rs, tid, [&](int e, int, int) { return L.Jc()[144 + e]; });)
+    HS_PHASE_L(NT, store_image_padded<NT, 12, 12>(P.luu + kk * P.rs, tid, [&](int e, int, int) { return L.Jc()[e]; });
+                   store_image_padded<NT, 12, 12>(P.lyy + kk * P.rs, tid, [&](int e, int, int) { return L.Jc()[144 + e]; });)
     LQ_STAMP(6)
 }
 
```

Result: no change. 95630 (-0.5%).
